# facebookresearch/habitat-lab

Measured on AMD Instinct MI355X. Metric: env-steps/sec (SPS) PointNav RGB-D 256x256, 64 envs x 128 rollout, higher is better.
Workload: dtype f32; 1 GPU; PointNav SimpleCNN+GRU, 64 envs x 128 steps, 256x256 RGB-D synthetic; envs_per_gpu=64, rollout_steps=128, ppo_epoch=4, num_mini_batch=4, parallelism=dp1

## Files before the change

### habitat-lab_amd/csrc/conv_patch_bf3.h

```cpp
#pragma once
#include <atomic>
#include "igemm_bf3.h"

namespace hab {

constexpr int CPB_CC = 32;
constexpr int CPB_PIX = CPB_CC + 8;

struct PatchGeom {
    const float* in;
    int Hi, Wi, Ci;
    int Ho, Wo;
    int KH, KW, off_h, off_w;
    int flip;
    int TH, tiles_per_img, PW, PP;
    FastDiv dPW;
    int nt_m, nt_n;
};

template <class P, int TW, int WM, int WN, int TN, int BT>
struct ConvPatchCfg {
    static constexpr int NT = WM * WN * 64;
    static constexpr int BN = WN * TN * 32;
    static constexpr int ROWS_PER_MT = 32 / TW;
    static constexpr int TH = WM * ROWS_PER_MT;
    static constexpr int BP = BT * CPB_CC + 8;
    static constexpr int B_PLANE = BN * BP;
    static constexpr int MAX_PP = (TH + 2) * (TW + 2);
    static constexpr size_t LDS_BYTES = (size_t)(3 * MAX_PP * CPB_PIX + 3 * B_PLANE) * 2;
};

inline size_t cpb_w_elems(const ConvFwdProb& p) { return (size_t)p.N * p.K; }
inline size_t cpb_w_elems(const ConvDgradProb& p) { return (size_t)p.N * p.Kfull; }

__global__ void cpb_split_weights(const float* __restrict__ w, size_t n, unsigned short* __restrict__ planes) {
    const size_t e = (size_t)blockIdx.x * blockDim.x + threadIdx.x;
    if (e >= n) return;
    unsigned h1, h2, h3;
    bf3_split(w[e], h1, h2, h3);
    planes[e] = (unsigned short)h1; planes[n + e] = (unsigned short)h2; planes[2 * n + e] = (unsigned short)h3;
    bf3_split(-w[e], h1, h2, h3);
    planes[3 * n + e] = (unsigned short)h1; planes[4 * n + e] = (unsigned short)h2; planes[5 * n + e] = (unsigned short)h3;
}

constexpr int CPB_DRAW_SLOTS = 64;
__device__ unsigned cpb_draw_pool[CPB_DRAW_SLOTS * 16];

template <class P, int TW, int WM, int WN, int TN, int BT, bool PRE>
__global__ void __launch_bounds__(WM* WN * 64) conv_patch_bf3_kernel(const P p, const PatchGeom gq, const int sign_schedule,
                                                                      const unsigned short* __restrict__ wplanes, const size_t wn_elems,
                                                                      unsigned* __restrict__ dyn_ctr) {
    using Cfg = ConvPatchCfg<P, TW, WM, WN, TN, BT>;
    constexpr int NT = Cfg::NT, BN = Cfg::BN, BP = Cfg::BP, TH = Cfg::TH;
    constexpr int PU = (Cfg::MAX_PP * (CPB_CC / 4) + NT - 1) / NT;
    static_assert(EpiV4<P>::value, "transposed-accumulator epilogue");
    extern __shared__ __attribute__((aligned(16))) unsigned short smem16[];
    const int PPL = gq.PP * CPB_PIX;
    unsigned short* Pa = smem16;
    unsigned short* Bs = smem16 + 3 * Cfg::MAX_PP * CPB_PIX;

    const int t = threadIdx.x;
    const int lane = t & 63, wave = t >> 6;
    const int wm = wave / WN, wn = wave % WN;
    const int li = lane & 31, hi = lane >> 5;
    const int ntiles = gq.nt_m * gq.nt_n;
    auto tile_of = [&](int vb) {
        const int q = ntiles >> 3, r = ntiles & 7, xcd = vb & 7, idx = vb >> 3;
        return (xcd < r ? xcd * (q + 1) : r * (q + 1) + (xcd - r) * q) + idx;
    };
    const int ty = wm * Cfg::ROWS_PER_MT + li / TW, tx = li % TW;
    const int txc = tx < gq.Wo ? tx : gq.Wo - 1;
    const int pix0 = ty * gq.PW + txc;
    const int patch_units = gq.PP * (CPB_CC / 4);
    const int nchunks = gq.Ci / CPB_CC;
    const int nstage = 9 / BT;
    const typename P::KCtx kc = p.k_ctx(0, p.K);

    f32x4 pv[PU];
    int prow[PU], poff[PU];
#pragma unroll
    for (int j = 0; j < PU; ++j) {
        const int u = t + NT * j;
        const int pix = u >> 3, cq = u & 7;
        int pr, pc;
        gq.dPW.divmod(pix, pr, pc);
        const int w_ = pc + gq.off_w;
        const bool colok = (u < patch_units) & ((unsigned)w_ < (unsigned)gq.Wi);
        prow[j] = colok ? pr + gq.off_h : HAB_FAR;
        poff[j] = ((pr + gq.off_h) * gq.Wi + w_) * gq.Ci + cq * 4;
    }
    auto fetch_patch = [&](int tile_m, int chunk) {
        const int img = tile_m / gq.tiles_per_img, ho0 = (tile_m - img * gq.tiles_per_img) * TH;
        const float* base = gq.in + ((size_t)img * gq.Hi + ho0) * gq.Wi * gq.Ci + chunk * CPB_CC;
#pragma unroll
        for (int j = 0; j < PU; ++j) {
// ... 143 lines not shown
                    load_group(g + 1, 1);
                    constexpr int PA[6] = {2, 0, 1, 1, 0, 0}, PB[6] = {0, 2, 1, 0, 1, 0};
#pragma unroll
                    for (int q = 0; q < 6; ++q)
#pragma unroll
                        for (int j = 0; j < TN; ++j) {
                            acc[j] = __builtin_amdgcn_mfma_f32_32x32x16_bf16(bf[0][j][PB[q]], af[0][PA[q]], acc[j], 0, 0, 0);
                            acc2[j] = __builtin_amdgcn_mfma_f32_32x32x16_bf16(bf[1][j][PB[q]], af[1][PA[q]], acc2[j], 0, 0, 0);
                        }
                }
                __syncthreads();
            }
#pragma unroll
            for (int j = 0; j < TN; ++j)
#pragma unroll
                for (int v = 0; v < 16; ++v) {
                    tot[j][v] += acc[j][v] + acc2[j][v];
                    acc[j][v] = 0.0f; acc2[j][v] = 0.0f;
                }
        }
#pragma unroll
        for (int j = 0; j < TN; ++j)
#pragma unroll
            for (int v = 0; v < 16; ++v) acc[j][v] = flip_all ? -tot[j][v] : tot[j][v];
        {
            const int img = tile_m / gq.tiles_per_img, ho = (tile_m - img * gq.tiles_per_img) * TH + ty;
            const int m = (tx < gq.Wo && ho < gq.Ho) ? (img * gq.Ho + ho) * gq.Wo + tx : p.M;
            const typename P::EpiRow erow = p.epi_row(m);
#pragma unroll
            for (int j = 0; j < TN; ++j) {
                typename P::EpiCol4 ecol[4];
                typename P::EpiAux4 aux[4];
#pragma unroll
                for (int g = 0; g < 4; ++g) {
                    ecol[g] = p.epi_col4(n0 + (wn * TN + j) * 32 + 8 * g + 4 * hi);
                    aux[g] = p.epi_fetch4(erow, ecol[g]);
                }
#pragma unroll
                for (int g = 0; g < 4; ++g) {
                    f32x4 v;
                    v[0] = acc[j][4 * g]; v[1] = acc[j][4 * g + 1]; v[2] = acc[j][4 * g + 2]; v[3] = acc[j][4 * g + 3];
                    p.epi_store4(erow, ecol[g], aux[g], v);
                }
            }
        }
        if (!more) { leave(); break; }
        vb = vb_next;
        if (dyn) { const int i2 = s_draw[it & 1]; vb_next = i2 < run_len ? i2 * 8 + xcd : ntiles; }
        else vb_next = vb + gridDim.x;
        ++it;
    }
}

template <class P, int TW, int WM, int WN, int TN, int BT>
inline int conv_patch_bf3_launch(const P& p, PatchGeom gq, float* ws, size_t ws_floats, hipStream_t stream) {
    using Cfg = ConvPatchCfg<P, TW, WM, WN, TN, BT>;
    gq.TH = Cfg::TH;
    gq.tiles_per_img = cdiv(gq.Ho, Cfg::TH);
    gq.PW = gq.Wo + 2;
    gq.PP = (Cfg::TH + 2) * gq.PW;
    gq.dPW = FastDiv(gq.PW);
    if (gq.PP > Cfg::MAX_PP) return 1;
    const int B = p.M / (gq.Ho * gq.Wo);
    gq.nt_m = B * gq.tiles_per_img;
    gq.nt_n = cdiv(p.N, Cfg::BN);
    const int ntiles = gq.nt_m * gq.nt_n;
    static const int sign_schedule = !hab_env_flag("HAB_BF3_NOSIGN");
    constexpr int wgs_per_cu = 2;
    const int occ = (int)(160 * 1024 / Cfg::LDS_BYTES) < wgs_per_cu ? (int)(160 * 1024 / Cfg::LDS_BYTES) : wgs_per_cu;
    int grid = 256 * (occ > 0 ? occ : 1);
    if (grid > ntiles) grid = (ntiles + 7) / 8 * 8;
    constexpr int pre_min = 131072;
    const size_t wn_elems = cpb_w_elems(p);
    const bool pre = ws && ((reinterpret_cast<uintptr_t>(ws) & 15) == 0) && ws_floats * 4 >= wn_elems * 12 && p.M >= pre_min && (wn_elems % 4 == 0);
    hipError_t e = hipSuccess;
    static const bool dyn_on = !hab_env_flag("HAB_NO_DYN_TILES");
    unsigned* ctr = nullptr;
    if (dyn_on && grid < ntiles) {
        static std::atomic<unsigned> next_slot{0};
        static unsigned* pool = nullptr;
        static const hipError_t sym_err = hipGetSymbolAddress(reinterpret_cast<void**>(&pool), HIP_SYMBOL(cpb_draw_pool));
        if (sym_err != hipSuccess || !pool) return HAB_ERR_ARG;
        ctr = pool + (size_t)(next_slot.fetch_add(1, std::memory_order_relaxed) % CPB_DRAW_SLOTS) * 16;
    }
    if (pre) {
        auto kern = conv_patch_bf3_kernel<P, TW, WM, WN, TN, BT, true>;
        static const hipError_t attr_err = (Cfg::LDS_BYTES > 64 * 1024) ? hipFuncSetAttribute(reinterpret_cast<const void*>(kern), hipFuncAttributeMaxDynamicSharedMemorySize, (int)Cfg::LDS_BYTES) : hipSuccess;
        if (attr_err != hipSuccess) return (int)attr_err;
        unsigned short* planes = reinterpret_cast<unsigned short*>(ws);
        cpb_split_weights<<<(unsigned)((wn_elems + 255) / 256), 256, 0, stream>>>(p.w, wn_elems, planes);
        HAB_LAUNCH_CHECK();
        kern<<<grid, Cfg::NT, Cfg::LDS_BYTES, stream>>>(p, gq, sign_schedule, planes, wn_elems, ctr);
    } else {
        auto kern = conv_patch_bf3_kernel<P, TW, WM, WN, TN, BT, false>;
        static const hipError_t attr_err = (Cfg::LDS_BYTES > 64 * 1024) ? hipFuncSetAttribute(reinterpret_cast<const void*>(kern), hipFuncAttributeMaxDynamicSharedMemorySize, (int)Cfg::LDS_BYTES) : hipSuccess;
        if (attr_err != hipSuccess) return (int)attr_err;
        kern<<<grid, Cfg::NT, Cfg::LDS_BYTES, stream>>>(p, gq, sign_schedule, nullptr, 0, ctr);
    }
    HAB_LAUNCH_CHECK();
    return HAB_OK;
}

template <class P>
inline int conv_patch_bf3_dispatch(const P& p, const PatchGeom& gq, float* ws, size_t ws_floats, hipStream_t stream) {
    if (gq.KH != 3 || gq.KW != 3 || gq.Ci % CPB_CC != 0 || (p.N & 31) || gq.Wo > 32 || gq.Wo < 5 || p.M % (gq.Ho * gq.Wo) != 0) return 1;
    if (p.N != 32) return 1;
    if (gq.Wo > 16) return conv_patch_bf3_launch<P, 32, 4, 1, 1, 3>(p, gq, ws, ws_floats, stream);
    if (gq.Wo > 8) return conv_patch_bf3_launch<P, 16, 4, 1, 1, 3>(p, gq, ws, ws_floats, stream);
    return 1;
}

}
```

### habitat-lab_amd/csrc/engine.h

```cpp
#pragma once
#include <string.h>

#include <algorithm>
#include <string>
#include <vector>

#include "heads.h"
#include "ops.h"
#include "problems.h"
#include "resnet_ops.h"
#include "../../include/habitat_amd.h"

struct ParamSpec {
    std::string name;
    int64_t shape[4];
    int ndim;
    int64_t offset;
    int64_t numel;
    int is_buffer = 0;
};

struct Arena {
    int64_t used = 0;
    int64_t take(int64_t n) {
        const int64_t o = used;
        used += (n + 63) & ~(int64_t)63;
        return o;
    }
};

struct RnnForm {
    int chunks = 0;
    bool wave = false;
};

struct hab_policy {
    hab_policy_desc d;
    std::vector<ParamSpec> params;
    int64_t param_floats = 0, packed_floats = 0, work_floats = 0;
    float *P = nullptr, *G = nullptr, *PK = nullptr, *WK = nullptr;
    int64_t work_bound = 0;
    int Cin = 0;
    hab::ConvDesc c1, c2, c3;
    int fc_in = 0, rnn_in = 0, rnn_ld = 0, G_ = 3, L = 1;
    int i_c1w = -1, i_c1b = -1, i_c2w = -1, i_c2b = -1, i_c3w = -1, i_c3b = -1, i_fcw = -1, i_fcb = -1, i_aw = -1, i_ab = -1, i_cw = -1, i_cb = -1;
    int i_astd = -1;
    int head_K = 0;
    int64_t w_gsaved = -1;
    std::vector<int> i_wih, i_whh, i_bih, i_bhh;
    int64_t pk_c1f = -1, pk_c2f = -1, pk_c2d = -1, pk_c3f = -1, pk_c3d = -1, pk_fc = -1;
    int64_t pk_c1img = -1;
    std::vector<int64_t> pk_whht;
    std::vector<int64_t> pk_wiht;
    int64_t pk_wih0 = -1;
    int64_t w_a1 = -1, w_a2 = -1, w_a3 = -1, w_da1 = -1, w_da2 = -1, w_da3 = -1;
    int64_t w_rnnin = -1, w_drnnin = -1, w_hinit = -1, w_cinit = -1, w_probs = -1, w_logitsn = -1, w_dzv = -1, w_dv = -1, w_dfeat = -1,
            w_scratch = -1, w_value = -1, w_logp = -1, w_ent = -1, w_hmask = -1, w_gistep = -1, w_step_h = -1, w_ws = -1;
    std::vector<int64_t> w_gi, w_gates, w_hn, w_hprev, w_cprev, w_c, w_out, w_dgi, w_dgh, w_dlayer;
    int64_t ws_floats = 0;
    int last_B = 0, last_n = 0;
    const uint8_t* last_masks = nullptr;
    hipStream_t s2 = nullptr;
    std::vector<hipEvent_t> evs;
    int64_t w_ws2 = -1, ws2_floats = 0, w_fmask = -1, w_iota = -1;
    RnnForm form;
    struct ResNetPlan* rn = nullptr;
    int save_acts = 1;
    int training = 1;
    hab_allreduce_fn allreduce_cb = nullptr;
    void* allreduce_ctx = nullptr;
    int world_size = 1;
    hab_grad_ready_fn grad_ready_cb = nullptr;
    void* grad_ready_ctx = nullptr;
    struct hab_comm* comm = nullptr;
    const float* xg_feat = nullptr; const float* xg_perc = nullptr;
    int comm_err = 0;
    int64_t comm_first = -1;
    hipStream_t cur_stream = nullptr;
    uint64_t probe_mask = 0;
    struct ProbeEv { int tag; hipEvent_t first, second; };
    std::vector<ProbeEv> probe_events;
    size_t probe_used = 0;
    double probe_flops[64] = {0}, probe_bytes[64] = {0};

    float* p(int i) const { return P + params[i].offset; }
    float* g(int i) const { return G + params[i].offset; }
};

inline int add_param(hab_policy* e, const std::string& name, std::initializer_list<int64_t> shape) {
    ParamSpec s;
    s.name = name;
    s.ndim = (int)shape.size();
    s.numel = 1;
    int k = 0;
    for (auto v : shape) { s.shape[k++] = v; s.numel *= v; }
    for (; k < 4; ++k) s.shape[k] = 1;
    s.offset = e->param_floats;
    e->param_floats += (s.numel + 3) & ~(int64_t)3;
    e->params.push_back(s);
    return (int)e->params.size() - 1;
}
inline int conv_out(int x, int k, int s, int p) { return (x + 2 * p - k) / s + 1; }

void add_tail_params(hab_policy* e);
void pack_tail(hab_policy* e, Arena& pk);
void plan_tail_workspace(hab_policy* e, Arena& wk, int64_t ws_floats);
int repack_tail(hab_policy* e, hipStream_t s);
int build_resnet(hab_policy* e);
void destroy_resnet(hab_policy* e);
int resnet_repack(hab_policy* e, hipStream_t s);
void grad_tail_ready(hab_policy* e, int first_param);
int comm_exchange_async(struct hab_comm* c, float* buf, int64_t first, int64_t count, hipStream_t compute);
extern "C" int hab_comm_allreduce_sum(struct hab_comm* c, float* buf, int64_t count, hipStream_t stream);
int resnet_feature_shape(const hab_policy* e, int* c, int* hf, int* wf);
int resnet_encode(hab_policy* e, const hab_obs* obs, int n, float* out, hipStream_t s);
int resnet_encoder_forward(hab_policy* e, const hab_obs* obs, const uint8_t* masks, const int* rows, int B, hipStream_t s, int f0 = 0, int nB = -1);
int resnet_encoder_backward(hab_policy* e, const hab_obs* obs, const uint8_t* masks, const int* rows, int B, hipStream_t s);
int resnet_tap(hab_policy* e, int which, const float** ptr, int64_t* floats);

struct Probe {
    hab_policy* e; hipStream_t s; bool on;
    Probe(hab_policy* e_, int tag, hipStream_t s_, double flops = 0.0, double bytes = 0.0) : e(e_), s(s_), on((e_->probe_mask >> tag) & 1) {
        if (!on) return;
        e->probe_flops[tag] += flops; e->probe_bytes[tag] += bytes;
        if (e->probe_used == e->probe_events.size()) {
            hipEvent_t a, b;
            (void)hipEventCreate(&a); (void)hipEventCreate(&b);
            e->probe_events.push_back({tag, a, b});
        }
        e->probe_events[e->probe_used].tag = tag;
        (void)hipEventRecord(e->probe_events[e->probe_used].first, s);
    }
    ~Probe() {
        if (!on) return;
        (void)hipEventRecord(e->probe_events[e->probe_used].second, s);
        e->probe_used++;
    }
};
```

### habitat-lab_amd/csrc/engine.hip

```cpp
#include <string.h>

#include <algorithm>

#include <string>
#include <vector>

#include "engine.h"

using namespace hab;

static void plan_tm_workspace(hab_policy* e, Arena& wk);
void add_tail_params(hab_policy* e) {
    const hab_policy_desc& d = e->d;
    const int H = d.hidden;
    const std::string rn = "net.state_encoder.rnn.";
    for (int l = 0; l < d.rnn_layers; ++l) {
        const int in = l == 0 ? e->rnn_in : H;
        const std::string sfx = "_l" + std::to_string(l);
        e->i_wih.push_back(add_param(e, rn + "weight_ih" + sfx, {e->G_ * H, in}));
        e->i_whh.push_back(add_param(e, rn + "weight_hh" + sfx, {e->G_ * H, H}));
        e->i_bih.push_back(add_param(e, rn + "bias_ih" + sfx, {e->G_ * H}));
        e->i_bhh.push_back(add_param(e, rn + "bias_hh" + sfx, {e->G_ * H}));
    }
    if (d.action_dist == HAB_DIST_GAUSSIAN) {
        if (d.gauss_flags & HAB_GAUSS_USE_STD_PARAM) e->i_astd = add_param(e, "action_distribution.std", {d.num_actions});
        e->head_K = (d.gauss_flags & HAB_GAUSS_USE_STD_PARAM) ? d.num_actions : 2 * d.num_actions;
        e->i_aw = add_param(e, "action_distribution.mu_maybe_std.weight", {e->head_K, H});
        e->i_ab = add_param(e, "action_distribution.mu_maybe_std.bias", {e->head_K});
    } else {
        e->i_aw = add_param(e, "action_distribution.linear.weight", {d.num_actions, H});
        e->i_ab = add_param(e, "action_distribution.linear.bias", {d.num_actions});
    }
    e->i_cw = add_param(e, "critic.fc.weight", {1, H});
    e->i_cb = add_param(e, "critic.fc.bias", {1});
}
void pack_tail(hab_policy* e, Arena& pk) {
    const int64_t GH = (int64_t)e->G_ * e->d.hidden;
    for (int l = 0; l < e->L; ++l) e->pk_whht.push_back(pk.take(GH * e->d.hidden));
    for (int l = 0; l < e->L; ++l) e->pk_wiht.push_back(l == 0 ? -1 : pk.take(GH * e->d.hidden));
    e->pk_wih0 = pk.take(GH * e->rnn_ld);
}
int repack_tail(hab_policy* e, hipStream_t s) {
    const int H = e->d.hidden;
    for (int l = 0; l < e->L; ++l) HAB_TRY(transpose2d(e->p(e->i_whh[l]), e->PK + e->pk_whht[l], e->G_ * H, H, s));
    for (int l = 1; l < e->L; ++l) HAB_TRY(transpose2d(e->p(e->i_wih[l]), e->PK + e->pk_wiht[l], e->G_ * H, H, s));
    return pad_rows(e->p(e->i_wih[0]), e->PK + e->pk_wih0, e->G_ * H, e->rnn_in, e->rnn_ld, s);
}
void plan_tail_workspace(hab_policy* e, Arena& wk, int64_t ws_floats) {
    const hab_policy_desc& d = e->d;
    const int64_t B = d.max_frames, F = d.max_frames;
    const int64_t H = d.hidden, GH = e->G_ * H;
    e->w_rnnin = wk.take(B * e->rnn_ld); e->w_drnnin = wk.take(B * e->rnn_ld);
    e->w_hinit = wk.take(e->L * F * H); e->w_cinit = wk.take(e->L * F * H);
    for (int l = 0; l < e->L; ++l) {
        e->w_gi.push_back(wk.take(B * GH)); e->w_gates.push_back(wk.take(B * GH));
        e->w_hn.push_back(wk.take(B * H)); e->w_hprev.push_back(wk.take(B * H));
        e->w_cprev.push_back(wk.take(B * H)); e->w_c.push_back(wk.take(B * H)); e->w_out.push_back(wk.take(B * H));
        e->w_dgi.push_back(wk.take(B * GH)); e->w_dgh.push_back(wk.take(B * GH));
        e->w_dlayer.push_back(wk.take(B * H));
    }
    e->w_probs = wk.take(B * 8); e->w_logitsn = wk.take(B * 8); e->w_dzv = wk.take(B * 8); e->w_dv = wk.take(B);
    e->w_dfeat = wk.take(B * H); e->w_scratch = wk.take((int64_t)std::max(3, 2 * e->L) * F * H);
    e->w_value = wk.take(B); e->w_logp = wk.take(B); e->w_ent = wk.take(B);
    if (d.action_dist == HAB_DIST_GAUSSIAN) e->w_gsaved = wk.take(B * 16);
    e->w_hmask = wk.take(2 * H * e->L * d.max_envs);
    e->w_gistep = wk.take(d.max_envs * GH);
    e->w_step_h = wk.take(d.max_envs * H * 2);
    e->ws_floats = ws_floats;
    e->w_ws = wk.take(ws_floats);
    plan_tm_workspace(e, wk);
}

static int build_baseline(hab_policy* e) {
    const hab_policy_desc& d = e->d;
    e->Cin = (d.has_rgb ? 3 : 0) + (d.has_depth ? 1 : 0);
    const bool blind = e->Cin == 0;
    if (blind && d.goal_dim <= 0) return HAB_ERR_ARG;
    if (d.rnn_type != HAB_RNN_GRU && d.rnn_type != HAB_RNN_LSTM) return HAB_ERR_ARG;
    const int H = d.hidden;
    e->G_ = d.rnn_type == HAB_RNN_GRU ? 3 : 4;
    e->L = d.rnn_layers;
    e->c1 = ConvDesc{0, d.H, d.W, blind ? 4 : e->Cin, 32, 8, 8, 4, 0};
    e->c2 = ConvDesc{0, conv_out(d.H, 8, 4, 0), conv_out(d.W, 8, 4, 0), 32, 64, 4, 4, 2, 0};
    e->c3 = ConvDesc{0, e->c2.Ho(), e->c2.Wo(), 64, 32, 3, 3, 1, 0};
    const int h3 = e->c3.Ho(), w3 = e->c3.Wo();
    if (!blind && (h3 <= 0 || w3 <= 0)) return HAB_ERR_ARG;
    e->fc_in = blind ? 0 : 32 * h3 * w3;
    e->rnn_in = (blind ? 0 : H) + d.goal_dim;
    e->rnn_ld = (e->rnn_in + 15) & ~15;
    const std::string ve = "net.visual_encoder.cnn.";
    if (!blind) {
        e->i_c1w = add_param(e, ve + "0.weight", {32, e->Cin, 8, 8});
        e->i_c1b = add_param(e, ve + "0.bias", {32});
        e->i_c2w = add_param(e, ve + "2.weight", {64, 32, 4, 4});
        e->i_c2b = add_param(e, ve + "2.bias", {64});
        e->i_c3w = add_param(e, ve + "4.weight", {32, 64, 3, 3});
        e->i_c3b = add_param(e, ve + "4.bias", {32});
        e->i_fcw = add_param(e, ve + "6.weight", {H, e->fc_in});
        e->i_fcb = add_param(e, ve + "6.bias", {H});
    }
    add_tail_params(e);

    Arena pk;
    e->pk_c1f = pk.take(32 * 64 * (blind ? 4 : e->Cin));
    e->pk_c1img = (!blind && e->Cin == 4) ? pk.take(obs_conv_weight_image_floats()) : -1;
    e->pk_c2f = pk.take(64 * 16 * 32);
    e->pk_c2d = pk.take(64 * 16 * 32);
    e->pk_c3f = pk.take(32 * 9 * 64);
    e->pk_c3d = pk.take(32 * 9 * 64);
    e->pk_fc = pk.take((int64_t)H * std::max(e->fc_in, 4));
    pack_tail(e, pk);
    e->packed_floats = pk.used;

    Arena wk;
    const int64_t B = d.max_frames;
    const int64_t m1 = blind ? 0 : (int64_t)e->c1.Ho() * e->c1.Wo() * 32, m2 = blind ? 0 : (int64_t)e->c2.Ho() * e->c2.Wo() * 64, m3 = e->fc_in;
    e->w_a1 = wk.take(B * m1); e->w_a2 = wk.take(B * m2); e->w_a3 = wk.take(B * m3);
    e->w_da1 = wk.take(B * m1); e->w_da2 = wk.take(B * m2); e->w_da3 = wk.take(B * m3);
    plan_tail_workspace(e, wk, std::max<int64_t>((int64_t)16 << 20, (int64_t)8 * H * e->fc_in / 4));
    e->work_floats = wk.used;
    return HAB_OK;
}

extern "C" int hab_policy_create(const hab_policy_desc* desc, hab_policy** out) {
    if (!desc || !out) return HAB_ERR_ARG;
    if (desc->hidden <= 0 || desc->hidden % 64 || desc->num_actions <= 0 || desc->num_actions > 8 || desc->max_frames <= 0 ||
        desc->max_envs <= 0 || desc->rnn_layers <= 0 || desc->goal_dim < 0 ||
        ((desc->has_rgb || desc->has_depth || desc->has_semantic) && (desc->H <= 0 || desc->W <= 0)))
        return HAB_ERR_ARG;
    if (desc->action_dist != HAB_DIST_CATEGORICAL && (desc->action_dist != HAB_DIST_GAUSSIAN || desc->arch != HAB_ARCH_RESNET))
        return HAB_ERR_UNSUPPORTED;
    if (desc->action_dist == HAB_DIST_GAUSSIAN && desc->num_actions > 4) return HAB_ERR_UNSUPPORTED;
    hab_policy* e = new hab_policy();
    e->d = *desc;
    int rc = HAB_ERR_UNSUPPORTED;
    if (desc->arch == HAB_ARCH_SIMPLE_CNN) rc = build_baseline(e);
    else if (desc->arch == HAB_ARCH_RESNET) rc = build_resnet(e);
    if (rc != HAB_OK) { destroy_resnet(e); delete e; return rc; }
    *out = e;
    return HAB_OK;
}
extern "C" void hab_policy_destroy(hab_policy* e) {
    if (!e) return;
    for (auto& ev : e->probe_events) { (void)hipEventDestroy(ev.first); (void)hipEventDestroy(ev.second); }
    for (auto& ev : e->evs) (void)hipEventDestroy(ev);
    if (e->s2) (void)hipStreamDestroy(e->s2);
    destroy_resnet(e);
    delete e;
}
extern "C" int hab_policy_num_params(const hab_policy* e) { return e ? (int)e->params.size() : HAB_ERR_ARG; }
extern "C" int hab_policy_param_info(const hab_policy* e, int i, char* name, int name_cap, int64_t* shape4, int* ndim,
                                     int64_t* offset_floats) {
    if (!e || i < 0 || i >= (int)e->params.size() || !name || name_cap <= 0) return HAB_ERR_ARG;
    const ParamSpec& s = e->params[i];
    strncpy(name, s.name.c_str(), name_cap - 1);
    name[name_cap - 1] = 0;
    if (shape4) for (int k = 0; k < 4; ++k) shape4[k] = s.shape[k];
    if (ndim) *ndim = s.ndim;
    if (offset_floats) *offset_floats = s.offset;
    return HAB_OK;
}
extern "C" int hab_policy_param_is_buffer(const hab_policy* e, int i) {
    if (!e || i < 0 || i >= (int)e->params.size()) return HAB_ERR_ARG;
    return e->params[i].is_buffer;
}
extern "C" int hab_policy_set_training(hab_policy* e, int training) {
    if (!e) return HAB_ERR_ARG;
    e->training = training ? 1 : 0;
    return HAB_OK;
}
extern "C" int hab_policy_set_grad_ready(hab_policy* e, hab_grad_ready_fn fn, void* ctx) {
    if (!e) return HAB_ERR_ARG;
    e->grad_ready_cb = fn; e->grad_ready_ctx = ctx;
    return HAB_OK;
}
void grad_tail_ready(hab_policy* e, int first_param) {
    if (e->comm) {
        static const bool no_overlap = hab_env_flag("HAB_NO_GRAD_OVERLAP");
        if (no_overlap || e->comm_err != HAB_OK) return;
        const int64_t first = e->g(first_param) - e->G;
        const int64_t end = e->comm_first < 0 ? (int64_t)e->param_floats : e->comm_first;
        if (first >= end) return;
        const int rc = comm_exchange_async(e->comm, e->G, first, end - first, e->cur_stream);
        if (rc == HAB_OK) e->comm_first = first;
        else e->comm_err = rc;
        return;
    }
    if (!e->grad_ready_cb) return;
    const int64_t first = e->g(first_param) - e->G;
    e->grad_ready_cb(first, (int64_t)e->param_floats - first, e->grad_ready_ctx);
}
extern "C" int hab_policy_set_allreduce(hab_policy* e, hab_allreduce_fn fn, void* ctx, int world_size) {
    if (!e || world_size < 1) return HAB_ERR_ARG;
    e->allreduce_cb = fn; e->allreduce_ctx = ctx; e->world_size = world_size;
    return HAB_OK;
}
extern "C" int64_t hab_policy_param_floats(const hab_policy* e) { return e ? e->param_floats : -1; }
extern "C" int64_t hab_policy_packed_floats(const hab_policy* e) { return e ? e->packed_floats : -1; }
extern "C" int64_t hab_policy_work_floats(const hab_policy* e) { return e ? e->work_floats : -1; }

extern "C" int hab_policy_bind(hab_policy* e, float* params, float* grads, float* packed, float* work, int64_t work_floats) {
    if (!e || !params || !packed || !work) return HAB_ERR_ARG;
    if (work_floats < e->work_floats) return HAB_ERR_ARG;
    if ((((uintptr_t)params | (uintptr_t)grads | (uintptr_t)packed | (uintptr_t)work) & 255) != 0) return HAB_ERR_ARG;
    e->P = params; e->G = grads; e->PK = packed; e->WK = work; e->work_bound = work_floats;
    return HAB_OK;
}

extern "C" int hab_policy_repack(hab_policy* e, hipStream_t stream) {
    if (!e || !e->P) return HAB_ERR_ARG;
    if (e->rn) return resnet_repack(e, stream);
    if (e->Cin == 0) return repack_tail(e, stream);
    HAB_TRY(repack_conv(e->p(e->i_c1w), e->PK + e->pk_c1f, nullptr, 32, e->Cin, 8, 8, e->Cin, stream));
    if (e->pk_c1img >= 0) {
        const int rc = obs_conv_weight_image(e->PK + e->pk_c1f, 32, 8, 8, e->Cin, e->PK + e->pk_c1img, stream);
        if (rc != HAB_OK) return rc == 1 ? HAB_ERR_UNSUPPORTED : rc;
    }
    HAB_TRY(repack_conv(e->p(e->i_c2w), e->PK + e->pk_c2f, e->PK + e->pk_c2d, 64, 32, 4, 4, 32, stream));
    HAB_TRY(repack_conv(e->p(e->i_c3w), e->PK + e->pk_c3f, e->PK + e->pk_c3d, 32, 64, 3, 3, 64, stream));
    HAB_TRY(repack_flatten(e->p(e->i_fcw), e->PK + e->pk_fc, e->d.hidden, 32, e->fc_in / 32, stream));
    return repack_tail(e, stream);
}

extern "C" int hab_policy_probe_enable(hab_policy* e, int tag) {
    if (!e || tag >= 64) return HAB_ERR_ARG;
    e->probe_mask = tag < 0 ? 0 : (uint64_t)1 << tag;
    e->probe_used = 0;
    for (int i = 0; i < 64; ++i) { e->probe_flops[i] = 0.0; e->probe_bytes[i] = 0.0; }
    return HAB_OK;
}
extern "C" int hab_policy_probe_enable_mask(hab_policy* e, uint64_t mask) {
    if (!e) return HAB_ERR_ARG;
    e->probe_mask = mask;
    e->probe_used = 0;
    for (int i = 0; i < 64; ++i) { e->probe_flops[i] = 0.0; e->probe_bytes[i] = 0.0; }
    return HAB_OK;
}
static int probe_sum(hab_policy* e, int tag, double* total_ms, int* count) {
    double t = 0;
    int n = 0;
    for (size_t i = 0; i < e->probe_used; ++i) {
        if (tag >= 0 && e->probe_events[i].tag != tag) continue;
        hipError_t err = hipEventSynchronize(e->probe_events[i].second);
        if (err != hipSuccess) return (int)err;
        float ms = 0;
        err = hipEventElapsedTime(&ms, e->probe_events[i].first, e->probe_events[i].second);
        if (err != hipSuccess) return (int)err;
        t += ms;
        ++n;
    }
    *total_ms = t;
    *count = n;
    return HAB_OK;
}
extern "C" int hab_policy_probe_work(hab_policy* e, int tag, double* flops, double* bytes) {
    if (!e || tag < 0 || tag >= 64 || !flops || !bytes) return HAB_ERR_ARG;
    *flops = e->probe_flops[tag]; *bytes = e->probe_bytes[tag];
    return HAB_OK;
}
extern "C" int hab_policy_probe_read(hab_policy* e, double* total_ms, int* count) {
    if (!e || !total_ms || !count) return HAB_ERR_ARG;
    HAB_TRY(probe_sum(e, -1, total_ms, count));
    e->probe_used = 0;
    return HAB_OK;
}
extern "C" int hab_policy_probe_read_tag(hab_policy* e, int tag, double* total_ms, int* count) {
    if (!e || !total_ms || !count || tag < 0 || tag >= 64) return HAB_ERR_ARG;
    return probe_sum(e, tag, total_ms, count);
}


static int encoder_forward(hab_policy* e, const hab_obs* obs, const uint8_t* masks, const int* rows, int B, hipStream_t s, int f0 = 0, int nB = -1) {
    if (e->rn) { Probe pr(e, HAB_PROBE_ENC_FWD, s); return resnet_encoder_forward(e, obs, masks, rows, B, s, f0, nB); }
    if (nB < 0) nB = B;
    float* W = e->WK;
    float* ws = W + e->w_ws;
    const int H = e->d.hidden;
    if (e->Cin == 0) {
        if (!rows && f0) return HAB_ERR_ARG;
        return gather_cols(obs->goal, e->d.goal_dim, rows ? rows + f0 : nullptr, W + e->w_rnnin + (int64_t)f0 * e->rnn_ld, e->rnn_ld, 0, e->d.goal_dim,
                           e->rnn_ld - e->rnn_in, nB, s);
    }
    const int64_t m1 = (int64_t)e->c1.Ho() * e->c1.Wo() * 32, m2 = (int64_t)e->c2.Ho() * e->c2.Wo() * 64, m3 = e->fc_in;
    float *a1 = W + e->w_a1 + f0 * m1, *a2 = W + e->w_a2 + f0 * m2, *a3 = W + e->w_a3 + f0 * m3, *rin = W + e->w_rnnin + (int64_t)f0 * e->rnn_ld;
    const int* rws = rows ? rows + f0 : nullptr;
    if (!rows && f0) return HAB_ERR_ARG;
    ObsView ov;
    ov.rgb = e->d.has_rgb ? obs->rgb : nullptr; ov.depth = e->d.has_depth ? obs->depth : nullptr; ov.rows = rws;
    ov.H = e->d.H; ov.W = e->d.W; ov.C = e->Cin;
    ConvDesc c1 = e->c1, c2 = e->c2, c3 = e->c3;
    c1.B = c2.B = c3.B = nB;
    { Probe pr(e, HAB_PROBE_CONV1_FWD, s);
      HAB_TRY(obs_conv_fwd(c1, ov, e->PK + e->pk_c1f, e->p(e->i_c1b), a1, 1, ws, e->ws_floats, s, e->pk_c1img >= 0 ? e->PK + e->pk_c1img : nullptr)); }
    { Probe pr(e, HAB_PROBE_CONV2_FWD, s);
      HAB_TRY(conv_fwd(c2, a1, e->PK + e->pk_c2f, e->p(e->i_c2b), a2, 1, ws, e->ws_floats, s)); }
    { Probe pr(e, HAB_PROBE_CONV3_FWD, s);
      HAB_TRY(conv_fwd(c3, a2, e->PK + e->pk_c3f, e->p(e->i_c3b), a3, 0, ws, e->ws_floats, s)); }
    { Probe pr(e, HAB_PROBE_FC_FWD, s);
      HAB_TRY(linear_fwd(a3, e->fc_in, e->PK + e->pk_fc, e->fc_in, e->p(e->i_fcb), rin, e->rnn_ld, nB, H, e->fc_in, 1, 0, ws, e->ws_floats, s)); }
    if (e->d.goal_dim > 0)
        HAB_TRY(gather_cols(obs->goal, e->d.goal_dim, rws, rin, e->rnn_ld, H, e->d.goal_dim, e->rnn_ld - e->rnn_in, nB, s));
    return HAB_OK;
}

static RnnForm rnn_form_cfg(const hab_policy* e, int frames, int n, bool tm_shape) {
    static const int chunks = hab_env_int("HAB_RNN_CHUNKS", 4), chunks_resnet = hab_env_int("HAB_RNN_CHUNKS_RESNET", -1);
    static const int wave = hab_env_int("HAB_RNN_WAVE", 1);
    RnnForm f;
    if (tm_shape) {
        int nc = chunks;
        if (e->rn && chunks > 1) nc = chunks_resnet >= 0 ? chunks_resnet : frames >= 4096 ? 2 : 0;
        f.chunks = std::max(0, std::min(nc, frames / n));
    }
    if (f.chunks == 0) f.wave = wave && e->L >= 2 && e->L <= 4;
    return f;
}
static RnnForm rnn_form(const hab_policy* e, const int* rows, const hab_pack_info* pack, int B, int n) {
    const bool tm_shape = e->Cin > 0 && rows && !pack->env_first_frame && (B % n) == 0 && B / n >= 2 && e->w_ws2 >= 0 &&
                          (int64_t)e->L * 2 * n <= 3 * (int64_t)e->d.max_frames;
    return rnn_form_cfg(e, B, n, tm_shape);
}
static void plan_tm_workspace(hab_policy* e, Arena& wk) {
    const int64_t B = e->d.max_frames;
    if (rnn_form_cfg(e, (int)B, 1, true).chunks == 0) return;
    e->ws2_floats = e->ws_floats;
    e->w_ws2 = wk.take(e->ws2_floats);
    e->w_fmask = wk.take((B + 3) / 4 + 64);
    e->w_iota = wk.take(B + 64);
}
static int tm_setup(hab_policy* e, int nev) {
    if (!e->s2) {
        int lo = 0, hi = 0;
        (void)hipDeviceGetStreamPriorityRange(&lo, &hi);
        hipError_t err = hipStreamCreateWithPriority(&e->s2, hipStreamNonBlocking, hi);
        if (err != hipSuccess) return (int)err;
    }
    while ((int)e->evs.size() < nev) {
        hipEvent_t ev;
        hipError_t err = hipEventCreateWithFlags(&ev, hipEventDisableTiming);
        if (err != hipSuccess) return (int)err;
        e->evs.push_back(ev);
    }
    return HAB_OK;
}
static int tm_order(hab_policy* e, int ev, hipStream_t from, hipStream_t to) {
    hipError_t err = hipEventRecord(e->evs[ev], from);
    if (err != hipSuccess) return (int)err;
    err = hipStreamWaitEvent(to, e->evs[ev], 0);
    return err == hipSuccess ? HAB_OK : (int)err;
}

static RnnLayerParams layer_params(hab_policy* e, int l) {
    RnnLayerParams lp;
    lp.w_ih = e->p(e->i_wih[l]); lp.w_hh = e->p(e->i_whh[l]); lp.b_ih = e->p(e->i_bih[l]); lp.b_hh = e->p(e->i_bhh[l]);
    lp.w_hh_t = e->PK + e->pk_whht[l];
    if (e->G) { lp.dw_ih = e->g(e->i_wih[l]); lp.dw_hh = e->g(e->i_whh[l]); lp.db_ih = e->g(e->i_bih[l]); lp.db_hh = e->g(e->i_bhh[l]); }
    else { lp.dw_ih = lp.dw_hh = lp.db_ih = lp.db_hh = nullptr; }
    lp.in_dim = l == 0 ? e->rnn_in : e->d.hidden;
    if (l == 0 && e->pk_wih0 >= 0) { lp.w_ih_pad = e->PK + e->pk_wih0; lp.w_ih_ld = e->rnn_ld; }
    else if (l > 0 && (e->d.hidden & 15) == 0) { lp.w_ih_pad = lp.w_ih; lp.w_ih_ld = e->d.hidden; }
    return lp;
}
static RnnWork layer_work(hab_policy* e, int l) {
    float* W = e->WK;
    RnnWork wk;
    wk.gi = W + e->w_gi[l]; wk.gates = W + e->w_gates[l]; wk.hn = W + e->w_hn[l]; wk.hprev = W + e->w_hprev[l];
    wk.cprev = W + e->w_cprev[l]; wk.c = W + e->w_c[l]; wk.out = W + e->w_out[l]; wk.dgi = W + e->w_dgi[l];
    wk.dgh = W + e->w_dgh[l];
    return wk;
}
static const float* layer_x(const hab_policy* e, int l) { return e->WK + (l == 0 ? e->w_rnnin : e->w_out[l - 1]); }
static int layer_ld(const hab_policy* e, int l) { return l == 0 ? e->rnn_ld : e->d.hidden; }
static float* layer_dx(const hab_policy* e, int l) { return e->WK + (l == 0 ? e->w_drnnin : e->w_dlayer[l]); }
static const float* layer_dout(const hab_policy* e, int l) { return l == e->L - 1 ? e->WK + e->w_dfeat : layer_dx(e, l + 1); }
static PackInfo pack_info(const hab_pack_info* pack, int n) {
    PackInfo pk;
    pk.select_inds = pack->select_inds; pk.step_offsets = pack->step_offsets_host; pk.num_seqs_at_step = pack->num_seqs_at_step_host;
    pk.frag_env = pack->frag_env; pk.frag_start = pack->frag_start; pk.P = pack->P; pk.F = pack->F; pk.max_len = pack->max_len;
    pk.n_envs = n;
    return pk;
}

extern "C" int hab_policy_encode(hab_policy* e, const hab_obs* obs, int n, float* out, hipStream_t stream) {
    if (!e || !e->P || !obs || !out || n <= 0 || n > e->d.max_frames) return HAB_ERR_ARG;
    if (!e->rn) return HAB_ERR_UNSUPPORTED;
    Probe pr(e, HAB_PROBE_ENC_FWD, stream);
    e->save_acts = 0;
    const int rc = resnet_encode(e, obs, n, out, stream);
    e->save_acts = 1;
    return rc;
}
extern "C" int hab_policy_visual_feature_shape(const hab_policy* e, int* c, int* hf, int* wf) {
    if (!e || !c || !hf || !wf) return HAB_ERR_ARG;
    if (!e->rn) return HAB_ERR_UNSUPPORTED;
    return resnet_feature_shape(e, c, hf, wf);
}

extern "C" int hab_policy_act(hab_policy* e, const hab_obs* obs, const float* hidden_in, const uint8_t* masks,
                              const float* exp_noise, int deterministic, int n, float* values, int64_t* actions,
                              float* action_log_probs, float* hidden_out, float* probs_out, hipStream_t stream) {
    if (!e || !e->P || !obs || !hidden_in || !masks || !values || n <= 0 || n > e->d.max_envs) return HAB_ERR_ARG;
// ... 16 lines not shown
        float* hout = hidden_out ? hidden_out + (size_t)l * H : step_h + (size_t)(l & 1) * n * H;
        const int hstride = hidden_out ? Lh * H : H;
        float* cout = (hidden_out && e->d.rnn_type == HAB_RNN_LSTM) ? hidden_out + (size_t)(L + l) * H : nullptr;
        HAB_TRY(rnn_step_layer_forward(e->d.rnn_type, H, lp, x, ldx, hidden_in + (size_t)l * H, Lh * H,
                                       e->d.rnn_type == HAB_RNN_LSTM ? hidden_in + (size_t)(L + l) * H : nullptr, Lh * H, masks, n,
                                       W + e->w_gistep, hout, hstride, cout, Lh * H, W + e->w_ws, e->ws_floats, stream));
        x = hout;
        ldx = hstride;
    }
    if (e->d.action_dist == HAB_DIST_GAUSSIAN) {
        GaussHeadsArgs ga;
        ga.B = n; ga.H = H; ga.A = e->d.num_actions; ga.K = e->head_K; ga.flags = e->d.gauss_flags;
        ga.min_std = e->d.gauss_min_std; ga.max_std = e->d.gauss_max_std;
        ga.mode = actions ? (deterministic ? 2 : 1) : 2;
        ga.feats = x; ga.feats_ld = ldx; ga.w = e->p(e->i_aw); ga.b = e->p(e->i_ab);
        ga.std_param = e->i_astd >= 0 ? e->p(e->i_astd) : nullptr; ga.w_critic = e->p(e->i_cw); ga.b_critic = e->p(e->i_cb);
        ga.actions_in = nullptr; ga.rows = nullptr; ga.noise = exp_noise;
        ga.actions_out = actions ? reinterpret_cast<float*>(actions) : W + e->w_dzv;
        ga.value = values; ga.logp = action_log_probs ? action_log_probs : W + e->w_logp; ga.entropy = nullptr; ga.saved = nullptr;
        if (ga.mode == 1 && !exp_noise) return HAB_ERR_ARG;
        if (probs_out) return HAB_ERR_ARG;
        return gauss_heads_forward(ga, stream);
    }
    HeadsArgs ha;
    ha.B = n; ha.H = H; ha.A = e->d.num_actions;
    ha.mode = actions ? (deterministic ? 2 : 1) : 2;
    ha.feats = x; ha.feats_ld = ldx; ha.w_actor = e->p(e->i_aw); ha.b_actor = e->p(e->i_ab); ha.w_critic = e->p(e->i_cw); ha.b_critic = e->p(e->i_cb);
    ha.actions_in = nullptr; ha.rows = nullptr; ha.noise = exp_noise;
    ha.actions_out = actions ? actions : reinterpret_cast<int64_t*>(W + e->w_dzv);
    ha.value = values; ha.logp = action_log_probs ? action_log_probs : W + e->w_logp; ha.entropy = nullptr;
    ha.probs = probs_out ? W + e->w_probs : nullptr; ha.logits_n = W + e->w_logitsn;
    if (ha.mode == 1 && !exp_noise) return HAB_ERR_ARG;
    HAB_TRY(heads_forward(ha, stream));
    if (probs_out) HAB_TRY(copy_rows(W + e->w_probs, nullptr, 8, probs_out, 8, n, 8, stream));
    return HAB_OK;
}

static int rnn_state_init(hab_policy* e, const float* hidden0, int hidden_env_stride, const int* rows, const uint8_t* masks,
                          const int* frag_env, const int* frag_start, int F, const int* env_first_frame, hipStream_t s) {
    const int H = e->d.hidden, L = e->L;
    for (int l = 0; l < L; ++l) {
        HAB_TRY(rnn_frag_init(hidden0 + (size_t)l * H, rows, hidden_env_stride, masks, rows, frag_env, frag_start, F, H,
                              e->WK + e->w_hinit + (size_t)l * F * H, s, env_first_frame));
        if (e->d.rnn_type == HAB_RNN_LSTM)
            HAB_TRY(rnn_frag_init(hidden0 + (size_t)(L + l) * H, rows, hidden_env_stride, masks, rows, frag_env, frag_start, F, H,
                                  e->WK + e->w_cinit + (size_t)l * F * H, s, env_first_frame));
    }
    return HAB_OK;
}
static int rnn_tm_forward(hab_policy* e, const hab_obs* obs, const int* rows, const float* hidden0, int hidden_env_stride,
                          const uint8_t* masks, int B, int n, hipStream_t stream) {
    float* W = e->WK;
    const int H = e->d.hidden, L = e->L, NC = e->form.chunks, T = B / n, Tc = (T + NC - 1) / NC;
    HAB_TRY(tm_setup(e, 2 * NC + 4));
    hipStream_t sB = e->s2;
    uint8_t* fmask = reinterpret_cast<uint8_t*>(W + e->w_fmask);
    HAB_TRY(rnn_tm_prepare(masks, rows, B, fmask, reinterpret_cast<int*>(W + e->w_iota), stream));
    HAB_TRY(rnn_state_init(e, hidden0, hidden_env_stride, rows, masks, nullptr, nullptr, n, nullptr, stream));
    for (int c = 0; c < NC; ++c) {
        const int t0 = c * Tc, t1 = std::min(T, t0 + Tc);
        if (t0 >= t1) break;
        HAB_TRY(encoder_forward(e, obs, masks, rows, B, stream, t0 * n, (t1 - t0) * n));
        HAB_TRY(tm_order(e, c, stream, sB));
        for (int l = 0; l < L; ++l) {
            Probe pr(e, HAB_PROBE_RNN_FWD, sB);
            HAB_TRY(rnn_tm_layer_forward(e->d.rnn_type, H, layer_params(e, l), layer_work(e, l), layer_x(e, l), layer_ld(e, l),
                                         W + e->w_hinit + (size_t)l * n * H, W + e->w_cinit + (size_t)l * n * H, fmask, n, T, t0, t1,
                                         W + e->w_ws2, e->ws2_floats, sB));
        }
    }
    return tm_order(e, NC, sB, stream);
}
static int rnn_packed_forward(hab_policy* e, const int* rows, const float* hidden0, int hidden_env_stride, const uint8_t* masks,
                              const hab_pack_info* pack, int n, hipStream_t stream) {
    float* W = e->WK;
    const int H = e->d.hidden, L = e->L;
    const PackInfo pk = pack_info(pack, n);
    HAB_TRY(rnn_state_init(e, hidden0, hidden_env_stride, rows, masks, pk.frag_env, pk.frag_start, pk.F, pack->env_first_frame, stream));
    if (e->form.wave) {
        RnnLayerParams lps[4]; RnnWork wks[4]; const float* hin[4]; const float* cin[4];
        for (int l = 0; l < L; ++l) {
            lps[l] = layer_params(e, l); wks[l] = layer_work(e, l);
            hin[l] = W + e->w_hinit + (size_t)l * pk.F * H; cin[l] = W + e->w_cinit + (size_t)l * pk.F * H;
        }
        Probe pr(e, HAB_PROBE_RNN_FWD, stream);
        const int rc = rnn_seq_wave_forward(e->d.rnn_type, H, L, lps, wks, layer_x(e, 0), layer_ld(e, 0), hin, cin, pk, W + e->w_ws,
                                            e->ws_floats, stream);
        return rc == 1 ? HAB_ERR_UNSUPPORTED : rc;
    }
    for (int l = 0; l < L; ++l) {
        Probe pr(e, HAB_PROBE_RNN_FWD, stream);
        HAB_TRY(rnn_seq_layer_forward(e->d.rnn_type, H, layer_params(e, l), layer_work(e, l), layer_x(e, l), layer_ld(e, l),
                                      W + e->w_hinit + (size_t)l * pk.F * H, W + e->w_cinit + (size_t)l * pk.F * H, pk, W + e->w_ws,
                                      e->ws_floats, stream));
    }
    return HAB_OK;
}

extern "C" int hab_policy_evaluate(hab_policy* e, const hab_obs* obs, const int* rows, const float* hidden0,
                                   int hidden_env_stride, const uint8_t* masks, const int64_t* actions,
                                   const hab_pack_info* pack, int B, int n, float* value, float* log_prob, float* entropy,
                                   hipStream_t stream) {
    if (!e || !e->P || !obs || !hidden0 || !masks || !actions || !pack || B <= 0 || n <= 0 || B > e->d.max_frames) return HAB_ERR_ARG;
    if (!pack->env_first_frame && (B % n)) return HAB_ERR_ARG;
    if (pack->P != B || pack->F <= 0 || pack->F > B || pack->max_len <= 0) return HAB_ERR_ARG;
    float* W = e->WK;
    const int H = e->d.hidden, L = e->L;
    e->form = rnn_form(e, rows, pack, B, n);
    if (e->form.chunks > 0) {
        HAB_TRY(rnn_tm_forward(e, obs, rows, hidden0, hidden_env_stride, masks, B, n, stream));
    } else {
        HAB_TRY(encoder_forward(e, obs, masks, rows, B, stream));
        HAB_TRY(rnn_packed_forward(e, rows, hidden0, hidden_env_stride, masks, pack, n, stream));
    }
    const float* feats = W + e->w_out[L - 1];
    if (e->d.action_dist == HAB_DIST_GAUSSIAN) {
        GaussHeadsArgs ga;
        ga.B = B; ga.H = H; ga.A = e->d.num_actions; ga.K = e->head_K; ga.flags = e->d.gauss_flags; ga.mode = 0;
        ga.min_std = e->d.gauss_min_std; ga.max_std = e->d.gauss_max_std;
        ga.feats = feats; ga.feats_ld = H; ga.w = e->p(e->i_aw); ga.b = e->p(e->i_ab);
        ga.std_param = e->i_astd >= 0 ? e->p(e->i_astd) : nullptr; ga.w_critic = e->p(e->i_cw); ga.b_critic = e->p(e->i_cb);
        ga.actions_in = reinterpret_cast<const float*>(actions); ga.rows = rows; ga.noise = nullptr; ga.actions_out = nullptr;
        ga.value = value ? value : W + e->w_value; ga.logp = log_prob ? log_prob : W + e->w_logp;
        ga.entropy = entropy ? entropy : W + e->w_ent; ga.saved = W + e->w_gsaved;
// ... 14 lines not shown
    return HAB_OK;
}

extern "C" int hab_policy_final_hidden(hab_policy* e, float* hidden_out, hipStream_t stream) {
    if (!e || !hidden_out || e->last_B <= 0 || e->last_n <= 0) return HAB_ERR_ARG;
    const int H = e->d.hidden, L = e->L, n = e->last_n, B = e->last_B;
    const int Lh = e->d.rnn_type == HAB_RNN_LSTM ? 2 * L : L;
    for (int l = 0; l < L; ++l) {
        HAB_TRY(copy_rows(e->WK + e->w_out[l] + (size_t)(B - n) * H, nullptr, H, hidden_out + (size_t)l * H, Lh * H, n, H, stream));
        if (e->d.rnn_type == HAB_RNN_LSTM)
            HAB_TRY(copy_rows(e->WK + e->w_c[l] + (size_t)(B - n) * H, nullptr, H, hidden_out + (size_t)(L + l) * H, Lh * H, n, H, stream));
    }
    return HAB_OK;
}

__global__ void add_rows_kernel(float* __restrict__ dst, const float* __restrict__ src, long long n) {
    for (long long i = (long long)blockIdx.x * blockDim.x + threadIdx.x; i < n; i += (long long)gridDim.x * blockDim.x) dst[i] += src[i];
}
__global__ void add_masked_cols_kernel(float* __restrict__ dst, int ldd, const float* __restrict__ src, const float* __restrict__ x, int ldx,
                                       int B, int H) {
    const long long n = (long long)B * H;
    for (long long i = (long long)blockIdx.x * blockDim.x + threadIdx.x; i < n; i += (long long)gridDim.x * blockDim.x) {
        const int f = (int)(i / H), c = (int)(i % H);
        if (x[(size_t)f * ldx + c] > 0.f) dst[(size_t)f * ldd + c] += src[i];
    }
}
extern "C" int hab_policy_set_extra_grads(hab_policy* e, const float* d_rnn_output, const float* d_perception_embed) {
    if (!e) return HAB_ERR_ARG;
    if (d_perception_embed && e->Cin == 0) return HAB_ERR_ARG;
    e->xg_feat = d_rnn_output; e->xg_perc = d_perception_embed;
    return HAB_OK;
}

static int cnn_dgrad(hab_policy* e, int64_t f0, int nB, hipStream_t s) {
    float* W = e->WK;
    float* ws = W + e->w_ws;
    const int64_t m1 = (int64_t)e->c1.Ho() * e->c1.Wo() * 32, m2 = (int64_t)e->c2.Ho() * e->c2.Wo() * 64, m3 = e->fc_in;
    ConvDesc c2 = e->c2, c3 = e->c3;
    c2.B = c3.B = nB;
    { Probe pr(e, HAB_PROBE_FC_DGRAD, s);
      HAB_TRY(linear_dgrad(W + e->w_drnnin + f0 * e->rnn_ld, e->rnn_ld, e->PK + e->pk_fc, e->fc_in, nullptr, 0, 0, W + e->w_da3 + f0 * m3,
                           e->fc_in, nB, e->fc_in, e->d.hidden, 0, ws, e->ws_floats, s)); }
    { Probe pr(e, HAB_PROBE_CONV3_DGRAD, s);
      HAB_TRY(conv_dgrad(c3, W + e->w_da3 + f0 * m3, e->PK + e->pk_c3d, W + e->w_a2 + f0 * m2, nullptr, W + e->w_da2 + f0 * m2, ws,
                         e->ws_floats, s)); }
    { Probe pr(e, HAB_PROBE_CONV2_DGRAD, s);
      HAB_TRY(conv_dgrad(c2, W + e->w_da2 + f0 * m2, e->PK + e->pk_c2d, W + e->w_a1 + f0 * m1, nullptr, W + e->w_da1 + f0 * m1, ws,
                         e->ws_floats, s)); }
    return HAB_OK;
}
static int rnn_tm_backward(hab_policy* e, int B, hipStream_t stream) {
    float* W = e->WK;
    const int H = e->d.hidden, L = e->L, n = e->last_n, T = B / n, NC = e->form.chunks, Tc = (T + NC - 1) / NC;
    hipStream_t sB = e->s2;
    const uint8_t* fmask = reinterpret_cast<const uint8_t*>(W + e->w_fmask);
    const int* iota = reinterpret_cast<const int*>(W + e->w_iota);
    HAB_TRY(tm_order(e, NC + 1, stream, sB));
    for (int c = NC - 1; c >= 0; --c) {
        const int t0 = c * Tc, t1 = std::min(T, t0 + Tc);
        if (t0 >= t1) continue;
        for (int l = L - 1; l >= 0; --l) {
            Probe pr(e, HAB_PROBE_RNN_BWD, sB);
            HAB_TRY(rnn_tm_layer_backward(e->d.rnn_type, H, layer_params(e, l), layer_work(e, l), layer_dout(e, l), layer_dx(e, l), layer_ld(e, l),
                                          l == 0 ? layer_x(e, 0) : nullptr, layer_ld(e, l), H, fmask, iota, n, T, t0, t1,
                                          W + e->w_scratch + (size_t)l * 2 * n * H, W + e->w_ws2, e->ws2_floats, sB));
        }
        if (!e->rn) {
            HAB_TRY(tm_order(e, NC + 2 + c, sB, stream));
            HAB_TRY(cnn_dgrad(e, (int64_t)t0 * n, (t1 - t0) * n, stream));
        }
    }
    for (int l = L - 1; l >= 0; --l)
        HAB_TRY(rnn_tm_layer_param_grads(e->d.rnn_type, H, layer_params(e, l), layer_work(e, l), layer_x(e, l), layer_ld(e, l), B, W + e->w_ws2,
                                         e->ws2_floats, sB));
    return HAB_OK;
}
static int rnn_packed_backward(hab_policy* e, const hab_pack_info* pack, hipStream_t stream) {
    float* W = e->WK;
    const int H = e->d.hidden, L = e->L;
    const PackInfo pk = pack_info(pack, e->last_n);
    const bool blind0 = !e->rn && e->Cin == 0, nofc = e->Cin == 0;
    const float* x0 = layer_x(e, 0);
    if (e->form.wave) {
        RnnLayerParams lps[4]; RnnWork wks[4]; const float* wiht[4];
        for (int l = 0; l < L; ++l) { lps[l] = layer_params(e, l); wks[l] = layer_work(e, l); wiht[l] = l ? e->PK + e->pk_wiht[l] : nullptr; }
        Probe pr(e, HAB_PROBE_RNN_BWD, stream);
        const int rc = rnn_seq_wave_backward(e->d.rnn_type, H, L, lps, wiht, wks, x0, e->rnn_ld, layer_dout(e, L - 1), blind0 ? nullptr : layer_dx(e, 0),
                                             e->rnn_ld, nofc ? nullptr : x0, e->rnn_ld, nofc ? 0 : H, pk, W + e->w_scratch, W + e->w_ws, e->ws_floats,
                                             stream);
        return rc == 1 ? HAB_ERR_UNSUPPORTED : rc;
    }
    for (int l = L - 1; l >= 0; --l) {
        Probe pr(e, HAB_PROBE_RNN_BWD, stream);
        HAB_TRY(rnn_seq_layer_backward(e->d.rnn_type, H, layer_params(e, l), layer_work(e, l), layer_x(e, l), layer_ld(e, l), layer_dout(e, l),
                                       (blind0 && l == 0) ? nullptr : layer_dx(e, l), layer_ld(e, l), (l == 0 && !nofc) ? x0 : nullptr,
                                       layer_ld(e, l), nofc ? 0 : H, pk, W + e->w_scratch, W + e->w_ws, e->ws_floats, stream));
    }
    return HAB_OK;
}

static int policy_backward_impl(hab_policy* e, const hab_obs* obs, const int* rows, const int64_t* actions,
                                const hab_pack_info* pack, const float* d_value, const float* d_log_prob,
                                const float* d_entropy, hipStream_t stream) {
    if (!e || !e->P || !e->G || !obs || !actions || !pack || !d_value || !d_log_prob || !d_entropy || e->last_B <= 0)
        return HAB_ERR_ARG;
    e->comm_err = HAB_OK;
    float* W = e->WK;
    float* ws = W + e->w_ws;
    const int H = e->d.hidden, L = e->L, B = e->last_B, A = e->d.num_actions;
    e->cur_stream = stream;
    e->comm_first = -1;
    const float* feats = W + e->w_out[L - 1];
    if (e->d.action_dist == HAB_DIST_GAUSSIAN) {
        const int K = e->head_K;
        GaussHeadsBwdArgs gb;
        gb.B = B; gb.H = H; gb.A = A; gb.K = K; gb.d_value = d_value; gb.d_logp = d_log_prob; gb.d_entropy = d_entropy;
        gb.actions = reinterpret_cast<const float*>(actions); gb.rows = rows; gb.saved = W + e->w_gsaved;
        gb.w = e->p(e->i_aw); gb.w_critic = e->p(e->i_cw); gb.dfeat = W + e->w_dfeat; gb.dz = W + e->w_dzv; gb.dv_out = W + e->w_dv;
        HAB_TRY(gauss_heads_backward(gb, stream));
        HAB_TRY(linear_wgrad(W + e->w_dzv, 8, feats, H, e->g(e->i_aw), H, B, K, H, 0, 0, 0, ws, e->ws_floats, stream));
        HAB_TRY(colsum(W + e->w_dzv, 8, B, K, e->g(e->i_ab), 0, ws, e->ws_floats, stream));
        if (e->i_astd >= 0) HAB_TRY(colsum(W + e->w_dzv + A, 8, B, A, e->g(e->i_astd), 0, ws, e->ws_floats, stream));
        HAB_TRY(linear_wgrad(W + e->w_dv, 1, feats, H, e->g(e->i_cw), H, B, 1, H, 0, 0, 0, ws, e->ws_floats, stream));
        HAB_TRY(colsum(W + e->w_dv, 1, B, 1, e->g(e->i_cb), 0, ws, e->ws_floats, stream));
    } else {
    HeadsBwdArgs hb;
        hb.B = B; hb.H = H; hb.A = A; hb.d_value = d_value; hb.d_logp = d_log_prob; hb.d_entropy = d_entropy;
        hb.actions = actions; hb.rows = rows; hb.probs = W + e->w_probs; hb.logits_n = W + e->w_logitsn;
        hb.w_actor = e->p(e->i_aw); hb.w_critic = e->p(e->i_cw); hb.dfeat = W + e->w_dfeat; hb.dzv = W + e->w_dzv; hb.dv_out = W + e->w_dv;
        HAB_TRY(heads_backward(hb, stream));
        HAB_TRY(linear_wgrad(W + e->w_dzv, 8, feats, H, e->g(e->i_aw), H, B, A, H, 0, 0, 0, ws, e->ws_floats, stream));
        HAB_TRY(linear_wgrad(W + e->w_dv, 1, feats, H, e->g(e->i_cw), H, B, 1, H, 0, 0, 0, ws, e->ws_floats, stream));
        HAB_TRY(colsum(W + e->w_dzv, 8, B, A, e->g(e->i_ab), 0, ws, e->ws_floats, stream));
        HAB_TRY(colsum(W + e->w_dv, 1, B, 1, e->g(e->i_cb), 0, ws, e->ws_floats, stream));
    }
    const int NC = e->form.chunks;
    if (e->xg_feat || e->xg_perc) {
        if (NC > 0) return HAB_ERR_UNSUPPORTED;
        if (e->xg_feat) {
            add_rows_kernel<<<(int)std::min<long long>(1024, cdivl((long long)B * H, 256)), 256, 0, stream>>>(W + e->w_dfeat, e->xg_feat, (long long)B * H);
            HAB_LAUNCH_CHECK();
        }
    }
    if (NC > 0) {
        HAB_TRY(rnn_tm_backward(e, B, stream));
    } else {
        HAB_TRY(rnn_packed_backward(e, pack, stream));
        if (e->xg_perc) {
            add_masked_cols_kernel<<<(int)std::min<long long>(1024, cdivl((long long)B * H, 256)), 256, 0, stream>>>(
                W + e->w_drnnin, e->rnn_ld, e->xg_perc, W + e->w_rnnin, e->rnn_ld, B, H);
            HAB_LAUNCH_CHECK();
        }
        if (!e->rn && e->Cin == 0) {
            grad_tail_ready(e, e->i_wih[0]);
            return HAB_OK;
        }
    }
    if (e->rn) {
        if (NC > 0) HAB_TRY(tm_order(e, 2 * NC + 3, e->s2, stream));
        Probe pr(e, HAB_PROBE_ENC_BWD, stream);
        return resnet_encoder_backward(e, obs, e->last_masks, rows, B, stream);
    }
    const float* dfc = W + e->w_drnnin;
    { Probe pr(e, HAB_PROBE_FC_WGRAD, stream);
      HAB_TRY(linear_wgrad(dfc, e->rnn_ld, W + e->w_a3, e->fc_in, e->g(e->i_fcw), e->fc_in, B, H, e->fc_in, 32, e->fc_in / 32, 0,
                           ws, e->ws_floats, stream)); }
    HAB_TRY(colsum(dfc, e->rnn_ld, B, H, e->g(e->i_fcb), 0, ws, e->ws_floats, stream));
    if (NC > 0) HAB_TRY(tm_order(e, 2 * NC + 3, e->s2, stream));
    grad_tail_ready(e, e->i_fcw);
    if (NC == 0) HAB_TRY(cnn_dgrad(e, 0, B, stream));
    ConvDesc c1 = e->c1, c2 = e->c2, c3 = e->c3;
    c1.B = c2.B = c3.B = B;
    { Probe pr(e, HAB_PROBE_CONV3_WGRAD, stream);
      HAB_TRY(conv_wgrad(c3, W + e->w_a2, W + e->w_da3, e->g(e->i_c3w), e->g(e->i_c3b), ws, e->ws_floats, stream)); }
    { Probe pr(e, HAB_PROBE_CONV2_WGRAD, stream);
      HAB_TRY(conv_wgrad(c2, W + e->w_a1, W + e->w_da2, e->g(e->i_c2w), e->g(e->i_c2b), ws, e->ws_floats, stream)); }
    ObsView ov;
    ov.rgb = e->d.has_rgb ? obs->rgb : nullptr; ov.depth = e->d.has_depth ? obs->depth : nullptr; ov.rows = rows;
    ov.H = e->d.H; ov.W = e->d.W; ov.C = e->Cin;
    { Probe pr(e, HAB_PROBE_CONV1_WGRAD, stream);
      HAB_TRY(obs_conv_wgrad(c1, ov, W + e->w_da1, e->g(e->i_c1w), e->g(e->i_c1b), ws, e->ws_floats, stream)); }
    return HAB_OK;
}
extern "C" int hab_policy_backward(hab_policy* e, const hab_obs* obs, const int* rows, const int64_t* actions,
                                   const hab_pack_info* pack, const float* d_value, const float* d_log_prob,
                                   const float* d_entropy, hipStream_t stream) {
    const int rc = policy_backward_impl(e, obs, rows, actions, pack, d_value, d_log_prob, d_entropy, stream);
    if (e) e->xg_feat = e->xg_perc = nullptr;
    return (rc == HAB_OK && e && e->comm_err != HAB_OK) ? e->comm_err : rc;
}

extern "C" int hab_policy_tap(hab_policy* e, int which, const float** ptr, int64_t* floats) {
    if (!e || !ptr || !floats || e->last_B <= 0) return HAB_ERR_ARG;
    const int64_t B = e->last_B;
    float* W = e->WK;
// ... 13 lines not shown
```

### habitat-lab_amd/csrc/engine_resnet.hip

```cpp
#include "engine.h"

using namespace hab;

namespace {

struct RnConv {
    ConvDesc cd;
    int groups = 0;
    int i_w = -1, i_gamma = -1, i_beta = -1;
    int64_t pk_f = -1, pk_d = -1;
    int64_t pk_p = -1;
    int64_t w_raw = -1, w_mean = -1, w_rstd = -1, w_out = -1;
    int cgroups = 1;
    int64_t out_floats() const { return (int64_t)cd.Ho() * cd.Wo() * cd.Cout; }
    int64_t in_floats() const { return (int64_t)cd.H * cd.W * cd.C; }
};

struct RnBlock {
    std::vector<int> convs;
    int ds = -1;
    int64_t w_in = -1;
    int64_t w_out = -1;
    int se_c = 0, se_r = 0;
    int i_se1w = -1, i_se1b = -1, i_se2w = -1, i_se2b = -1;
// ... 238 lines not shown
            place(c, true);
            r->gbuf_floats = std::max(r->gbuf_floats, c.out_floats());
        }
        if (blk.ds >= 0) { place(r->convs[blk.ds], true); r->gbuf_floats = std::max(r->gbuf_floats, r->convs[blk.ds].out_floats()); }
        blk.w_out = r->convs[blk.convs.back()].w_out;
        if (blk.se_c) {
            blk.w_out = wk.take(B * r->convs[blk.convs.back()].out_floats());
            blk.w_se_pool = wk.take(B * blk.se_c); blk.w_se_h = wk.take(B * blk.se_r); blk.w_se_gate = wk.take(B * blk.se_c);
        }
        prev = blk.w_out;
    }
    place(r->comp, true);
    r->gbuf_floats = std::max(r->gbuf_floats, r->comp.out_floats());
    for (int k = 0; k < 2; ++k) r->w_gstem[k] = wk.take(B * r->stem.out_floats());
    for (int k = 0; k < 6; ++k) r->w_gbuf.push_back(wk.take(B * r->gbuf_floats));
    r->w_chansums = wk.take(B * 2 * r->cmax);
    r->w_stats = wk.take(64);
    r->w_dscratch = wk.take(2 * (INGEST_MOM_MAX_BLOCKS * 16 + 16));
    if (se) r->w_se_scr = wk.take(B * ((int64_t)3 * r->cmax + r->cmax / 16 + 16));
    if (r->gdense_floats) r->w_gdense = wk.take(r->gdense_floats);
    }
    r->w_embsave = wk.take(B * 4 * EMB_MAX_SLOTS);
    plan_tail_workspace(e, wk, (int64_t)32 << 20);
    e->work_floats = wk.used;
    return HAB_OK;
}

void destroy_resnet(hab_policy* e) {
    delete e->rn;
    e->rn = nullptr;
}

int resnet_repack(hab_policy* e, hipStream_t s) {
    ResNetPlan* r = e->rn;
    auto rp = [&](const RnConv& c, int cin_real) {
        if (c.cgroups > 1)
            return repack_conv_grouped(e->p(c.i_w), e->PK + c.pk_f, c.pk_d >= 0 ? e->PK + c.pk_d : nullptr, c.cd.Cout, c.cd.C, c.cgroups,
                                       c.cd.KH, c.cd.KW, s);
        return repack_conv(e->p(c.i_w), e->PK + c.pk_f, c.pk_d >= 0 ? e->PK + c.pk_d : nullptr, c.cd.Cout, cin_real, c.cd.KH, c.cd.KW,
                           c.cd.C, s);
    };
    auto planes = [&](const RnConv& c) {
        if (c.pk_p < 0) return (int)HAB_OK;
        return weight_planes(e->PK + c.pk_f, c.cd.Cout, c.cd.KH * c.cd.KW * c.cd.C, reinterpret_cast<unsigned short*>(e->PK + c.pk_p), s);
    };
    if (!r->blind) {
        HAB_TRY(rp(r->stem, r->creal));
        if (r->stem.pk_p >= 0) HAB_TRY(stem_weight_planes(e->PK + r->stem.pk_f, reinterpret_cast<unsigned short*>(e->PK + r->stem.pk_p), s));
        for (const auto& c : r->convs) { HAB_TRY(rp(c, c.cd.C)); HAB_TRY(planes(c)); }
        HAB_TRY(rp(r->comp, r->comp.cd.C));
        HAB_TRY(planes(r->comp));
        HAB_TRY(repack_flatten(e->p(r->i_fcw), e->PK + r->pk_fc, e->d.hidden, r->comp_c, r->comp_hw, s));
    }
    return repack_tail(e, s);
}

static int fill_embed_slots(hab_policy* e, const hab_obs* obs, EmbedSlot* sl, bool grads) {
    ResNetPlan* r = e->rn;
    const hab_policy_desc& d = e->d;
    int n = 0;
    auto add = [&](int kind, const void* in, int iw, int ib, int ntok) {
        EmbedSlot& q = sl[n++];
        q.kind = kind; q.in = in; q.w = e->p(iw); q.b = ib >= 0 ? e->p(ib) : nullptr; q.ntok = ntok;
        q.dw = grads ? e->g(iw) : nullptr; q.db = (grads && ib >= 0) ? e->g(ib) : nullptr;
        return in != nullptr;
    };
    bool ok = true;
    if (d.goal_dim == 2) ok &= add(EMB_POLAR, obs->goal, r->i_tgw, r->i_tgb, 0);
    if (d.pointgoal_dim > 0) ok &= add(EMB_LINN, obs->pointgoal, r->i_pgw, r->i_pgb, d.pointgoal_dim);
    if (d.proximity_dim > 0) ok &= add(EMB_LINN, obs->proximity, r->i_pxw, r->i_pxb, d.proximity_dim);
    if (d.num_object_categories > 0) ok &= add(EMB_TOKEN, obs->objectgoal, r->i_objw, -1, d.num_object_categories);
    if (d.has_compass) ok &= add(EMB_COSSIN, obs->compass, r->i_cmpw, r->i_cmpb, 0);
    if (d.has_gps) ok &= add(EMB_LIN2, obs->gps, r->i_gpsw, r->i_gpsb, 0);
    if (d.action_dist == HAB_DIST_GAUSSIAN) ok &= add(EMB_PREVLIN, obs->prev_actions, r->i_emb, r->i_embb, d.num_actions);
    else ok &= add(EMB_PREV, obs->prev_actions, r->i_emb, -1, d.num_actions + 1);
    return (ok && n == r->nslots) ? HAB_OK : HAB_ERR_ARG;
}

static GnArgs gn_args(hab_policy* e, const RnConv& c, int B, int f0, int relu, const float* residual) {
    float* W = e->WK;
    GnArgs g;
    g.x = W + c.w_raw + (int64_t)f0 * c.out_floats(); g.y = W + c.w_out + (int64_t)f0 * c.out_floats();
    g.gamma = e->p(c.i_gamma); g.beta = e->p(c.i_beta); g.residual = residual;
    g.mean = W + c.w_mean + (int64_t)f0 * c.groups; g.rstd = W + c.w_rstd + (int64_t)f0 * c.groups;
    g.B = B; g.HW = c.cd.Ho() * c.cd.Wo(); g.C = c.cd.Cout; g.groups = c.groups; g.relu = relu; g.eps = 1e-5f;
    g.scratch = W + e->w_ws; g.scratch_floats = e->ws_floats;
    return g;
}

static int conv_gn_forward(hab_policy* e, const RnConv& c, const float* in, const float* residual, int relu, int B, hipStream_t s, int f0 = 0) {
    float* W = e->WK;
    ConvDesc cd = c.cd;
    cd.B = B;
    float* raw = W + c.w_raw + (int64_t)f0 * c.out_floats();
    const GnArgs g = gn_args(e, c, B, f0, relu, residual);
    constexpr int cgs_max_b = 256;
    if (c.pk_p >= 0 && B <= cgs_max_b && !e->save_acts) {
        ConvGnArgs q;
        q.x = in; q.w_planes = reinterpret_cast<const unsigned short*>(e->PK + c.pk_p); q.gamma = e->p(c.i_gamma); q.beta = e->p(c.i_beta);
        q.residual = residual; q.y = g.y;
        q.B = B; q.H = cd.H; q.W = cd.W; q.C = cd.C; q.Cout = cd.Cout; q.KH = cd.KH; q.KW = cd.KW; q.stride = cd.stride; q.pad = cd.pad;
        q.groups = c.groups; q.relu = relu; q.eps = 1e-5f;
        const int rc = conv_gn_fused(q, s);
        if (rc != 1) return rc;
    }
    HAB_TRY(conv_fwd(cd, in, e->PK + c.pk_f, nullptr, raw, 0, W + e->w_ws, e->ws_floats, s));
    return groupnorm_forward(g, s);
// ... 432 lines not shown
```

### habitat-lab_amd/csrc/gemm_ops.hip

```cpp
#include "igemm.h"
#include "igemm_dma.h"
#include "igemm_dma_wgrad.h"
#include "igemm_bf3.h"
#include "igemm_bf3_ws.h"
#include "dense_bf3.h"
#include "obs_conv_bf3.h"
#include "obs_conv_bf3_ws.h"
#include "obs_conv_patch.h"
#include "wgrad3x3_bf3.h"
#include "conv2_fwd_strip.h"
#include "conv2_dgrad_strip.h"
#include "obs_wgrad_bf3.h"
#include "conv_patch_bf3.h"
#include "wgrad3x3_patch.h"
#include "prob_build.h"
#include <stdlib.h>

#include <atomic>

#include "../../include/habitat_amd.h"

namespace hab {

static bool no_dma() { static const bool v = hab_env_flag("HAB_NO_DMA"); return v; }
// ... 37 lines not shown
            if (p.N <= 32) return bf3_launch<P, 2, 1, 4, 1>(p, ws, ws_floats, target_blocks, stream);
            if (p.N <= 64) {
                if (p.M >= 256 * 512 && p.K >= 576) return bf3_launch<P, 2, 2, 4, 1>(p, ws, ws_floats, target_blocks, stream);
                return bf3_launch<P, 1, 2, 4, 1>(p, ws, ws_floats, target_blocks, stream);
            }
            return bf3_launch<P, 2, 2, 2, 2>(p, ws, ws_floats, target_blocks, stream);
        }
    } else if constexpr (AKv<P>::value == 4) {
        if ((bf3_mode() & 4) && p.M > 64) {
            if (p.N <= 32) {
                if constexpr (WG) {
                    if (p.M % 96 == 0 || cdiv(p.M, 96) * 96 < cdiv(p.M, 256) * 256)
                        return bf3_launch<P, 1, 1, 3, 1>(p, ws, ws_floats, target_blocks, stream);
                }
                return bf3_launch<P, 2, 1, 4, 1>(p, ws, ws_floats, target_blocks, stream);
            }
            if (p.N <= 64) {
                if constexpr (WG) {
                    if (p.M % 96 == 0 || cdiv(p.M, 96) * 96 < cdiv(p.M, 128) * 128)
                        return bf3_launch<P, 1, 2, 3, 1>(p, ws, ws_floats, target_blocks, stream);
                }
                return bf3_launch<P, 1, 2, 4, 1>(p, ws, ws_floats, target_blocks, stream);
            }
            return bf3_launch<P, 2, 2, 2, 2>(p, ws, ws_floats, target_blocks, stream);
        }
    }
    if constexpr (std::is_same_v<P, ConvFwdProb> || std::is_same_v<P, ConvDgradProb>) {
        if (p.dma_ok() && p.M > 64 && !no_dma()) {
            if (p.N <= 32) return igemm_dma_launch<P, 2, 1, 4, 1, false>(p, ws, ws_floats, target_blocks, stream);
            if (p.N <= 64) return igemm_dma_launch<P, 1, 2, 4, 1, false>(p, ws, ws_floats, target_blocks, stream);
            if (p.N <= 128) return igemm_dma_launch<P, 2, 2, 2, 2, true>(p, ws, ws_floats, target_blocks, stream);
        }
    }
    if (p.N <= 32) {
        if (p.M <= 64) return igemm_launch<P, 1, 1, 2, 1>(p, ws, ws_floats, target_blocks, stream);
        if constexpr (WG) {
            if (p.M % 96 == 0 || cdiv(p.M, 96) * 96 < cdiv(p.M, 256) * 256)
                return igemm_launch<P, 1, 1, 3, 1>(p, ws, ws_floats, target_blocks, stream);
        }
        return igemm_launch<P, 2, 1, 4, 1>(p, ws, ws_floats, target_blocks, stream);
    } else if (p.N <= 64) {
        if (p.M <= 64) return igemm_launch<P, 1, 1, 2, 2>(p, ws, ws_floats, target_blocks, stream);
        if constexpr (WG) {
            if (p.M % 96 == 0 || cdiv(p.M, 96) * 96 < cdiv(p.M, 128) * 128)
                return igemm_launch<P, 1, 2, 3, 1>(p, ws, ws_floats, target_blocks, stream);
        }
        return igemm_launch<P, 1, 2, 4, 1>(p, ws, ws_floats, target_blocks, stream);
    } else {
        if (p.M <= 64) return igemm_launch<P, 1, 2, 2, 2>(p, ws, ws_floats, target_blocks, stream);
        return igemm_launch<P, 2, 2, 2, 2>(p, ws, ws_floats, target_blocks, stream);
    }
}

int conv_fwd(const ConvDesc& d, const float* x, const float* wf, const float* bias, float* y, int relu, float* ws,
             size_t ws_floats, hipStream_t stream) {
    ConvFwdProb p;
    HAB_TRY(build(p, d, x, wf, bias, y, relu));
    if ((bf3_mode() & 256) && (bf3_mode() & 1)) {
        const int rc = conv2_fwd_strip(p, ws, ws_floats, stream);
        if (rc != 1) return rc;
    }
    if ((bf3_mode() & 16) && d.stride == 1 && d.KH == 3 && d.KW == 3 && p.M > 64) {
        PatchGeom gq{};
        gq.in = x; gq.Hi = d.H; gq.Wi = d.W; gq.Ci = d.C; gq.Ho = p.g.Ho; gq.Wo = p.g.Wo; gq.KH = 3; gq.KW = 3;
        gq.off_h = -d.pad; gq.off_w = -d.pad; gq.flip = 0;
        const int rc = conv_patch_bf3_dispatch(p, gq, ws, ws_floats, stream);
        if (rc != 1) return rc;
    }
    return run_igemm(p, ws, ws_floats, stream);
}
int64_t obs_conv_weight_image_floats() { return ((int64_t)OCP_W_ELEMS + 1) / 2 + 4; }
int obs_conv_weight_image(const float* wf, int Cout, int KH, int KW, int C, void* img, hipStream_t stream) {
    return obs_conv_patch_weight_image(wf, Cout, KH, KW, C, reinterpret_cast<unsigned short*>(img), stream);
}
int obs_conv_fwd(const ConvDesc& d, const ObsView& obs, const float* wf, const float* bias, float* y, int relu, float* ws,
                 size_t ws_floats, hipStream_t stream, const void* wimg) {
    ObsConvFwdProb p;
    HAB_TRY(build(p, d, obs, wf, bias, y, relu));
    if ((bf3_mode() & 64) && (bf3_mode() & 2) && p.quad) {
        const int rc = obs_conv_patch_launch(p, ws, ws_floats, stream, reinterpret_cast<const unsigned short*>(wimg));
        if (rc != 1) return rc;
    }
    if ((bf3_mode() & 32) && (bf3_mode() & 2) && p.quad && p.M > 64) {
        const int rc = obs_conv_bf3_ws_launch(p, ws, ws_floats, stream);
        if (rc != 1) return rc;
    }
    if ((bf3_mode() & 2) && p.quad && p.M > 64) {
        const int rc = obs_conv_bf3_launch<2>(p, ws, ws_floats, stream);
        if (rc != 1) return rc;
    }
    return run_igemm(p, ws, ws_floats, stream);
}
__global__ void dgrad_empty_class_kernel(ConvDgradProb p) {
    const long long total = (long long)p.g.B * p.Hc * p.Wc * p.N;
    for (long long e = (long long)blockIdx.x * blockDim.x + threadIdx.x; e < total; e += (long long)gridDim.x * blockDim.x)
        p.store((int)(e / p.N), (int)(e % p.N), 0.f);
}

int conv_dgrad(const ConvDesc& d, const float* dy, const float* wd, const float* mask, const float* add, float* dx,
               float* ws, size_t ws_floats, hipStream_t stream) {
    if ((bf3_mode() & 512) && (bf3_mode() & 1)) {
        const int rc = conv2_dgrad_strip(d, dy, wd, mask, add, dx, stream);
        if (rc != 1) return rc;
    }
    if (d.stride > 1 && !no_dma() && !no_merged_dgrad()) {
        ConvDgradMergedProb q;
        HAB_TRY(check_conv(d));
        q.g = make_geom(d);
        if (ConvDgradMergedProb::applicable(q.g)) {
            q.dy = dy; q.w = wd; q.mask = mask; q.add = add; q.dx = dx;
            q.finish();
            if ((bf3_mode() & 1) && q.M > 64) {
                if (q.N <= 32) return bf3_launch<ConvDgradMergedProb, 2, 1, 4, 1>(q, ws, ws_floats, 256, stream);
                if (q.N <= 64) return bf3_launch<ConvDgradMergedProb, 1, 2, 4, 1>(q, ws, ws_floats, 256, stream);
                return bf3_launch<ConvDgradMergedProb, 2, 2, 2, 2>(q, ws, ws_floats, 256, stream);
            }
            if (q.dma_ok()) {
                if (q.N <= 32) return igemm_dma_launch<ConvDgradMergedProb, 2, 1, 4, 1, false>(q, ws, ws_floats, 1024, stream);
                if (q.N <= 64) return igemm_dma_launch<ConvDgradMergedProb, 1, 2, 4, 1, false>(q, ws, ws_floats, 1024, stream);
                return igemm_dma_launch<ConvDgradMergedProb, 2, 2, 2, 2, false>(q, ws, ws_floats, 1024, stream);
            }
        }
    }
    for (int ph = 0; ph < d.stride; ++ph)
        for (int pw = 0; pw < d.stride; ++pw) {
            ConvDgradProb p;
            HAB_TRY(build(p, d, dy, wd, mask, add, dx, ph, pw));
// ... 8 lines not shown
            }
            if (p.K <= 0) {
                p.M = d.B * p.Hc * p.Wc;
                dgrad_empty_class_kernel<<<1024, 256, 0, stream>>>(p);
                HAB_LAUNCH_CHECK();
                continue;
            }
            HAB_TRY(run_igemm(p, ws, ws_floats, stream));
        }
    return HAB_OK;
}
int conv_wgrad(const ConvDesc& d, const float* x, const float* dy, float* dw_oihw, float* dbias, float* ws, size_t ws_floats,
               hipStream_t stream) {
    ConvWgradProb p;
    HAB_TRY(build(p, d, x, dy, dw_oihw, dbias));
    if (ws && (bf3_mode() & 8) && (bf3_mode() & 128) && wgrad3x3_bf3_shape(p)) {
        const int rc = wgrad3x3_bf3(p, ws, ws_floats, stream);
        if (rc != 1) return rc;
    }
    if (ws && wgrad3x3_patch_ok(p) && !no_patch() && !(bf3_mode() & 8)) {
        ConvWgradProb q = p;
        q.colsum = nullptr;
        if (dbias) HAB_TRY(colsum(dy, p.N, p.K, p.N, dbias, 0, ws, ws_floats, stream));
        return wgrad3x3_patch(q, ws, ws_floats, stream);
    }
    if (ws && d.pad == 0 && p.N <= 32 && !no_dma() && !(bf3_mode() & 8)) {
        ConvWgradProb q = p;
        q.colsum = nullptr;
        if (wgrad_dma_ok(q)) {
            if (dbias) HAB_TRY(colsum(dy, p.N, p.K, p.N, dbias, 0, ws, ws_floats, stream));
            if ((q.M % 288 == 0) || (cdiv(q.M, 288) * 288 < cdiv(q.M, 256) * 256)) return igemm_dma_wgrad_launch<3, 3, 1>(q, ws, ws_floats, 1024, stream);
            return igemm_dma_wgrad_launch<2, 4, 1>(q, ws, ws_floats, 1024, stream);
        }
    }
    return run_igemm(p, ws, ws_floats, stream);
}
int obs_conv_wgrad(const ConvDesc& d, const ObsView& obs, const float* dy, float* dw_oihw, float* dbias, float* ws,
                   size_t ws_floats, hipStream_t stream) {
    ObsConvWgradProb p;
    HAB_TRY(build(p, d, obs, dy, dw_oihw, dbias));
    if ((bf3_mode() & 2) && p.quad && p.K > 4096) {
        const int rc = obs_wgrad_bf3_launch(p, ws, ws_floats, stream);
        if (rc != 1) return rc;
    }
    return run_igemm(p, ws, ws_floats, stream);
}
static bool dense_on() { return (bf3_mode() & 1024) && (bf3_mode() & 1); }
static bool dense_worth(long long M, long long N, long long K) {
    if (bf3_mode() & 2048) return true;
    static const long long min_flop = (long long)hab_env_int("HAB_DENSE_MIN_MFLOP", 4000) * 1000000LL;
    return 2 * M * N * K >= min_flop;
}
int linear_fwd(const float* x, int ldx, const float* w, int ldw, const float* bias, float* y, int ldy, int M, int N, int K,
               int relu, int accumulate, float* ws, size_t ws_floats, hipStream_t stream) {
    LinearFwdProb p;
    HAB_TRY(build(p, x, ldx, w, ldw, bias, y, ldy, M, N, K, relu, accumulate));
    if (dense_on() && dense_worth(M, N, K)) {
        DenseArgs g{};
        g.M = M; g.N = N; g.K = K; g.a = x; g.lda = ldx; g.b = w; g.ldb = ldw; g.c = y; g.ldc = ldy; g.bias = bias; g.relu = relu;
        g.accumulate = accumulate; g.partial = ws;
        g.a_bytes = ((long long)(M - 1) * ldx + K) * 4; g.b_bytes = ((long long)(N - 1) * ldw + K) * 4;
        if (dense_bf3_ok(g, false, false)) {
            g.nsplit = ws ? dense_bf3_splits(g, ws_floats) : 1;
            HAB_TRY((dense_bf3_launch<0, 0>(g, stream)));
            if (g.nsplit > 1) {
                igemm_splitk_reduce<LinearFwdProb>(p, ws, g.nsplit, stream);
                HAB_LAUNCH_CHECK();
            }
            return HAB_OK;
        }
    }
    return run_igemm(p, ws, ws_floats, stream);
}
int linear_dgrad(const float* dy, int lddy, const float* w, int ldw, const float* mask, int ldmask, int mask_cols, float* dx,
                 int lddx, int M, int Nin, int Kout, int accumulate, float* ws, size_t ws_floats, hipStream_t stream) {
    LinearDgradProb p;
    HAB_TRY(build(p, dy, lddy, w, ldw, mask, ldmask, mask_cols, dx, lddx, M, Nin, Kout, accumulate));
    if (dense_on() && !mask && dense_worth(M, Nin, Kout)) {
        DenseArgs g{};
        g.M = M; g.N = Nin; g.K = Kout; g.a = dy; g.lda = lddy; g.b = w; g.ldb = ldw; g.c = dx; g.ldc = lddx; g.accumulate = accumulate;
        g.partial = ws;
        g.a_bytes = ((long long)(M - 1) * lddy + Kout) * 4; g.b_bytes = ((long long)(Kout - 1) * ldw + Nin) * 4;
        if (dense_bf3_ok(g, false, true)) {
            g.nsplit = ws ? dense_bf3_splits(g, ws_floats) : 1;
            HAB_TRY((dense_bf3_launch<0, 1>(g, stream)));
            if (g.nsplit > 1) {
                igemm_splitk_reduce<LinearDgradProb>(p, ws, g.nsplit, stream);
                HAB_LAUNCH_CHECK();
            }
            return HAB_OK;
        }
    }
    return run_igemm(p, ws, ws_floats, stream);
}
int linear_wgrad(const float* dy, int lddy, const float* x, int ldx, float* dw, int lddw, int Mrows, int Nout, int Kin,
                 int perm_c, int perm_hw, int accumulate, float* ws, size_t ws_floats, hipStream_t stream) {
    LinearWgradProb p;
    HAB_TRY(build(p, dy, lddy, x, ldx, dw, lddw, Mrows, Nout, Kin, perm_c, perm_hw, accumulate));
    if (dense_on() && dense_worth(Nout, Kin, Mrows)) {
        DenseArgs g{};
        g.M = Nout; g.N = Kin; g.K = Mrows; g.a = dy; g.lda = lddy; g.b = x; g.ldb = ldx; g.c = dw; g.ldc = lddw; g.accumulate = accumulate;
        g.perm_c = perm_c; g.perm_hw = perm_hw; g.partial = ws;
        g.a_bytes = ((long long)(Mrows - 1) * lddy + Nout) * 4; g.b_bytes = ((long long)(Mrows - 1) * ldx + Kin) * 4;
        if (dense_bf3_ok(g, true, true)) {
            g.nsplit = ws ? dense_bf3_splits(g, ws_floats) : 1;
            HAB_TRY((dense_bf3_launch<1, 1>(g, stream)));
            if (g.nsplit > 1) {
                igemm_splitk_reduce<LinearWgradProb>(p, ws, g.nsplit, stream);
                HAB_LAUNCH_CHECK();
// ... 21 lines not shown
        }
        if (m < m_end) s0 += a[(size_t)m * lda + n];
    }
    sm[threadIdx.x] = s0 + s1;
    __syncthreads();
    if (r == 0 && n < N) {
        float t = 0.f;
        for (int q = 0; q < rl; ++q) t += sm[q * cw + c];
        partial[(size_t)blockIdx.y * N + n] = t;
    }
}
__global__ void __launch_bounds__(256) colsum_stage2(const float* __restrict__ partial, int nblocks, int N, float* __restrict__ out,
                                                     int accumulate) {
    __shared__ float sm[4][64];
    const int c = threadIdx.x & 63, r = threadIdx.x >> 6;
    const int n = blockIdx.x * 64 + c;
    float s0 = 0.f, s1 = 0.f, s2 = 0.f, s3 = 0.f;
    if (n < N) {
        int b = r;
        for (; b + 12 < nblocks; b += 16) {
            s0 += partial[(size_t)b * N + n];
            s1 += partial[(size_t)(b + 4) * N + n];
            s2 += partial[(size_t)(b + 8) * N + n];
            s3 += partial[(size_t)(b + 12) * N + n];
        }
        for (; b < nblocks; b += 4) s0 += partial[(size_t)b * N + n];
    }
    const float s = (s0 + s1) + (s2 + s3);
    sm[r][c] = s;
    __syncthreads();
    if (r == 0 && n < N) {
        const float t = (sm[0][c] + sm[1][c]) + (sm[2][c] + sm[3][c]);
        out[n] = accumulate ? out[n] + t : t;
    }
}

int colsum(const float* a, int lda, int M, int N, float* out, int accumulate, float* ws, size_t ws_floats, hipStream_t stream) {
    if (M <= 0 || N <= 0 || !a || !out || !ws) return HAB_ERR_ARG;
    const int cw = N < 64 ? N : 64;
    const int colblocks = cdiv(N, cw);
    int chunks = cdiv(1024, colblocks);
    if (chunks > cdiv(M, 16)) chunks = cdiv(M, 16);
    while (chunks > 1 && (size_t)chunks * N > ws_floats) chunks >>= 1;
    if ((size_t)chunks * N > ws_floats) return HAB_ERR_ARG;
    const int rpb = cdiv(M, chunks);
    chunks = cdiv(M, rpb);
    colsum_stage1<<<dim3(colblocks, chunks), 256, 0, stream>>>(a, lda, M, N, rpb, ws);
    HAB_LAUNCH_CHECK();
    colsum_stage2<<<cdiv(N, 64), 256, 0, stream>>>(ws, chunks, N, out, accumulate);
    HAB_LAUNCH_CHECK();
    return HAB_OK;
}

__global__ void repack_conv_kernel(const float* __restrict__ w, float* __restrict__ wf, float* __restrict__ wd, int Cout,
                                   int Cin, int KH, int KW, int cpad) {
    const int total = Cout * cpad * KH * KW;
    for (int e = blockIdx.x * blockDim.x + threadIdx.x; e < total; e += gridDim.x * blockDim.x) {
        const int ci = e % cpad;
        int t = e / cpad;
        const int kw = t % KW; t /= KW;
        const int kh = t % KH;
        const int co = t / KH;
        const float v = (ci < Cin) ? w[(((size_t)co * Cin + ci) * KH + kh) * KW + kw] : 0.f;
        if (wf) wf[e] = v;
        if (wd && ci < Cin) wd[(((size_t)ci * KH + kh) * KW + kw) * Cout + co] = v;
    }
}

int repack_conv(const float* w_oihw, float* wf, float* wd, int Cout, int Cin, int KH, int KW, int cpad, hipStream_t stream) {
    if (!w_oihw || Cout <= 0 || Cin <= 0 || KH <= 0 || KW <= 0 || cpad < Cin) return HAB_ERR_ARG;
    if (wd && cpad != Cin) return HAB_ERR_UNSUPPORTED;
    const int total = Cout * cpad * KH * KW;
    repack_conv_kernel<<<min(1024, cdiv(total, 256)), 256, 0, stream>>>(w_oihw, wf, wd, Cout, Cin, KH, KW, cpad);
    HAB_LAUNCH_CHECK();
    return HAB_OK;
}

__global__ void repack_flatten_kernel(const float* __restrict__ w, float* __restrict__ wp, int N, int C, int HW) {
    const size_t total = (size_t)N * C * HW;
    for (size_t e = (size_t)blockIdx.x * blockDim.x + threadIdx.x; e < total; e += (size_t)gridDim.x * blockDim.x) {
        const int c = (int)(e % C);
        const size_t t = e / C;
        const int hw = (int)(t % HW);
        const size_t n = t / HW;
        wp[e] = w[(n * C + c) * HW + hw];
    }
}
int repack_flatten(const float* w, float* wp, int N, int C, int HW, hipStream_t stream) {
    if (!w || !wp || N <= 0 || C <= 0 || HW <= 0) return HAB_ERR_ARG;
    const size_t total = (size_t)N * C * HW;
    repack_flatten_kernel<<<(int)fmin(4096.0, (double)cdivl((long long)total, 256)), 256, 0, stream>>>(w, wp, N, C, HW);
    HAB_LAUNCH_CHECK();
    return HAB_OK;
}

__global__ void transpose_kernel(const float* __restrict__ w, float* __restrict__ wt, int R, int C) {
    __shared__ float tile[32][33];
    const int bx = blockIdx.x * 32, by = blockIdx.y * 32;
    for (int j = threadIdx.y; j < 32; j += blockDim.y) {
        const int r = by + j, c = bx + threadIdx.x;
        tile[j][threadIdx.x] = (r < R && c < C) ? w[(size_t)r * C + c] : 0.f;
    }
    __syncthreads();
    for (int j = threadIdx.y; j < 32; j += blockDim.y) {
        const int c = bx + j, r = by + threadIdx.x;
        if (c < C && r < R) wt[(size_t)c * R + r] = tile[threadIdx.x][j];
    }
}
__global__ void pad_rows_kernel(const float* __restrict__ w, float* __restrict__ wp, int R, int C, int ld) {
    const long long total = (long long)R * ld;
    for (long long e = (long long)blockIdx.x * blockDim.x + threadIdx.x; e < total; e += (long long)gridDim.x * blockDim.x) {
        const int c = (int)(e % ld);
        const long long r = e / ld;
        wp[e] = c < C ? w[r * C + c] : 0.f;
    }
}
int pad_rows(const float* w, float* wp, int R, int C, int ld, hipStream_t stream) {
    if (!w || !wp || R <= 0 || C <= 0 || ld < C) return HAB_ERR_ARG;
    const long long total = (long long)R * ld;
    pad_rows_kernel<<<(int)fmin(2048.0, (double)cdivl(total, 256)), 256, 0, stream>>>(w, wp, R, C, ld);
    HAB_LAUNCH_CHECK();
    return HAB_OK;
}
int transpose2d(const float* w, float* wt, int R, int C, hipStream_t stream) {
    if (!w || !wt || R <= 0 || C <= 0) return HAB_ERR_ARG;
    transpose_kernel<<<dim3(cdiv(C, 32), cdiv(R, 32)), dim3(32, 8), 0, stream>>>(w, wt, R, C);
    HAB_LAUNCH_CHECK();
    return HAB_OK;
}

}

using namespace hab;

static ConvDesc mk(int B, int H, int W, int C, int Cout, int KH, int KW, int stride, int pad) {
    ConvDesc d;
    d.B = B; d.H = H; d.W = W; d.C = C; d.Cout = Cout; d.KH = KH; d.KW = KW; d.stride = stride; d.pad = pad;
    return d;
}
static ObsView mkobs(const uint8_t* rgb, const float* depth, const int* rows, int H, int W) {
    ObsView o;
    o.rgb = rgb; o.depth = depth; o.rows = rows; o.H = H; o.W = W; o.C = (rgb ? 3 : 0) + (depth ? 1 : 0);
    return o;
}

extern "C" int hab_conv2d_fwd(const float* x, const float* w_fwd, const float* bias, float* y, int B, int H, int W, int C,
                              int Cout, int KH, int KW, int stride, int pad, int relu, float* ws, size_t ws_floats,
                              hipStream_t stream) {
    if (!x || !w_fwd || !y) return HAB_ERR_ARG;
    return conv_fwd(mk(B, H, W, C, Cout, KH, KW, stride, pad), x, w_fwd, bias, y, relu, ws, ws_floats, stream);
}
extern "C" int hab_obs_conv2d_fwd(const uint8_t* rgb, const float* depth, const int* rows, const float* w_fwd,
                                  const float* bias, float* y, int B, int H, int W, int Cout, int KH, int KW, int stride,
                                  int pad, int relu, float* ws, size_t ws_floats, hipStream_t stream) {
    if ((!rgb && !depth) || !w_fwd || !y) return HAB_ERR_ARG;
    ObsView o = mkobs(rgb, depth, rows, H, W);
    return obs_conv_fwd(mk(B, H, W, o.C, Cout, KH, KW, stride, pad), o, w_fwd, bias, y, relu, ws, ws_floats, stream);
}
extern "C" int hab_conv2d_dgrad(const float* dy, const float* w_dgrad, const float* relu_mask, const float* add, float* dx,
                                int B, int H, int W, int C, int Cout, int KH, int KW, int stride, int pad, float* ws,
                                size_t ws_floats, hipStream_t stream) {
    if (!dy || !w_dgrad || !dx) return HAB_ERR_ARG;
    return conv_dgrad(mk(B, H, W, C, Cout, KH, KW, stride, pad), dy, w_dgrad, relu_mask, add, dx, ws, ws_floats, stream);
}
extern "C" int hab_conv2d_wgrad(const float* x, const float* dy, float* dw_oihw, float* dbias, int B, int H, int W, int C, int Cout,
                                int KH, int KW, int stride, int pad, float* ws, size_t ws_floats, hipStream_t stream) {
    if (!x || !dy || !dw_oihw) return HAB_ERR_ARG;
    return conv_wgrad(mk(B, H, W, C, Cout, KH, KW, stride, pad), x, dy, dw_oihw, dbias, ws, ws_floats, stream);
}
extern "C" int hab_obs_conv2d_wgrad(const uint8_t* rgb, const float* depth, const int* rows, const float* dy, float* dw_oihw,
                                    float* dbias, int B, int H, int W, int Cout, int KH, int KW, int stride, int pad, float* ws,
                                    size_t ws_floats, hipStream_t stream) {
    if ((!rgb && !depth) || !dy || !dw_oihw) return HAB_ERR_ARG;
    ObsView o = mkobs(rgb, depth, rows, H, W);
    return obs_conv_wgrad(mk(B, H, W, o.C, Cout, KH, KW, stride, pad), o, dy, dw_oihw, dbias, ws, ws_floats, stream);
}
extern "C" int hab_linear_fwd(const float* x, int ldx, const float* w, int ldw, const float* bias, float* y, int ldy, int M,
                              int N, int K, int relu, int accumulate, float* ws, size_t ws_floats, hipStream_t stream) {
    return linear_fwd(x, ldx, w, ldw, bias, y, ldy, M, N, K, relu, accumulate, ws, ws_floats, stream);
}
extern "C" int hab_linear_dgrad(const float* dy, int lddy, const float* w, int ldw, const float* relu_mask, int ldmask,
// ... 27 lines not shown
```

### habitat-lab_amd/csrc/hab_common.h

```cpp
#pragma once
#include <stdlib.h>
#include <hip/hip_runtime.h>
#include <stdint.h>

#define HAB_OK 0
#define HAB_ERR_ARG -1
#define HAB_ERR_UNSUPPORTED -2

#define HAB_LAUNCH_CHECK()                                  \
    do {                                                    \
        hipError_t e__ = hipGetLastError();                 \
        if (e__ != hipSuccess) return (int)e__;             \
    } while (0)

#define HAB_TRY(expr)                                       \
    do {                                                    \
        int r__ = (int)(expr);                              \
        if (r__ != 0) return r__;                           \
    } while (0)

typedef float f32x4 __attribute__((ext_vector_type(4)));
typedef float f32x16 __attribute__((ext_vector_type(16)));

namespace hab {

constexpr int WAVE = 64;

inline bool hab_env_flag(const char* name) { return getenv(name) != nullptr; }
inline int hab_env_int(const char* name, int dflt) { const char* v = getenv(name); return v ? atoi(v) : dflt; }

__host__ __device__ inline int cdiv(int a, int b) { return (a + b - 1) / b; }
__host__ __device__ inline long long cdivl(long long a, long long b) { return (a + b - 1) / b; }

__device__ inline float wave_sum(float v) {
#pragma unroll
    for (int o = 32; o > 0; o >>= 1) v += __shfl_xor(v, o, 64);
    return v;
}
__device__ inline float wave_max(float v) {
#pragma unroll
    for (int o = 32; o > 0; o >>= 1) v = fmaxf(v, __shfl_xor(v, o, 64));
    return v;
}
__device__ inline float wave_min(float v) {
#pragma unroll
    for (int o = 32; o > 0; o >>= 1) v = fminf(v, __shfl_xor(v, o, 64));
    return v;
}

__device__ inline float block_sum_256(float v, float* smem4) {
    v = wave_sum(v);
    const int w = threadIdx.x >> 6;
    __syncthreads();
    if ((threadIdx.x & 63) == 0) smem4[w] = v;
    __syncthreads();
    return (smem4[0] + smem4[1]) + (smem4[2] + smem4[3]);
}

__device__ inline float sigmoidf_(float x) { return 1.0f / (1.0f + expf(-x)); }

}

namespace hab {
struct FastDiv {
    uint32_t mul, shift, d, add;
    FastDiv() : mul(0), shift(0), d(1), add(1) {}
    explicit FastDiv(int dd) {
        d = (uint32_t)dd;
        mul = 0;
        shift = 0;
        add = 1;
        if (dd <= 1) return;
// ... 21 lines not shown
```

### habitat-lab_amd/csrc/igemm.h

```cpp
#pragma once
#include <type_traits>

#include "hab_common.h"

namespace hab {

constexpr int IGEMM_BK = 32;
constexpr int IGEMM_ICPAD = 4;

template <class P, class = void>
struct ColsumB : std::false_type {};
template <class P>
struct ColsumB<P, std::void_t<decltype(P::COLSUM_B)>> : std::bool_constant<P::COLSUM_B && !P::B_RC> {};

template <class P, class = void>
struct AKv : std::integral_constant<int, 4> {};
template <class P>
struct AKv<P, std::void_t<decltype(P::A_KV)>> : std::integral_constant<int, P::A_KV> {};

template <class P, class = void>
struct EpiV4 : std::false_type {};
template <class P>
struct EpiV4<P, std::void_t<decltype(P::EPI_VEC4)>> : std::bool_constant<P::EPI_VEC4> {};

template <class P, int TM, int TN>
__device__ __forceinline__ void igemm_epilogue_v4(const P& p, const f32x16 (&acc)[TM][TN], int mbase, int nbase, int li, int hi) {
    typename P::EpiCol4 ecol[TN][4];
#pragma unroll
    for (int j = 0; j < TN; ++j)
#pragma unroll
        for (int g = 0; g < 4; ++g) ecol[j][g] = p.epi_col4(nbase + j * 32 + 8 * g + 4 * hi);
#pragma unroll
    for (int i = 0; i < TM; ++i) {
        const typename P::EpiRow erow = p.epi_row(mbase + i * 32 + li);
#pragma unroll
        for (int j = 0; j < TN; ++j) {
            typename P::EpiAux4 aux[4];
#pragma unroll
            for (int g = 0; g < 4; ++g) aux[g] = p.epi_fetch4(erow, ecol[j][g]);
#pragma unroll
            for (int g = 0; g < 4; ++g) {
                f32x4 v;
                v[0] = acc[i][j][4 * g]; v[1] = acc[i][j][4 * g + 1]; v[2] = acc[i][j][4 * g + 2]; v[3] = acc[i][j][4 * g + 3];
                p.epi_store4(erow, ecol[j][g], aux[g], v);
            }
        }
    }
}

template <class P, int TM, int TN>
__device__ __forceinline__ void igemm_partial_v4(const P& p, const f32x16 (&acc)[TM][TN], float* __restrict__ slab, int mbase, int nbase,
                                                 int li, int hi) {
    const bool vec = ((p.N & 3) == 0) && ((reinterpret_cast<uintptr_t>(slab) & 15) == 0);
#pragma unroll
    for (int i = 0; i < TM; ++i) {
        const int row = mbase + i * 32 + li;
        if (row >= p.M) continue;
#pragma unroll
        for (int j = 0; j < TN; ++j)
#pragma unroll
            for (int g = 0; g < 4; ++g) {
                const int col = nbase + j * 32 + 8 * g + 4 * hi;
                float* dst = slab + (size_t)row * p.N + col;
                if (vec && col + 3 < p.N) {
                    f32x4 v;
                    v[0] = acc[i][j][4 * g]; v[1] = acc[i][j][4 * g + 1]; v[2] = acc[i][j][4 * g + 2]; v[3] = acc[i][j][4 * g + 3];
// ... 204 lines not shown
    }
    if (split) {
#pragma unroll
        for (int i = 0; i < TM; ++i)
#pragma unroll
            for (int j = 0; j < TN; ++j) {
                const int col = n0 + (wn * TN + j) * 32 + li;
#pragma unroll
                for (int v = 0; v < 16; ++v) {
                    const int row = m0 + (wm * TM + i) * 32 + (v & 3) + 8 * (v >> 2) + 4 * hi;
                    if (row < p.M && col < p.N) partial[((size_t)kz * MP + row) * p.N + col] = acc[i][j][v];
                }
            }
        return;
    }
    typename P::EpiCol ecol[TN];
#pragma unroll
    for (int j = 0; j < TN; ++j) ecol[j] = p.epi_col(n0 + (wn * TN + j) * 32 + li);
#pragma unroll
    for (int i = 0; i < TM; ++i)
#pragma unroll
        for (int g = 0; g < 4; ++g) {
            typename P::EpiRow erow[4];
            typename P::EpiAux eaux[4][TN];
#pragma unroll
            for (int q = 0; q < 4; ++q) {
                erow[q] = p.epi_row(m0 + (wm * TM + i) * 32 + q + 8 * g + 4 * hi);
#pragma unroll
                for (int j = 0; j < TN; ++j) eaux[q][j] = p.epi_fetch(erow[q], ecol[j]);
            }
#pragma unroll
            for (int q = 0; q < 4; ++q)
#pragma unroll
                for (int j = 0; j < TN; ++j) p.epi_store(erow[q], ecol[j], eaux[q][j], acc[i][j][g * 4 + q]);
        }
}

template <class P, bool WIDE>
__global__ void __launch_bounds__(256) igemm_splitk_reduce_kernel(const P p, const float* __restrict__ partial, int splits) {
    __shared__ float red[4][64];
    int MP = p.M;
    if constexpr (ColsumB<P>::value) MP += (p.colsum != nullptr) ? 1 : 0;
    const size_t total = (size_t)MP * p.N;
    if constexpr (!WIDE) {
        for (size_t e = (size_t)blockIdx.x * 256 + threadIdx.x; e < total; e += (size_t)gridDim.x * 256) {
            float s = 0.0f;
            for (int z = 0; z < splits; ++z) s += partial[(size_t)z * total + e];
            const int m = (int)(e / p.N), n = (int)(e % p.N);
            if constexpr (ColsumB<P>::value) {
                if (m == p.M) { p.store_colsum(n, s); continue; }
            }
            p.store(m, n, s);
        }
        return;
    }
    const int tx = threadIdx.x & 63, ty = threadIdx.x >> 6;
    const int chunk = (splits + 3) >> 2;
    const int z0 = ty * chunk, z1 = min(splits, z0 + chunk);
    for (size_t e0 = (size_t)blockIdx.x * 64; e0 < total; e0 += (size_t)gridDim.x * 64) {
        const size_t e = e0 + tx;
        float s = 0.0f;
        if (e < total) {
            const float* src = partial + e;
            int z = z0;
            for (; z + 8 <= z1; z += 8) {
                float v[8];
#pragma unroll
                for (int u = 0; u < 8; ++u) v[u] = src[(size_t)(z + u) * total];
#pragma unroll
                for (int u = 0; u < 8; ++u) s += v[u];
            }
            for (; z < z1; ++z) s += src[(size_t)z * total];
        }
        red[ty][tx] = s;
        __syncthreads();
        if (ty == 0 && e < total) {
            s = (red[0][tx] + red[1][tx]) + (red[2][tx] + red[3][tx]);
            const int m = (int)(e / p.N), n = (int)(e % p.N);
            bool done = false;
            if constexpr (ColsumB<P>::value) {
                if (m == p.M) { p.store_colsum(n, s); done = true; }
            }
            if (!done) p.store(m, n, s);
        }
        __syncthreads();
    }
}

template <class P>
inline void igemm_splitk_reduce(const P& p, const float* ws, int splits, hipStream_t stream) {
    const long long total = (long long)(p.M + 1) * p.N;
    if (splits >= 16) {
        int blocks = (int)cdivl(total, 64);
        if (blocks > 8192) blocks = 8192;
        igemm_splitk_reduce_kernel<P, true><<<blocks, 256, 0, stream>>>(p, ws, splits);
    } else {
        int blocks = (int)cdivl(total, 256);
        if (blocks > 4096) blocks = 4096;
        igemm_splitk_reduce_kernel<P, false><<<blocks, 256, 0, stream>>>(p, ws, splits);
    }
}

struct IgemmPlan {
    int splits = 1;
    int k_per_split = 0;
    size_t partial_floats = 0;
};

inline IgemmPlan igemm_plan(int BM, int BN, int M, int N, int K, int target_blocks, int max_splits, size_t max_partial_floats) {
    IgemmPlan pl;
    const long long tiles = (long long)cdiv(M, BM) * cdiv(N, BN);
    int splits = 1;
    if (tiles < target_blocks) splits = (int)((target_blocks + tiles - 1) / tiles);
    const int ktiles = cdiv(K, IGEMM_BK);
    if (splits > ktiles) splits = ktiles;
    if (splits > max_splits) splits = max_splits;
    while (splits > 1 && (size_t)splits * (size_t)(M + 1) * (size_t)N > max_partial_floats) --splits;
    if (splits < 1) splits = 1;
    pl.k_per_split = cdiv(ktiles, splits) * IGEMM_BK;
    pl.splits = cdiv(K, pl.k_per_split);
    pl.partial_floats = pl.splits > 1 ? (size_t)pl.splits * (M + 1) * N : 0;
    return pl;
}

template <class P, int TM, int TN, int WM, int WN>
inline int igemm_launch(const P& p, float* ws, size_t ws_floats, int target_blocks, hipStream_t stream) {
    using Cfg = IgemmCfg<P, TM, TN, WM, WN>;
    if (p.M <= 0 || p.N <= 0 || p.K <= 0) return HAB_ERR_ARG;
    const IgemmPlan pl = igemm_plan(Cfg::BM, Cfg::BN, p.M, p.N, p.K, target_blocks, 4096, ws ? ws_floats : 0);
    auto kern = igemm_kernel<P, TM, TN, WM, WN>;
    static const hipError_t attr_err = (Cfg::LDS_BYTES > 64 * 1024) ? hipFuncSetAttribute(reinterpret_cast<const void*>(kern), hipFuncAttributeMaxDynamicSharedMemorySize, (int)Cfg::LDS_BYTES) : hipSuccess;
    if (attr_err != hipSuccess) return (int)attr_err;
    dim3 grid(cdiv(p.M, Cfg::BM) * cdiv(p.N, Cfg::BN), 1, pl.splits);
    kern<<<grid, Cfg::NT, Cfg::LDS_BYTES, stream>>>(p, pl.k_per_split, ws);
    HAB_LAUNCH_CHECK();
    if (pl.splits > 1) {
        igemm_splitk_reduce<P>(p, ws, pl.splits, stream);
        HAB_LAUNCH_CHECK();
    }
    return HAB_OK;
}

}
```

### habitat-lab_amd/csrc/obs_conv_patch.h

```cpp
#pragma once
#include <utility>

#include "igemm_bf3.h"

namespace hab {

constexpr int OCP_TH = 4;
constexpr int OCP_R = 4 * OCP_TH + 4;
constexpr int OCP_KP = 256 + 8;
constexpr int OCP_DP = 64 + 8;

constexpr int OCP_W_ELEMS = 3 * 32 * OCP_KP + 2 * 32 * OCP_DP;
__global__ void obs_patch_split_weights(const float* __restrict__ w, int N, unsigned short* __restrict__ img) {
    const int e = blockIdx.x * blockDim.x + threadIdx.x;
    if (e >= 32 * 256) return;
    const int n = e >> 8, k = e & 255, c = k & 3;
    float v = n < N ? w[(size_t)n * 256 + k] : 0.f;
    if (c < 3) v *= HAB_RCP255;
    unsigned h1, h2, h3;
    bf3_split(v, h1, h2, h3);
    img[(0 * 32 + n) * OCP_KP + k] = (unsigned short)h1;
    img[(1 * 32 + n) * OCP_KP + k] = (unsigned short)h2;
    img[(2 * 32 + n) * OCP_KP + k] = (unsigned short)h3;
    if (c == 3) {
        unsigned short* d = img + 3 * 32 * OCP_KP;
        const int kd = k >> 2;
        d[(0 * 32 + n) * OCP_DP + kd] = (unsigned short)h1;
        d[(1 * 32 + n) * OCP_DP + kd] = (unsigned short)h2;
    }
    if (k < 8) {
        img[(0 * 32 + n) * OCP_KP + 256 + k] = 0; img[(1 * 32 + n) * OCP_KP + 256 + k] = 0; img[(2 * 32 + n) * OCP_KP + 256 + k] = 0;
        unsigned short* d = img + 3 * 32 * OCP_KP;
        d[(0 * 32 + n) * OCP_DP + 64 + k] = 0; d[(1 * 32 + n) * OCP_DP + 64 + k] = 0;
    }
}

template <class F, int... Is>
__device__ __forceinline__ void ocp_static_for_impl(F& f, std::integer_sequence<int, Is...>) { (f(std::integral_constant<int, Is>()), ...); }
template <int N, class F>
__device__ __forceinline__ void ocp_static_for(F& f) { ocp_static_for_impl(f, std::make_integer_sequence<int, N>()); }

struct ObsPatchGeom {
    int W, H, Ho, Wo, tiles_per_img, ntiles;
    int units;
    int patch_elems;
};

template <int UPT>
__global__ void __launch_bounds__(512) obs_conv_patch_kernel(const ObsConvFwdProb p, const ObsPatchGeom gq, const unsigned short* __restrict__ wimg,
                                                              const int sign_schedule, const int ablate) {
    using P = ObsConvFwdProb;
    static_assert(EpiV4<P>::value, "transposed-accumulator epilogue");
    extern __shared__ __attribute__((aligned(16))) unsigned short smem16[];
    const int W = gq.W;
    const int t = threadIdx.x;
    const int lane = t & 63, wave = __builtin_amdgcn_readfirstlane(t >> 6), group = wave >> 2, gw = wave & 3, tg = t & 255;
    const int li = lane & 31, hi = lane >> 5;
    unsigned short* W12 = smem16;
    unsigned short* WD1 = W12 + 2 * 32 * OCP_KP;
    float* biasL = reinterpret_cast<float*>(WD1 + 32 * OCP_DP);
    unsigned short* P0 = WD1 + 32 * OCP_DP + 64 + group * gq.patch_elems;
    unsigned short* P1 = P0 + OCP_R * W * 4;
    unsigned short* P2 = P1 + OCP_R * W;

    for (int i = t; i < 2 * 32 * OCP_KP / 8; i += 512) reinterpret_cast<u32x4*>(W12)[i] = reinterpret_cast<const u32x4*>(wimg)[i];
    for (int i = t; i < 32 * OCP_DP / 8; i += 512) reinterpret_cast<u32x4*>(WD1)[i] = reinterpret_cast<const u32x4*>(wimg + 3 * 32 * OCP_KP)[i];
    if (t < 32) biasL[t] = (p.bias && t < p.N) ? p.bias[t] : 0.f;
    bf16x8 w3f[8][2], wd2f[4];
    {
        const unsigned short* w3 = wimg + 2 * 32 * OCP_KP + li * OCP_KP + hi * 8;
        const unsigned short* wd = wimg + 3 * 32 * OCP_KP + li * OCP_DP + hi * 8;
#pragma unroll
        for (int kh = 0; kh < 8; ++kh)
#pragma unroll
            for (int s = 0; s < 2; ++s) w3f[kh][s] = *reinterpret_cast<const bf16x8*>(w3 + kh * 32 + s * 16);
#pragma unroll
        for (int j = 0; j < 4; ++j) wd2f[j] = *reinterpret_cast<const bf16x8*>(wd + 32 * OCP_DP + j * 16);
    }

    auto tile_of = [&](int vb) {
        const int q = gq.ntiles >> 3, r = gq.ntiles & 7, xcd = vb & 7, idx = vb >> 3;
        return (xcd < r ? xcd * (q + 1) : r * (q + 1) + (xcd - r) * q) + idx;
    };

    struct Rgb12 { uint32_t d0, d1, d2; };
    Rgb12 rg[UPT];
    f32x4 dp[UPT];
// ... 134 lines not shown
    auto store_tile = [&](int tile, bool neg) {
        if ((ablate & 4) && acc[0][0] != 12345.f) return;
        const int img = tile / gq.tiles_per_img, ho = (tile - img * gq.tiles_per_img) * OCP_TH + gw;
        if (ho >= gq.Ho) return;
#pragma unroll
        for (int i = 0; i < 2; ++i) {
            const int wo = 32 * i + li;
            if (wo >= gq.Wo) continue;
            const size_t base = ((size_t)(img * gq.Ho + ho) * gq.Wo + wo) * p.N;
#pragma unroll
            for (int g = 0; g < 4; ++g) {
                const int n = 8 * g + 4 * hi;
                if (n + 3 >= p.N) continue;
                f32x4 v;
                v[0] = acc[i][4 * g]; v[1] = acc[i][4 * g + 1]; v[2] = acc[i][4 * g + 2]; v[3] = acc[i][4 * g + 3];
                if (neg) { v[0] = -v[0]; v[1] = -v[1]; v[2] = -v[2]; v[3] = -v[3]; }
                v += *reinterpret_cast<const f32x4*>(biasL + n);
                if (p.relu) { v[0] = fmaxf(v[0], 0.f); v[1] = fmaxf(v[1], 0.f); v[2] = fmaxf(v[2], 0.f); v[3] = fmaxf(v[3], 0.f); }
                if (p.y) *reinterpret_cast<f32x4*>(p.y + base + n) = v;
            }
        }
    };

    const int vstep = 2 * gridDim.x;
    const int vb0 = blockIdx.x + group * gridDim.x;
    const int n_mine = vb0 < gq.ntiles ? (gq.ntiles - vb0 + vstep - 1) / vstep : 0;
    const int n_first = (int)blockIdx.x < gq.ntiles ? (gq.ntiles - (int)blockIdx.x + vstep - 1) / vstep : 0;
    if (n_first == 0) return;
    if (n_mine > 0) { fetch_depth(tile_of(vb0)); if (group == 0) fetch_rgb(tile_of(vb0)); }
    if (group == 0) stage();
    __syncthreads();
    for (int pI = 0; pI <= 2 * n_first; ++pI) {
        if ((pI & 1) == group) {
            const int k = pI >> 1;
            if (k < n_mine) {
                if (k + 1 < n_mine) fetch_depth(tile_of(vb0 + (k + 1) * vstep));
                const int tile = tile_of(vb0 + k * vstep);
                matrix_phase((sign_schedule && (tile & 1)) ? 0x80008000u : 0u);
            }
        } else {
            const int kd = (pI - 1 - group) / 2;
            const int ks = (pI + 1 - group) / 2;
            if (ks < n_mine) {
                fetch_rgb(tile_of(vb0 + ks * vstep));
                stage();
            }
            if (pI >= 1 + group && kd < n_mine) {
                const int tile_d = tile_of(vb0 + kd * vstep);
                store_tile(tile_d, sign_schedule && (tile_d & 1));
            }
        }
        __syncthreads();
    }
}

inline int obs_conv_patch_weight_image(const float* w_packed, int N, int KH, int KW, int C, unsigned short* img, hipStream_t stream) {
    if (KH != 8 || KW != 8 || C != 4 || N > 32 || (N & 3) || !w_packed || !img || (reinterpret_cast<uintptr_t>(img) & 15)) return 1;
    obs_patch_split_weights<<<32, 256, 0, stream>>>(w_packed, N, img);
    HAB_LAUNCH_CHECK();
    return HAB_OK;
}

inline int obs_conv_patch_launch(const ObsConvFwdProb& p, float* ws, size_t ws_floats, hipStream_t stream, const unsigned short* wimg_cached = nullptr) {
    const ConvGeom& g = p.g;
    if (!p.quad || g.KH != 8 || g.KW != 8 || g.stride != 4 || g.pad != 0 || p.N > 32 || (p.N & 3) || p.K != 256 || g.W > 256 || (g.W & 3) || g.Wo > 64 ||
        g.Wo < 1 || p.M <= 0)
        return 1;
    if (!wimg_cached && (!ws || ws_floats * 4 < (size_t)OCP_W_ELEMS * 2 || (reinterpret_cast<uintptr_t>(ws) & 15))) return 1;
    if (reinterpret_cast<uintptr_t>(wimg_cached) & 15) return 1;
    ObsPatchGeom gq;
    gq.W = g.W; gq.H = g.H; gq.Ho = g.Ho; gq.Wo = g.Wo;
    gq.tiles_per_img = cdiv(g.Ho, OCP_TH);
    gq.ntiles = g.B * gq.tiles_per_img;
    gq.units = OCP_R * (g.W >> 2);
    if (cdiv(gq.units, 256) > 5) return 1;
    gq.patch_elems = OCP_R * g.W * 6 + 64;
    const size_t lds = ((size_t)2 * 32 * OCP_KP + 32 * OCP_DP + 64 + (size_t)2 * gq.patch_elems) * 2;
    if (lds > 160 * 1024) return 1;
    const unsigned short* wimg = wimg_cached;
    if (!wimg) {
        unsigned short* built = reinterpret_cast<unsigned short*>(ws);
        obs_patch_split_weights<<<32, 256, 0, stream>>>(p.w, p.N, built);
        HAB_LAUNCH_CHECK();
        wimg = built;
    }
    auto kern = obs_conv_patch_kernel<5>;
    static const hipError_t attr_err = hipFuncSetAttribute(reinterpret_cast<const void*>(kern), hipFuncAttributeMaxDynamicSharedMemorySize, 160 * 1024);
    if (attr_err != hipSuccess) return (int)attr_err;
    static const int sign_schedule = !hab_env_flag("HAB_BF3_NOSIGN");
    static const int ablate = hab_env_int("HAB_OCP_ABLATE", 0);
    const int pairs = (gq.ntiles + 1) / 2;
    const int grid = pairs < 256 ? (pairs + 7) / 8 * 8 : 256;
    kern<<<grid, 512, lds, stream>>>(p, gq, wimg, sign_schedule, ablate);
    HAB_LAUNCH_CHECK();
    return HAB_OK;
}

}
```

### habitat-lab_amd/csrc/ops.h

```cpp
#pragma once
#include "hab_common.h"

namespace hab {

struct ConvDesc {
    int B, H, W, C, Cout, KH, KW, stride, pad;
    int Creal = 0;
    int Ho() const { return (H + 2 * pad - KH) / stride + 1; }
    int Wo() const { return (W + 2 * pad - KW) / stride + 1; }
};
struct ObsView;

int conv_fwd(const ConvDesc& d, const float* x, const float* wf, const float* bias, float* y, int relu, float* ws,
             size_t ws_floats, hipStream_t stream);
int obs_conv_fwd(const ConvDesc& d, const ObsView& obs, const float* wf, const float* bias, float* y, int relu, float* ws,
                 size_t ws_floats, hipStream_t stream, const void* wimg = nullptr);
int64_t obs_conv_weight_image_floats();
int obs_conv_weight_image(const float* wf, int Cout, int KH, int KW, int C, void* img, hipStream_t stream);
int conv_dgrad(const ConvDesc& d, const float* dy, const float* wd, const float* mask, const float* add, float* dx,
               float* ws, size_t ws_floats, hipStream_t stream);
int conv_wgrad(const ConvDesc& d, const float* x, const float* dy, float* dw_oihw, float* dbias, float* ws, size_t ws_floats,
               hipStream_t stream);
int obs_conv_wgrad(const ConvDesc& d, const ObsView& obs, const float* dy, float* dw_oihw, float* dbias, float* ws,
                   size_t ws_floats, hipStream_t stream);
int linear_fwd(const float* x, int ldx, const float* w, int ldw, const float* bias, float* y, int ldy, int M, int N, int K,
               int relu, int accumulate, float* ws, size_t ws_floats, hipStream_t stream);
int linear_dgrad(const float* dy, int lddy, const float* w, int ldw, const float* mask, int ldmask, int mask_cols, float* dx,
                 int lddx, int M, int Nin, int Kout, int accumulate, float* ws, size_t ws_floats, hipStream_t stream);
int linear_wgrad(const float* dy, int lddy, const float* x, int ldx, float* dw, int lddw, int Mrows, int Nout, int Kin,
                 int perm_c, int perm_hw, int accumulate, float* ws, size_t ws_floats, hipStream_t stream);
int colsum(const float* a, int lda, int M, int N, float* out, int accumulate, float* ws, size_t ws_floats, hipStream_t stream);
int repack_conv(const float* w_oihw, float* wf, float* wd, int Cout, int Cin, int KH, int KW, int cpad, hipStream_t stream);
int repack_flatten(const float* w, float* wp, int N, int C, int HW, hipStream_t stream);
int transpose2d(const float* w, float* wt, int R, int C, hipStream_t stream);
int pad_rows(const float* w, float* wp, int R, int C, int ld, hipStream_t stream);

struct PackInfo {
    const int* select_inds;
    const int* step_offsets;
    const int* num_seqs_at_step;
    const int* frag_env;
    const int* frag_start;
    int P, F, max_len, n_envs;
};

struct RnnLayerParams {
    const float* w_ih; const float* w_hh; const float* b_ih; const float* b_hh;
    const float* w_hh_t;
    float* dw_ih; float* dw_hh; float* db_ih; float* db_hh;
    int in_dim;
    const float* w_ih_pad = nullptr;
    int w_ih_ld = 0;
};

struct RnnWork {
    float* gi;
    float* gates;
    float* hn;
    float* hprev;
    float* cprev;
    float* c;
    float* out;
    float* dgi;
    float* dgh;
};

int rnn_frag_init(const float* h0, const int* env_rows, int env_stride, const uint8_t* masks, const int* mask_rows,
                  const int* frag_env, const int* frag_start, int F, int H, float* hinit, hipStream_t stream,
                  const int* env_first = nullptr);
int rnn_seq_layer_forward(int rnn_type, int H, const RnnLayerParams& lp, const RnnWork& wk, const float* x, int ldx,
                          const float* hinit, const float* cinit, const PackInfo& pk, float* ws, size_t ws_floats,
                          hipStream_t stream);
int rnn_seq_wave_forward(int rnn_type, int H, int L, const RnnLayerParams* lp, const RnnWork* wk, const float* x, int ldx,
                         const float* const* hinit, const float* const* cinit, const PackInfo& pk, float* ws, size_t ws_floats,
                         hipStream_t stream);
int rnn_seq_wave_backward(int rnn_type, int H, int L, const RnnLayerParams* lp, const float* const* w_ih_t, const RnnWork* wk, const float* x0,
                          int ldx0, const float* dout, float* dx0, int lddx0, const float* dx_mask, int ldmask, int mask_cols,
                          const PackInfo& pk, float* scratch , float* ws, size_t ws_floats, hipStream_t stream);
int rnn_step_layer_forward(int rnn_type, int H, const RnnLayerParams& lp, const float* x, int ldx, const float* h_in, int h_in_stride,
                           const float* c_in, int c_in_stride, const uint8_t* masks, int n, float* gi_scratch, float* h_out,
                           int h_out_stride, float* c_out, int c_out_stride, float* ws, size_t ws_floats, hipStream_t stream);
int rnn_seq_layer_backward(int rnn_type, int H, const RnnLayerParams& lp, const RnnWork& wk, const float* x, int ldx,
                           const float* dout, float* dx, int lddx, const float* dx_mask, int ldmask, int mask_cols,
                           const PackInfo& pk, float* scratch , float* ws, size_t ws_floats,
                           hipStream_t stream);
int matrix_path_bits();
int rnn_tm_prepare(const uint8_t* masks, const int* rows, int B, uint8_t* frame_mask, int* iota, hipStream_t stream);
int rnn_tm_layer_forward(int rnn_type, int H, const RnnLayerParams& lp, const RnnWork& wk, const float* x, int ldx, const float* hinit,
                         const float* cinit, const uint8_t* frame_mask, int n, int T_total, int t0, int t1, float* ws, size_t ws_floats,
                         hipStream_t stream);
int rnn_tm_layer_backward(int rnn_type, int H, const RnnLayerParams& lp, const RnnWork& wk, const float* dout, float* dx, int lddx,
                          const float* dx_mask, int ldmask, int mask_cols, const uint8_t* frame_mask, const int* iota, int n, int T, int t0,
                          int t1, float* scratch, float* ws, size_t ws_floats, hipStream_t stream);
int rnn_tm_layer_param_grads(int rnn_type, int H, const RnnLayerParams& lp, const RnnWork& wk, const float* x, int ldx, int P, float* ws,
                             size_t ws_floats, hipStream_t stream);

}
```

### habitat-lab_amd/csrc/problems.h

```cpp
#pragma once
#include <math.h>

#include "hab_common.h"
#include "bf3_split.h"

namespace hab {

#define HAB_HD __host__ __device__ inline

HAB_HD f32x4 zero4() {
    f32x4 z;
    z[0] = 0.f; z[1] = 0.f; z[2] = 0.f; z[3] = 0.f;
    return z;
}
HAB_HD f32x4 ld4(const float* p) { return *reinterpret_cast<const f32x4*>(p); }

struct Raw4 { f32x4 v; int ok; };
struct KKey { int k, ok; };
HAB_HD KKey kkey(int k, int k_end) { KKey q; q.k = k; q.ok = k < k_end; return q; }
HAB_HD f32x4 sel4(const Raw4& r) { return r.ok ? r.v : zero4(); }
struct NoCtx {};
struct NoAux {};

constexpr int HAB_FAR = -(1 << 28);
// ... 863 lines not shown
        EpiRow r;
        r.ok = i < M;
        int tap, ci, kh, kw;
        g.dC.divmod(r.ok ? i : 0, tap, ci);
        g.dKW.divmod(tap, kh, kw);
        r.off = (ci * g.KH + kh) * g.KW + kw;
        r.scale = (quad && ci < 3) ? HAB_RCP255 : 1.0f;
        return r;
    }
    HAB_HD EpiAux epi_fetch(const EpiRow&, const EpiCol&) const { return EpiAux(); }
    HAB_HD void epi_store(const EpiRow& r, const EpiCol& c, const EpiAux&, float v) const {
        if (!(r.ok & c.ok)) return;
        dw[(size_t)c.n * g.C * g.KH * g.KW + r.off] = v * r.scale;
    }
    HAB_GENERIC_STORE
};

HAB_HD Raw4 row_fetch4(const float* row, int row_ok, const KKey& q, int K, int vec) {
    Raw4 r;
    if (vec) {
        r.ok = row_ok & q.ok;
        r.v = ld4(row + (q.k & -r.ok));
    } else {
        r.ok = 1;
        r.v = zero4();
        for (int e = 0; e < 4; ++e)
            if (row_ok && q.ok && q.k + e < K) r.v[e] = row[q.k + e];
    }
    return r;
}
HAB_HD Raw4 col_fetch4(const float* base, int ld, int r, int r_ok, int j, int n) {
    Raw4 q;
    if (((ld & 3) == 0) && (j + 3 < n || j >= n)) {
        q.ok = r_ok & (j < n);
        q.v = ld4(base + (((size_t)r * ld + j) & (size_t)(-(long long)q.ok)));
    } else {
        q.ok = 1;
        q.v = zero4();
        for (int e = 0; e < 4; ++e)
            if (r_ok && j + e < n) q.v[e] = base[(size_t)r * ld + j + e];
    }
    return q;
}

struct LinearFwdProb {
    static constexpr bool A_RC = true, B_RC = true;
    int M, N, K;
    const float* x; int ldx;
    const float* w; int ldw;
    const float* bias;
    float* y; int ldy;
    int relu, vec;
    int accumulate;
    HAB_NO_KCTX
    using ACtx = WRowCtx;
    using BCtx = WRowCtx;
    using ARaw = Raw4;
    using BRaw = Raw4;
    HAB_HD ACtx a_ctx(int m) const { ACtx c; c.ok = m < M; c.row = c.ok ? x + (size_t)m * ldx : x; return c; }
    using AKey = KKey;
    using BKey = KKey;
    HAB_HD AKey a_key(const KCtx&, int k, int k_end) const { return kkey(k, k_end); }
    HAB_HD BKey b_key(const KCtx&, int k, int k_end) const { return kkey(k, k_end); }
    HAB_HD ARaw a_fetch(const ACtx& c, const KCtx&, const AKey& q) const { return row_fetch4(c.row, c.ok, q, K, vec); }
    HAB_HD BCtx b_ctx(int n) const { BCtx c; c.ok = n < N; c.row = c.ok ? w + (size_t)n * ldw : w; return c; }
    HAB_HD BRaw b_fetch(const BCtx& c, const KCtx&, const BKey& q) const { return row_fetch4(c.row, c.ok, q, K, vec); }
    HAB_PLAIN_CVT
    using EpiCol = ColN;
    using EpiRow = RowBase;
    struct EpiAux { float old; };
    HAB_HD EpiCol epi_col(int n) const { EpiCol c; c.n = n; c.ok = n < N; c.bias = (bias && c.ok) ? bias[n] : 0.f; return c; }
    HAB_HD EpiRow epi_row(int m) const { EpiRow r; r.ok = m < M; r.base = (size_t)m * ldy; return r; }
    HAB_HD EpiAux epi_fetch(const EpiRow& r, const EpiCol& c) const {
        EpiAux a;
        a.old = accumulate ? y[(r.ok & c.ok) ? r.base + c.n : 0] : 0.f;
        return a;
    }
    HAB_HD void epi_store(const EpiRow& r, const EpiCol& c, const EpiAux& a, float v) const {
        if (!(r.ok & c.ok)) return;
        v += c.bias;
        v += a.old;
        if (relu) v = v > 0.f ? v : 0.f;
        y[r.base + c.n] = v;
    }
    HAB_GENERIC_STORE
};

struct LinearDgradProb {
    static constexpr bool A_RC = true, B_RC = false;
    int M, N, K;
    const float* dy; int lddy;
    const float* w; int ldw;
    const float* mask; int ldmask;
    int mask_cols;
    float* dx; int lddx;
    int vec_a;
    int accumulate;
    HAB_NO_KCTX
    using ACtx = WRowCtx;
    struct BCtx { int j; };
    using ARaw = Raw4;
    using BRaw = Raw4;
    HAB_HD ACtx a_ctx(int m) const { ACtx c; c.ok = m < M; c.row = c.ok ? dy + (size_t)m * lddy : dy; return c; }
    using AKey = KKey;
    using BKey = KKey;
    HAB_HD AKey a_key(const KCtx&, int k, int k_end) const { return kkey(k, k_end); }
// ... 78 lines not shown
```

### habitat-lab_amd/csrc/rnn.hip

```cpp
#include "ops.h"
#include "rnn_gates.h"
#include "rnn_persist.h"
#include "../../include/habitat_amd.h"

namespace hab {

constexpr int RNN_GRU = 0, RNN_LSTM = 1;

__global__ void rnn_frag_init_kernel(const float* __restrict__ h0, const int* __restrict__ env_rows, int env_stride,
                                     const uint8_t* __restrict__ masks, const int* __restrict__ mask_rows,
                                     const int* __restrict__ frag_env, const int* __restrict__ frag_start, int F, int H,
                                     float* __restrict__ hinit, const int* __restrict__ env_first) {
    const int q = blockIdx.x;
    if (q >= F) return;
    const int f = frag_start ? frag_start[q] : q;
    int e = frag_env ? frag_env[q] : q;
    if (env_first) e = env_first[e];
    const bool keep = masks[mask_rows ? mask_rows[f] : f] != 0;
    const float* src = h0 + (size_t)(env_rows ? env_rows[e] : e) * env_stride;
    for (int u = threadIdx.x; u < H; u += blockDim.x) hinit[(size_t)q * H + u] = keep ? src[u] : 0.f;
}

int rnn_frag_init(const float* h0, const int* env_rows, int env_stride, const uint8_t* masks, const int* mask_rows,
                  const int* frag_env, const int* frag_start, int F, int H, float* hinit, hipStream_t stream, const int* env_first) {
// ... 476 lines not shown
        int rmax = 0;
        for (int l = 0; l < L; ++l) {
            BwdStepArgs& g = n.l[l];
            const int s = pk.max_len - 1 - (w - (L - 1 - l));
            g.H = H; g.K = K;
            g.R = (s >= 0 && s < pk.max_len) ? pk.num_seqs_at_step[s] : 0;
            if (g.R <= 0) { g.R = 0; continue; }
            rmax = std::max(rmax, g.R);
            g.R_next = (s + 1 < pk.max_len) ? pk.num_seqs_at_step[s + 1] : 0;
            g.idx = pk.select_inds + pk.step_offsets[s];
            g.idx_next = g.R_next ? pk.select_inds + pk.step_offsets[s + 1] : g.idx;
            g.next_keep = nullptr;
            g.dout = (l == L - 1) ? dout : nullptr;
            g.w_hh_t = lp[l].w_hh_t;
            g.dh_direct = scratch + (size_t)l * 2 * pk.F * H;
            g.dc_carry = g.dh_direct + (size_t)pk.F * H;
            g.gates = wk[l].gates; g.hn = wk[l].hn; g.hprev = wk[l].hprev; g.cprev = wk[l].cprev; g.c = wk[l].c;
            g.dgi = wk[l].dgi; g.dgh = (rnn_type == RNN_GRU) ? wk[l].dgh : wk[l].dgi;
            if (l < L - 1) { g.up_dgi = wk[l + 1].dgi; g.up_w_ih_t = w_ih_t[l + 1]; }
        }
        if (rmax == 0) continue;
        const dim3 grid(cdiv(rmax, 16), H / 16, L);
        if (rnn_type == RNN_GRU) {
            if (wide) rnn_bwd_step_wave_kernel<3, 8><<<grid, 512, 0, stream>>>(n);
            else rnn_bwd_step_wave_kernel<3, 4><<<grid, 256, 0, stream>>>(n);
        } else {
            if (wide) rnn_bwd_step_wave_kernel<4, 8><<<grid, 512, 0, stream>>>(n);
            else rnn_bwd_step_wave_kernel<4, 4><<<grid, 256, 0, stream>>>(n);
        }
        HAB_LAUNCH_CHECK();
    }
    for (int l = L - 1; l >= 0; --l) {
        const float* x = l == 0 ? x0 : wk[l - 1].out;
        const int ldx = l == 0 ? ldx0 : H;
        float* dgh = (rnn_type == RNN_GRU) ? wk[l].dgh : wk[l].dgi;
        HAB_TRY(linear_wgrad(wk[l].dgi, K, x, ldx, lp[l].dw_ih, lp[l].in_dim, pk.P, K, lp[l].in_dim, 0, 0, 0, ws, ws_floats, stream));
        HAB_TRY(linear_wgrad(dgh, K, wk[l].hprev, H, lp[l].dw_hh, H, pk.P, K, H, 0, 0, 0, ws, ws_floats, stream));
        HAB_TRY(colsum(wk[l].dgi, K, pk.P, K, lp[l].db_ih, 0, ws, ws_floats, stream));
        HAB_TRY(colsum(dgh, K, pk.P, K, lp[l].db_hh, 0, ws, ws_floats, stream));
    }
    if (dx0) HAB_TRY(linear_dgrad(wk[0].dgi, K, lp[0].w_ih, lp[0].in_dim, dx_mask, ldmask, mask_cols, dx0, lddx0, pk.P, lp[0].in_dim, K, 0, ws,
                                  ws_floats, stream));
    return HAB_OK;
}

__global__ void gather_u8_kernel(const uint8_t* __restrict__ src, const int* __restrict__ rows, int n, uint8_t* __restrict__ dst) {
    const int i = blockIdx.x * blockDim.x + threadIdx.x;
    if (i < n) dst[i] = src[rows ? rows[i] : i];
}
__global__ void iota_kernel(int* __restrict__ dst, int n) {
    const int i = blockIdx.x * blockDim.x + threadIdx.x;
    if (i < n) dst[i] = i;
}
int rnn_tm_prepare(const uint8_t* masks, const int* rows, int B, uint8_t* frame_mask, int* iota, hipStream_t stream) {
    if (!masks || !frame_mask || !iota || B <= 0) return HAB_ERR_ARG;
    gather_u8_kernel<<<cdiv(B, 256), 256, 0, stream>>>(masks, rows, B, frame_mask);
    iota_kernel<<<cdiv(B, 256), 256, 0, stream>>>(iota, B);
    HAB_LAUNCH_CHECK();
    return HAB_OK;
}

static bool tm_persist_ok(int rnn_type, int H, int n, int T, const float* ws, size_t ws_floats) {
    static const bool on = hab_env_int("HAB_RNN_PERSIST", 1) != 0;
    const int G = rnn_type == RNN_GRU ? 3 : 4;
    if (!on || (matrix_path_bits() & 4096) || !ws || ws_floats < 64) return false;
    if (H != 128 && H != 256 && H != 512) return false;
    if (cdiv(n, 16) > RNNP_MAX_ROW_TILES) return false;
    if ((size_t)T * n * G * H * 4 >= ((size_t)1 << 31)) return false;
    return true;
}

int rnn_tm_layer_forward(int rnn_type, int H, const RnnLayerParams& lp, const RnnWork& wk, const float* x, int ldx, const float* hinit,
                         const float* cinit, const uint8_t* frame_mask, int n, int T_total, int t0, int t1, float* ws, size_t ws_floats,
                         hipStream_t stream) {
    const int G = rnn_type == RNN_GRU ? 3 : 4;
    const size_t f0 = (size_t)t0 * n;
    HAB_TRY(linear_fwd(x + f0 * ldx, ldx, lp.w_ih, lp.in_dim, lp.b_ih, wk.gi + f0 * G * H, G * H, (t1 - t0) * n, G * H, lp.in_dim, 0, 0, ws,
                       ws_floats, stream));
    if (tm_persist_ok(rnn_type, H, n, T_total, ws, ws_floats) && wk.gates) {
        TmPersistFwdArgs a;
        a.n = n; a.H = H; a.T = T_total; a.t0 = t0; a.t1 = t1;
        a.hinit = hinit; a.cinit = cinit; a.frame_mask = frame_mask; a.gi = wk.gi; a.w_hh = lp.w_hh; a.b_hh = lp.b_hh;
        a.gates = wk.gates; a.hn = wk.hn; a.hprev = wk.hprev; a.cprev = wk.cprev; a.c = wk.c; a.out = wk.out;
        a.counters = reinterpret_cast<rnnp_u64*>(ws);
        if (hipMemsetAsync(ws, 0, 16 * sizeof(rnnp_u64), stream) != hipSuccess) return HAB_ERR_ARG;
        const dim3 grid(H / 16, cdiv(n, 16));
        const int kch = H / 128;
        if (rnn_type == RNN_GRU) {
            if (kch == 4) rnn_tm_persist_fwd_kernel<3, 4><<<grid, 512, 0, stream>>>(a);
            else if (kch == 2) rnn_tm_persist_fwd_kernel<3, 2><<<grid, 512, 0, stream>>>(a);
            else rnn_tm_persist_fwd_kernel<3, 1><<<grid, 512, 0, stream>>>(a);
        } else {
            if (kch == 4) rnn_tm_persist_fwd_kernel<4, 4><<<grid, 512, 0, stream>>>(a);
            else if (kch == 2) rnn_tm_persist_fwd_kernel<4, 2><<<grid, 512, 0, stream>>>(a);
            else rnn_tm_persist_fwd_kernel<4, 1><<<grid, 512, 0, stream>>>(a);
        }
        HAB_LAUNCH_CHECK();
        return HAB_OK;
    }
    for (int t = t0; t < t1; ++t) {
        const size_t f = (size_t)t * n, fp = (size_t)(t - 1) * n;
        StepArgs a;
        a.R = n; a.H = H;
        if (t == 0) {
            a.hp_base = hinit; a.cp_base = cinit; a.row_mask = nullptr;
        } else {
            a.hp_base = wk.out + fp * H; a.cp_base = wk.c + fp * H; a.row_mask = frame_mask + f;
        }
        a.hp_idx = nullptr; a.hp_stride = H; a.cp_idx = nullptr; a.cp_stride = H;
        a.out_idx = nullptr;
        a.gi = wk.gi + f * G * H; a.w_hh = lp.w_hh; a.b_hh = lp.b_hh;
        a.gates = wk.gates + f * G * H; a.hn = wk.hn ? wk.hn + f * H : nullptr; a.hprev = wk.hprev + f * H;
        a.cprev = wk.cprev ? wk.cprev + f * H : nullptr; a.c = wk.c ? wk.c + f * H : nullptr;
        a.out = wk.out + f * H; a.out_stride = H; a.c_out = nullptr; a.c_out_stride = 0;
        HAB_TRY(launch_step(rnn_type, a, stream));
    }
    return HAB_OK;
}

int rnn_tm_layer_backward(int rnn_type, int H, const RnnLayerParams& lp, const RnnWork& wk, const float* dout, float* dx, int lddx,
                          const float* dx_mask, int ldmask, int mask_cols, const uint8_t* frame_mask, const int* iota, int n, int T, int t0,
                          int t1, float* scratch, float* ws, size_t ws_floats, hipStream_t stream) {
    const int G = rnn_type == RNN_GRU ? 3 : 4;
    if (H % 64) return HAB_ERR_UNSUPPORTED;
    float* dh_direct = scratch;
    float* dc_carry = scratch + (size_t)n * H;
    float* dgh = (rnn_type == RNN_GRU) ? wk.dgh : wk.dgi;
    const int K = G * H;
    const bool wide = K % 128 == 0;
    bool persisted = false;
    if (tm_persist_ok(rnn_type, H, n, T, ws, ws_floats) && dout) {
        TmPersistBwdArgs a;
        a.n = n; a.H = H; a.T = T; a.t0 = t0; a.t1 = t1;
        a.frame_mask = frame_mask; a.dout = dout; a.w_hh_t = lp.w_hh_t; a.dh_direct = dh_direct; a.dc_carry = dc_carry;
        a.gates = wk.gates; a.hn = wk.hn; a.hprev = wk.hprev; a.cprev = wk.cprev; a.c = wk.c; a.dgi = wk.dgi; a.dgh = dgh;
        a.counters = reinterpret_cast<rnnp_u64*>(ws);
        if (hipMemsetAsync(ws, 0, 16 * sizeof(rnnp_u64), stream) != hipSuccess) return HAB_ERR_ARG;
        const dim3 grid(H / 16, cdiv(n, 16));
        const int kch = H / 128;
        if (rnn_type == RNN_GRU) {
            if (kch == 4) rnn_tm_persist_bwd_kernel<3, 12><<<grid, 512, 0, stream>>>(a);
            else if (kch == 2) rnn_tm_persist_bwd_kernel<3, 6><<<grid, 512, 0, stream>>>(a);
            else rnn_tm_persist_bwd_kernel<3, 3><<<grid, 512, 0, stream>>>(a);
        } else {
            if (kch == 4) rnn_tm_persist_bwd_kernel<4, 16><<<grid, 512, 0, stream>>>(a);
            else if (kch == 2) rnn_tm_persist_bwd_kernel<4, 8><<<grid, 512, 0, stream>>>(a);
            else rnn_tm_persist_bwd_kernel<4, 4><<<grid, 512, 0, stream>>>(a);
        }
        HAB_LAUNCH_CHECK();
        persisted = true;
    }
    for (int t = t1 - 1; t >= t0 && !persisted; --t) {
        BwdStepArgs g;
        g.R = n; g.H = H; g.K = K;
        g.R_next = (t + 1 < T) ? n : 0;
        g.idx = iota + (size_t)t * n;
        g.idx_next = g.R_next ? iota + (size_t)(t + 1) * n : g.idx;
        g.next_keep = g.R_next ? frame_mask + (size_t)(t + 1) * n : nullptr;
        g.dout = dout; g.w_hh_t = lp.w_hh_t; g.dh_direct = dh_direct; g.dc_carry = dc_carry;
        g.gates = wk.gates; g.hn = wk.hn; g.hprev = wk.hprev; g.cprev = wk.cprev; g.c = wk.c;
        g.dgi = wk.dgi; g.dgh = dgh;
        const dim3 grid(cdiv(g.R, 16), H / 16);
        if (rnn_type == RNN_GRU) {
            if (wide) rnn_bwd_step_kernel<3, 8><<<grid, 512, 0, stream>>>(g);
            else rnn_bwd_step_kernel<3, 4><<<grid, 256, 0, stream>>>(g);
        } else {
            if (wide) rnn_bwd_step_kernel<4, 8><<<grid, 512, 0, stream>>>(g);
            else rnn_bwd_step_kernel<4, 4><<<grid, 256, 0, stream>>>(g);
        }
        HAB_LAUNCH_CHECK();
    }
    const size_t f0 = (size_t)t0 * n;
    if (dx) HAB_TRY(linear_dgrad(wk.dgi + f0 * G * H, G * H, lp.w_ih, lp.in_dim, dx_mask ? dx_mask + f0 * ldmask : nullptr, ldmask, mask_cols,
                                 dx + f0 * lddx, lddx, (t1 - t0) * n, lp.in_dim, G * H, 0, ws, ws_floats, stream));
    return HAB_OK;
}

int rnn_tm_layer_param_grads(int rnn_type, int H, const RnnLayerParams& lp, const RnnWork& wk, const float* x, int ldx, int P, float* ws,
                             size_t ws_floats, hipStream_t stream) {
    const int G = rnn_type == RNN_GRU ? 3 : 4;
    float* dgh = (rnn_type == RNN_GRU) ? wk.dgh : wk.dgi;
    HAB_TRY(linear_wgrad(wk.dgi, G * H, x, ldx, lp.dw_ih, lp.in_dim, P, G * H, lp.in_dim, 0, 0, 0, ws, ws_floats, stream));
    HAB_TRY(linear_wgrad(dgh, G * H, wk.hprev, H, lp.dw_hh, H, P, G * H, H, 0, 0, 0, ws, ws_floats, stream));
    HAB_TRY(colsum(wk.dgi, G * H, P, G * H, lp.db_ih, 0, ws, ws_floats, stream));
    HAB_TRY(colsum(dgh, G * H, P, G * H, lp.db_hh, 0, ws, ws_floats, stream));
    return HAB_OK;
}

}
```

Baseline: 61750 env-steps/s.

## Cut per-step launches: batch repacks, precompute conv3 planes, preallocate RNN counters

Several launch-overhead reductions land together. Weight repacks are batched into one table-driven launch. The conv3 bf3 weight planes are precomputed at repack time instead of split on every forward call. The goal columns are fused into the FC epilogue. The iota buffer is cached, and the per-call counter memsets for the persistent RNN kernels are replaced by one memset over preallocated counters. The last chunk's RNN forward and first chunk's backward also run on the main stream, dropping some cross-stream event syncs. These changes shrink kernel launch and sync counts, at the cost of more bookkeeping and risk of stale cached state (e.g. iota_valid, precomputed planes) if weights change without a repack.

Result: no change. 62730 env-steps/s, median of 2 (+1.6%).

```diff
diff --git a/habitat-lab_amd/csrc/conv_patch_bf3.h b/habitat-lab_amd/csrc/conv_patch_bf3.h
--- a/habitat-lab_amd/csrc/conv_patch_bf3.h
+++ b/habitat-lab_amd/csrc/conv_patch_bf3.h
@@ -33,14 +33,16 @@
 inline size_t cpb_w_elems(const ConvFwdProb& p) { return (size_t)p.N * p.K; }
 inline size_t cpb_w_elems(const ConvDgradProb& p) { return (size_t)p.N * p.Kfull; }
 
+__device__ __forceinline__ void cpb_split_one(float v, size_t e, size_t n, unsigned short* __restrict__ planes) {
+    unsigned h1, h2, h3;
+    bf3_split(v, h1, h2, h3);
+    planes[e] = (unsigned short)h1; planes[n + e] = (unsigned short)h2; planes[2 * n + e] = (unsigned short)h3;
+    bf3_split(-v, h1, h2, h3);
+    planes[3 * n + e] = (unsigned short)h1; planes[4 * n + e] = (unsigned short)h2; planes[5 * n + e] = (unsigned short)h3;
+}
 __global__ void cpb_split_weights(const float* __restrict__ w, size_t n, unsigned short* __restrict__ planes) {
     const size_t e = (size_t)blockIdx.x * blockDim.x + threadIdx.x;
-    if (e >= n) return;
-    unsigned h1, h2, h3;
-    bf3_split(w[e], h1, h2, h3);
-    planes[e] = (unsigned short)h1; planes[n + e] = (unsigned short)h2; planes[2 * n + e] = (unsigned short)h3;
-    bf3_split(-w[e], h1, h2, h3);
-    planes[3 * n + e] = (unsigned short)h1; planes[4 * n + e] = (unsigned short)h2; planes[5 * n + e] = (unsigned short)h3;
+    if (e < n) cpb_split_one(w[e], e, n, planes);
 }
 
 constexpr int CPB_DRAW_SLOTS = 64;
@@ -290,8 +292,15 @@
     }
 }
 
+inline int64_t cpb_planes_floats(size_t n) { return (int64_t)(n * 12 + 3) / 4; }
+inline int cpb_split_weights_launch(const float* w, size_t n, void* planes, hipStream_t stream) {
+    cpb_split_weights<<<(unsigned)((n + 255) / 256), 256, 0, stream>>>(w, n, reinterpret_cast<unsigned short*>(planes));
+    HAB_LAUNCH_CHECK();
+    return HAB_OK;
+}
+
 template <class P, int TW, int WM, int WN, int TN, int BT>
-inline int conv_patch_bf3_launch(const P& p, PatchGeom gq, float* ws, size_t ws_floats, hipStream_t stream) {
+inline int conv_patch_bf3_launch(const P& p, PatchGeom gq, float* ws, size_t ws_floats, hipStream_t stream, const void* prepared = nullptr) {
     using Cfg = ConvPatchCfg<P, TW, WM, WN, TN, BT>;
     gq.TH = Cfg::TH;
     gq.tiles_per_img = cdiv(gq.Ho, Cfg::TH);
@@ -310,7 +319,9 @@
     if (grid > ntiles) grid = (ntiles + 7) / 8 * 8;
     constexpr int pre_min = 131072;
     const size_t wn_elems = cpb_w_elems(p);
-    const bool pre = ws && ((reinterpret_cast<uintptr_t>(ws) & 15) == 0) && ws_floats * 4 >= wn_elems * 12 && p.M >= pre_min && (wn_elems % 4 == 0);
+    const bool room = prepared ? (reinterpret_cast<uintptr_t>(prepared) & 15) == 0
+                               : ws && ((reinterpret_cast<uintptr_t>(ws) & 15) == 0) && ws_floats * 4 >= wn_elems * 12;
+    const bool pre = room && p.M >= pre_min && (wn_elems % 4 == 0);
     hipError_t e = hipSuccess;
     static const bool dyn_on = !hab_env_flag("HAB_NO_DYN_TILES");
     unsigned* ctr = nullptr;
@@ -325,9 +336,8 @@
         auto kern = conv_patch_bf3_kernel<P, TW, WM, WN, TN, BT, true>;
         static const hipError_t attr_err = (Cfg::LDS_BYTES > 64 * 1024) ? hipFuncSetAttribute(reinterpret_cast<const void*>(kern), hipFuncAttributeMaxDynamicSharedMemorySize, (int)Cfg::LDS_BYTES) : hipSuccess;
         if (attr_err != hipSuccess) return (int)attr_err;
-        unsigned short* planes = reinterpret_cast<unsigned short*>(ws);
-        cpb_split_weights<<<(unsigned)((wn_elems + 255) / 256), 256, 0, stream>>>(p.w, wn_elems, planes);
-        HAB_LAUNCH_CHECK();
+        const unsigned short* planes = reinterpret_cast<const unsigned short*>(prepared ? prepared : ws);
+        if (!prepared) HAB_TRY(cpb_split_weights_launch(p.w, wn_elems, ws, stream));
         kern<<<grid, Cfg::NT, Cfg::LDS_BYTES, stream>>>(p, gq, sign_schedule, planes, wn_elems, ctr);
     } else {
         auto kern = conv_patch_bf3_kernel<P, TW, WM, WN, TN, BT, false>;
@@ -340,11 +350,11 @@
 }
 
 template <class P>
-inline int conv_patch_bf3_dispatch(const P& p, const PatchGeom& gq, float* ws, size_t ws_floats, hipStream_t stream) {
+inline int conv_patch_bf3_dispatch(const P& p, const PatchGeom& gq, float* ws, size_t ws_floats, hipStream_t stream, const void* prepared = nullptr) {
     if (gq.KH != 3 || gq.KW != 3 || gq.Ci % CPB_CC != 0 || (p.N & 31) || gq.Wo > 32 || gq.Wo < 5 || p.M % (gq.Ho * gq.Wo) != 0) return 1;
     if (p.N != 32) return 1;
-    if (gq.Wo > 16) return conv_patch_bf3_launch<P, 32, 4, 1, 1, 3>(p, gq, ws, ws_floats, stream);
-    if (gq.Wo > 8) return conv_patch_bf3_launch<P, 16, 4, 1, 1, 3>(p, gq, ws, ws_floats, stream);
+    if (gq.Wo > 16) return conv_patch_bf3_launch<P, 32, 4, 1, 1, 3>(p, gq, ws, ws_floats, stream, prepared);
+    if (gq.Wo > 8) return conv_patch_bf3_launch<P, 16, 4, 1, 1, 3>(p, gq, ws, ws_floats, stream, prepared);
     return 1;
 }
 
diff --git a/habitat-lab_amd/csrc/engine.h b/habitat-lab_amd/csrc/engine.h
--- a/habitat-lab_amd/csrc/engine.h
+++ b/habitat-lab_amd/csrc/engine.h
@@ -49,6 +49,7 @@
     int64_t w_gsaved = -1;
     std::vector<int> i_wih, i_whh, i_bih, i_bhh;
     int64_t pk_c1f = -1, pk_c2f = -1, pk_c2d = -1, pk_c3f = -1, pk_c3d = -1, pk_fc = -1;
+    int64_t pk_c3pl = -1;
     int64_t pk_c1img = -1;
     std::vector<int64_t> pk_whht;
     std::vector<int64_t> pk_wiht;
@@ -63,6 +64,9 @@
     hipStream_t s2 = nullptr;
     std::vector<hipEvent_t> evs;
     int64_t w_ws2 = -1, ws2_floats = 0, w_fmask = -1, w_iota = -1;
+    int iota_valid = 0;
+    int64_t w_ctr = -1;
+    int ctr_chunks = 0;
     RnnForm form;
     struct ResNetPlan* rn = nullptr;
     int save_acts = 1;
@@ -105,7 +109,7 @@
 void add_tail_params(hab_policy* e);
 void pack_tail(hab_policy* e, Arena& pk);
 void plan_tail_workspace(hab_policy* e, Arena& wk, int64_t ws_floats);
-int repack_tail(hab_policy* e, hipStream_t s);
+int repack_tail(hab_policy* e, hab::RepackBatch& rb);
 int build_resnet(hab_policy* e);
 void destroy_resnet(hab_policy* e);
 int resnet_repack(hab_policy* e, hipStream_t s);
diff --git a/habitat-lab_amd/csrc/engine.hip b/habitat-lab_amd/csrc/engine.hip
--- a/habitat-lab_amd/csrc/engine.hip
+++ b/habitat-lab_amd/csrc/engine.hip
@@ -40,11 +40,11 @@
     for (int l = 0; l < e->L; ++l) e->pk_wiht.push_back(l == 0 ? -1 : pk.take(GH * e->d.hidden));
     e->pk_wih0 = pk.take(GH * e->rnn_ld);
 }
-int repack_tail(hab_policy* e, hipStream_t s) {
+int repack_tail(hab_policy* e, RepackBatch& rb) {
     const int H = e->d.hidden;
-    for (int l = 0; l < e->L; ++l) HAB_TRY(transpose2d(e->p(e->i_whh[l]), e->PK + e->pk_whht[l], e->G_ * H, H, s));
-    for (int l = 1; l < e->L; ++l) HAB_TRY(transpose2d(e->p(e->i_wih[l]), e->PK + e->pk_wiht[l], e->G_ * H, H, s));
-    return pad_rows(e->p(e->i_wih[0]), e->PK + e->pk_wih0, e->G_ * H, e->rnn_in, e->rnn_ld, s);
+    for (int l = 0; l < e->L; ++l) HAB_TRY(rb.transpose(e->p(e->i_whh[l]), e->PK + e->pk_whht[l], e->G_ * H, H));
+    for (int l = 1; l < e->L; ++l) HAB_TRY(rb.transpose(e->p(e->i_wih[l]), e->PK + e->pk_wiht[l], e->G_ * H, H));
+    return rb.pad_rows(e->p(e->i_wih[0]), e->PK + e->pk_wih0, e->G_ * H, e->rnn_in, e->rnn_ld);
 }
 void plan_tail_workspace(hab_policy* e, Arena& wk, int64_t ws_floats) {
     const hab_policy_desc& d = e->d;
@@ -108,6 +108,7 @@
     e->pk_c2d = pk.take(64 * 16 * 32);
     e->pk_c3f = pk.take(32 * 9 * 64);
     e->pk_c3d = pk.take(32 * 9 * 64);
+    e->pk_c3pl = pk.take(conv_fwd_planes_floats(32, 3, 3, 64));
     e->pk_fc = pk.take((int64_t)H * std::max(e->fc_in, 4));
     pack_tail(e, pk);
     e->packed_floats = pk.used;
@@ -204,22 +205,22 @@
     if (work_floats < e->work_floats) return HAB_ERR_ARG;
     if ((((uintptr_t)params | (uintptr_t)grads | (uintptr_t)packed | (uintptr_t)work) & 255) != 0) return HAB_ERR_ARG;
     e->P = params; e->G = grads; e->PK = packed; e->WK = work; e->work_bound = work_floats;
+    e->iota_valid = 0;
     return HAB_OK;
 }
 
 extern "C" int hab_policy_repack(hab_policy* e, hipStream_t stream) {
     if (!e || !e->P) return HAB_ERR_ARG;
     if (e->rn) return resnet_repack(e, stream);
-    if (e->Cin == 0) return repack_tail(e, stream);
-    HAB_TRY(repack_conv(e->p(e->i_c1w), e->PK + e->pk_c1f, nullptr, 32, e->Cin, 8, 8, e->Cin, stream));
-    if (e->pk_c1img >= 0) {
-        const int rc = obs_conv_weight_image(e->PK + e->pk_c1f, 32, 8, 8, e->Cin, e->PK + e->pk_c1img, stream);
-        if (rc != HAB_OK) return rc == 1 ? HAB_ERR_UNSUPPORTED : rc;
-    }
-    HAB_TRY(repack_conv(e->p(e->i_c2w), e->PK + e->pk_c2f, e->PK + e->pk_c2d, 64, 32, 4, 4, 32, stream));
-    HAB_TRY(repack_conv(e->p(e->i_c3w), e->PK + e->pk_c3f, e->PK + e->pk_c3d, 32, 64, 3, 3, 64, stream));
-    HAB_TRY(repack_flatten(e->p(e->i_fcw), e->PK + e->pk_fc, e->d.hidden, 32, e->fc_in / 32, stream));
-    return repack_tail(e, stream);
+    RepackBatch rb(stream);
+    if (e->Cin > 0) {
+        HAB_TRY(rb.conv(e->p(e->i_c1w), e->PK + e->pk_c1f, nullptr, 32, e->Cin, 8, 8, e->Cin, e->pk_c1img >= 0 ? e->PK + e->pk_c1img : nullptr));
+        HAB_TRY(rb.conv(e->p(e->i_c2w), e->PK + e->pk_c2f, e->PK + e->pk_c2d, 64, 32, 4, 4, 32));
+        HAB_TRY(rb.conv(e->p(e->i_c3w), e->PK + e->pk_c3f, e->PK + e->pk_c3d, 32, 64, 3, 3, 64, nullptr, e->PK + e->pk_c3pl));
+        HAB_TRY(rb.flatten(e->p(e->i_fcw), e->PK + e->pk_fc, e->d.hidden, 32, e->fc_in / 32));
+    }
+    HAB_TRY(repack_tail(e, rb));
+    return rb.flush();
 }
 
 extern "C" int hab_policy_probe_enable(hab_policy* e, int tag) {
@@ -295,10 +296,15 @@
     { Probe pr(e, HAB_PROBE_CONV2_FWD, s);
       HAB_TRY(conv_fwd(c2, a1, e->PK + e->pk_c2f, e->p(e->i_c2b), a2, 1, ws, e->ws_floats, s)); }
     { Probe pr(e, HAB_PROBE_CONV3_FWD, s);
-      HAB_TRY(conv_fwd(c3, a2, e->PK + e->pk_c3f, e->p(e->i_c3b), a3, 0, ws, e->ws_floats, s)); }
+      HAB_TRY(conv_fwd(c3, a2, e->PK + e->pk_c3f, e->p(e->i_c3b), a3, 0, ws, e->ws_floats, s, e->PK + e->pk_c3pl)); }
+    int goal_done = 0;
+    ExtraCols xc;
+    xc.src = obs->goal; xc.rows = rws; xc.dst = rin + H; xc.src_ld = e->d.goal_dim; xc.dst_ld = e->rnn_ld; xc.ncols = e->d.goal_dim;
+    xc.npad = e->rnn_ld - e->rnn_in; xc.B = nB; xc.done = &goal_done;
     { Probe pr(e, HAB_PROBE_FC_FWD, s);
-      HAB_TRY(linear_fwd(a3, e->fc_in, e->PK + e->pk_fc, e->fc_in, e->p(e->i_fcb), rin, e->rnn_ld, nB, H, e->fc_in, 1, 0, ws, e->ws_floats, s)); }
-    if (e->d.goal_dim > 0)
+      HAB_TRY(linear_fwd(a3, e->fc_in, e->PK + e->pk_fc, e->fc_in, e->p(e->i_fcb), rin, e->rnn_ld, nB, H, e->fc_in, 1, 0, ws, e->ws_floats, s,
+                         e->d.goal_dim > 0 ? &xc : nullptr)); }
+    if (e->d.goal_dim > 0 && !goal_done)
         HAB_TRY(gather_cols(obs->goal, e->d.goal_dim, rws, rin, e->rnn_ld, H, e->d.goal_dim, e->rnn_ld - e->rnn_in, nB, s));
     return HAB_OK;
 }
@@ -327,6 +333,8 @@
     e->w_ws2 = wk.take(e->ws2_floats);
     e->w_fmask = wk.take((B + 3) / 4 + 64);
     e->w_iota = wk.take(B + 64);
+    e->ctr_chunks = rnn_form_cfg(e, (int)B, 1, true).chunks;
+    e->w_ctr = wk.take((int64_t)2 * e->L * e->ctr_chunks * RNN_TM_COUNTER_FLOATS);
 }
 static int tm_setup(hab_policy* e, int nev) {
     if (!e->s2) {
@@ -347,6 +355,15 @@
     hipError_t err = hipEventRecord(e->evs[ev], from);
     if (err != hipSuccess) return (int)err;
     err = hipStreamWaitEvent(to, e->evs[ev], 0);
+    return err == hipSuccess ? HAB_OK : (int)err;
+}
+
+static float* tm_counters(hab_policy* e, int bwd, int l, int c) {
+    return e->WK + e->w_ctr + ((int64_t)(bwd * e->L + l) * e->ctr_chunks + c) * RNN_TM_COUNTER_FLOATS;
+}
+static int tm_zero_counters(hab_policy* e, int bwd, hipStream_t s) {
+    if (e->form.chunks > e->ctr_chunks) return HAB_ERR_ARG;
+    const hipError_t err = hipMemsetAsync(tm_counters(e, bwd, 0, 0), 0, (size_t)e->L * e->ctr_chunks * RNN_TM_COUNTER_FLOATS * sizeof(float), s);
     return err == hipSuccess ? HAB_OK : (int)err;
 }
 
@@ -469,24 +486,27 @@
                           const uint8_t* masks, int B, int n, hipStream_t stream) {
     float* W = e->WK;
     const int H = e->d.hidden, L = e->L, NC = e->form.chunks, T = B / n, Tc = (T + NC - 1) / NC;
+    const int last = (T + Tc - 1) / Tc - 1;
     HAB_TRY(tm_setup(e, 2 * NC + 4));
     hipStream_t sB = e->s2;
     uint8_t* fmask = reinterpret_cast<uint8_t*>(W + e->w_fmask);
-    HAB_TRY(rnn_tm_prepare(masks, rows, B, fmask, reinterpret_cast<int*>(W + e->w_iota), stream));
+    HAB_TRY(tm_zero_counters(e, 0, stream));
+    HAB_TRY(rnn_tm_prepare(masks, rows, B, fmask, reinterpret_cast<int*>(W + e->w_iota), &e->iota_valid, stream));
     HAB_TRY(rnn_state_init(e, hidden0, hidden_env_stride, rows, masks, nullptr, nullptr, n, nullptr, stream));
-    for (int c = 0; c < NC; ++c) {
+    for (int c = 0; c <= last; ++c) {
         const int t0 = c * Tc, t1 = std::min(T, t0 + Tc);
-        if (t0 >= t1) break;
         HAB_TRY(encoder_forward(e, obs, masks, rows, B, stream, t0 * n, (t1 - t0) * n));
-        HAB_TRY(tm_order(e, c, stream, sB));
+        hipStream_t sr = c < last ? sB : stream;
+        if (c < last) HAB_TRY(tm_order(e, c, stream, sB));
+        else if (c > 0) HAB_TRY(tm_order(e, NC, sB, stream));
         for (int l = 0; l < L; ++l) {
-            Probe pr(e, HAB_PROBE_RNN_FWD, sB);
+            Probe pr(e, HAB_PROBE_RNN_FWD, sr);
             HAB_TRY(rnn_tm_layer_forward(e->d.rnn_type, H, layer_params(e, l), layer_work(e, l), layer_x(e, l), layer_ld(e, l),
                                          W + e->w_hinit + (size_t)l * n * H, W + e->w_cinit + (size_t)l * n * H, fmask, n, T, t0, t1,
-                                         W + e->w_ws2, e->ws2_floats, sB));
+                                         W + (c < last ? e->w_ws2 : e->w_ws), e->ws_floats, tm_counters(e, 0, l, c), sr));
         }
     }
-    return tm_order(e, NC, sB, stream);
+    return HAB_OK;
 }
 static int rnn_packed_forward(hab_policy* e, const int* rows, const float* hidden0, int hidden_env_stride, const uint8_t* masks,
                               const hab_pack_info* pack, int n, hipStream_t stream) {
@@ -607,23 +627,23 @@
 static int rnn_tm_backward(hab_policy* e, int B, hipStream_t stream) {
     float* W = e->WK;
     const int H = e->d.hidden, L = e->L, n = e->last_n, T = B / n, NC = e->form.chunks, Tc = (T + NC - 1) / NC;
+    const int last = (T + Tc - 1) / Tc - 1;
     hipStream_t sB = e->s2;
     const uint8_t* fmask = reinterpret_cast<const uint8_t*>(W + e->w_fmask);
     const int* iota = reinterpret_cast<const int*>(W + e->w_iota);
-    HAB_TRY(tm_order(e, NC + 1, stream, sB));
-    for (int c = NC - 1; c >= 0; --c) {
+    for (int c = last; c >= 0; --c) {
         const int t0 = c * Tc, t1 = std::min(T, t0 + Tc);
-        if (t0 >= t1) continue;
+        hipStream_t sr = c == last ? stream : sB;
         for (int l = L - 1; l >= 0; --l) {
-            Probe pr(e, HAB_PROBE_RNN_BWD, sB);
+            Probe pr(e, HAB_PROBE_RNN_BWD, sr);
             HAB_TRY(rnn_tm_layer_backward(e->d.rnn_type, H, layer_params(e, l), layer_work(e, l), layer_dout(e, l), layer_dx(e, l), layer_ld(e, l),
                                           l == 0 ? layer_x(e, 0) : nullptr, layer_ld(e, l), H, fmask, iota, n, T, t0, t1,
-                                          W + e->w_scratch + (size_t)l * 2 * n * H, W + e->w_ws2, e->ws2_floats, sB));
+                                          W + e->w_scratch + (size_t)l * 2 * n * H, W + (c == last ? e->w_ws : e->w_ws2), e->ws_floats,
+                                          tm_counters(e, 1, l, c), sr));
         }
-        if (!e->rn) {
-            HAB_TRY(tm_order(e, NC + 2 + c, sB, stream));
-            HAB_TRY(cnn_dgrad(e, (int64_t)t0 * n, (t1 - t0) * n, stream));
-        }
+        if (c == last) HAB_TRY(tm_order(e, NC + 2 + c, stream, sB));
+        else if (!e->rn) HAB_TRY(tm_order(e, NC + 2 + c, sB, stream));
+        if (!e->rn) HAB_TRY(cnn_dgrad(e, (int64_t)t0 * n, (t1 - t0) * n, stream));
     }
     for (int l = L - 1; l >= 0; --l)
         HAB_TRY(rnn_tm_layer_param_grads(e->d.rnn_type, H, layer_params(e, l), layer_work(e, l), layer_x(e, l), layer_ld(e, l), B, W + e->w_ws2,
@@ -666,6 +686,11 @@
     e->cur_stream = stream;
     e->comm_first = -1;
     const float* feats = W + e->w_out[L - 1];
+    const int NC = e->form.chunks;
+    if (NC > 0 && (e->xg_feat || e->xg_perc)) return HAB_ERR_UNSUPPORTED;
+    hipStream_t hs = NC > 0 ? e->s2 : stream;
+    float* hws = NC > 0 ? W + e->w_ws2 : ws;
+    if (NC > 0) HAB_TRY(tm_zero_counters(e, 1, stream));
     if (e->d.action_dist == HAB_DIST_GAUSSIAN) {
         const int K = e->head_K;
         GaussHeadsBwdArgs gb;
@@ -673,29 +698,27 @@
         gb.actions = reinterpret_cast<const float*>(actions); gb.rows = rows; gb.saved = W + e->w_gsaved;
         gb.w = e->p(e->i_aw); gb.w_critic = e->p(e->i_cw); gb.dfeat = W + e->w_dfeat; gb.dz = W + e->w_dzv; gb.dv_out = W + e->w_dv;
         HAB_TRY(gauss_heads_backward(gb, stream));
-        HAB_TRY(linear_wgrad(W + e->w_dzv, 8, feats, H, e->g(e->i_aw), H, B, K, H, 0, 0, 0, ws, e->ws_floats, stream));
-        HAB_TRY(colsum(W + e->w_dzv, 8, B, K, e->g(e->i_ab), 0, ws, e->ws_floats, stream));
-        if (e->i_astd >= 0) HAB_TRY(colsum(W + e->w_dzv + A, 8, B, A, e->g(e->i_astd), 0, ws, e->ws_floats, stream));
-        HAB_TRY(linear_wgrad(W + e->w_dv, 1, feats, H, e->g(e->i_cw), H, B, 1, H, 0, 0, 0, ws, e->ws_floats, stream));
-        HAB_TRY(colsum(W + e->w_dv, 1, B, 1, e->g(e->i_cb), 0, ws, e->ws_floats, stream));
+        if (NC > 0) HAB_TRY(tm_order(e, NC + 1, stream, hs));
+        HAB_TRY(linear_wgrad(W + e->w_dzv, 8, feats, H, e->g(e->i_aw), H, B, K, H, 0, 0, 0, hws, e->ws_floats, hs));
+        HAB_TRY(colsum(W + e->w_dzv, 8, B, K, e->g(e->i_ab), 0, hws, e->ws_floats, hs));
+        if (e->i_astd >= 0) HAB_TRY(colsum(W + e->w_dzv + A, 8, B, A, e->g(e->i_astd), 0, hws, e->ws_floats, hs));
+        HAB_TRY(linear_wgrad(W + e->w_dv, 1, feats, H, e->g(e->i_cw), H, B, 1, H, 0, 0, 0, hws, e->ws_floats, hs));
+        HAB_TRY(colsum(W + e->w_dv, 1, B, 1, e->g(e->i_cb), 0, hws, e->ws_floats, hs));
     } else {
     HeadsBwdArgs hb;
         hb.B = B; hb.H = H; hb.A = A; hb.d_value = d_value; hb.d_logp = d_log_prob; hb.d_entropy = d_entropy;
         hb.actions = actions; hb.rows = rows; hb.probs = W + e->w_probs; hb.logits_n = W + e->w_logitsn;
         hb.w_actor = e->p(e->i_aw); hb.w_critic = e->p(e->i_cw); hb.dfeat = W + e->w_dfeat; hb.dzv = W + e->w_dzv; hb.dv_out = W + e->w_dv;
         HAB_TRY(heads_backward(hb, stream));
-        HAB_TRY(linear_wgrad(W + e->w_dzv, 8, feats, H, e->g(e->i_aw), H, B, A, H, 0, 0, 0, ws, e->ws_floats, stream));
-        HAB_TRY(linear_wgrad(W + e->w_dv, 1, feats, H, e->g(e->i_cw), H, B, 1, H, 0, 0, 0, ws, e->ws_floats, stream));
-        HAB_TRY(colsum(W + e->w_dzv, 8, B, A, e->g(e->i_ab), 0, ws, e->ws_floats, stream));
-        HAB_TRY(colsum(W + e->w_dv, 1, B, 1, e->g(e->i_cb), 0, ws, e->ws_floats, stream));
-    }
-    const int NC = e->form.chunks;
-    if (e->xg_feat || e->xg_perc) {
-        if (NC > 0) return HAB_ERR_UNSUPPORTED;
-        if (e->xg_feat) {
-            add_rows_kernel<<<(int)std::min<long long>(1024, cdivl((long long)B * H, 256)), 256, 0, stream>>>(W + e->w_dfeat, e->xg_feat, (long long)B * H);
-            HAB_LAUNCH_CHECK();
-        }
+        if (NC > 0) HAB_TRY(tm_order(e, NC + 1, stream, hs));
+        HAB_TRY(linear_wgrad(W + e->w_dzv, 8, feats, H, e->g(e->i_aw), H, B, A, H, 0, 0, 0, hws, e->ws_floats, hs));
+        HAB_TRY(linear_wgrad(W + e->w_dv, 1, feats, H, e->g(e->i_cw), H, B, 1, H, 0, 0, 0, hws, e->ws_floats, hs));
+        HAB_TRY(colsum(W + e->w_dzv, 8, B, A, e->g(e->i_ab), 0, hws, e->ws_floats, hs));
+        HAB_TRY(colsum(W + e->w_dv, 1, B, 1, e->g(e->i_cb), 0, hws, e->ws_floats, hs));
+    }
+    if (e->xg_feat) {
+        add_rows_kernel<<<(int)std::min<long long>(1024, cdivl((long long)B * H, 256)), 256, 0, stream>>>(W + e->w_dfeat, e->xg_feat, (long long)B * H);
+        HAB_LAUNCH_CHECK();
     }
     if (NC > 0) {
         HAB_TRY(rnn_tm_backward(e, B, stream));
diff --git a/habitat-lab_amd/csrc/engine_resnet.hip b/habitat-lab_amd/csrc/engine_resnet.hip
--- a/habitat-lab_amd/csrc/engine_resnet.hip
+++ b/habitat-lab_amd/csrc/engine_resnet.hip
@@ -314,7 +314,9 @@
         HAB_TRY(planes(r->comp));
         HAB_TRY(repack_flatten(e->p(r->i_fcw), e->PK + r->pk_fc, e->d.hidden, r->comp_c, r->comp_hw, s));
     }
-    return repack_tail(e, s);
+    RepackBatch rb(s);
+    HAB_TRY(repack_tail(e, rb));
+    return rb.flush();
 }
 
 static int fill_embed_slots(hab_policy* e, const hab_obs* obs, EmbedSlot* sl, bool grads) {
diff --git a/habitat-lab_amd/csrc/gemm_ops.hip b/habitat-lab_amd/csrc/gemm_ops.hip
--- a/habitat-lab_amd/csrc/gemm_ops.hip
+++ b/habitat-lab_amd/csrc/gemm_ops.hip
@@ -113,8 +113,9 @@
     }
 }
 
+int64_t conv_fwd_planes_floats(int Cout, int KH, int KW, int C) { return cpb_planes_floats((size_t)Cout * KH * KW * C); }
 int conv_fwd(const ConvDesc& d, const float* x, const float* wf, const float* bias, float* y, int relu, float* ws,
-             size_t ws_floats, hipStream_t stream) {
+             size_t ws_floats, hipStream_t stream, const void* planes) {
     ConvFwdProb p;
     HAB_TRY(build(p, d, x, wf, bias, y, relu));
     if ((bf3_mode() & 256) && (bf3_mode() & 1)) {
@@ -125,15 +126,12 @@
         PatchGeom gq{};
         gq.in = x; gq.Hi = d.H; gq.Wi = d.W; gq.Ci = d.C; gq.Ho = p.g.Ho; gq.Wo = p.g.Wo; gq.KH = 3; gq.KW = 3;
         gq.off_h = -d.pad; gq.off_w = -d.pad; gq.flip = 0;
-        const int rc = conv_patch_bf3_dispatch(p, gq, ws, ws_floats, stream);
+        const int rc = conv_patch_bf3_dispatch(p, gq, ws, ws_floats, stream, planes);
         if (rc != 1) return rc;
     }
     return run_igemm(p, ws, ws_floats, stream);
 }
 int64_t obs_conv_weight_image_floats() { return ((int64_t)OCP_W_ELEMS + 1) / 2 + 4; }
-int obs_conv_weight_image(const float* wf, int Cout, int KH, int KW, int C, void* img, hipStream_t stream) {
-    return obs_conv_patch_weight_image(wf, Cout, KH, KW, C, reinterpret_cast<unsigned short*>(img), stream);
-}
 int obs_conv_fwd(const ConvDesc& d, const ObsView& obs, const float* wf, const float* bias, float* y, int relu, float* ws,
                  size_t ws_floats, hipStream_t stream, const void* wimg) {
     ObsConvFwdProb p;
@@ -248,9 +246,13 @@
     return 2 * M * N * K >= min_flop;
 }
 int linear_fwd(const float* x, int ldx, const float* w, int ldw, const float* bias, float* y, int ldy, int M, int N, int K,
-               int relu, int accumulate, float* ws, size_t ws_floats, hipStream_t stream) {
+               int relu, int accumulate, float* ws, size_t ws_floats, hipStream_t stream, const ExtraCols* xc) {
     LinearFwdProb p;
     HAB_TRY(build(p, x, ldx, w, ldw, bias, y, ldy, M, N, K, relu, accumulate));
+    if (xc) {
+        if (!xc->src || !xc->dst || !xc->done || xc->B != M || xc->ncols <= 0 || xc->npad < 0) return HAB_ERR_ARG;
+        p.xc = *xc;
+    }
     if (dense_on() && dense_worth(M, N, K)) {
         DenseArgs g{};
         g.M = M; g.N = N; g.K = K; g.a = x; g.lda = ldx; g.b = w; g.ldb = ldw; g.c = y; g.ldc = ldy; g.bias = bias; g.relu = relu;
@@ -378,10 +380,11 @@
     return HAB_OK;
 }
 
-__global__ void repack_conv_kernel(const float* __restrict__ w, float* __restrict__ wf, float* __restrict__ wd, int Cout,
-                                   int Cin, int KH, int KW, int cpad) {
+__device__ __forceinline__ void repack_conv_body(const float* __restrict__ w, float* __restrict__ wf, float* __restrict__ wd, int Cout, int Cin,
+                                                 int KH, int KW, int cpad, unsigned short* __restrict__ img, unsigned short* __restrict__ planes,
+                                                 int bid, int nblk) {
     const int total = Cout * cpad * KH * KW;
-    for (int e = blockIdx.x * blockDim.x + threadIdx.x; e < total; e += gridDim.x * blockDim.x) {
+    for (int e = bid * 256 + threadIdx.x; e < total; e += nblk * 256) {
         const int ci = e % cpad;
         int t = e / cpad;
         const int kw = t % KW; t /= KW;
@@ -390,7 +393,13 @@
         const float v = (ci < Cin) ? w[(((size_t)co * Cin + ci) * KH + kh) * KW + kw] : 0.f;
         if (wf) wf[e] = v;
         if (wd && ci < Cin) wd[(((size_t)ci * KH + kh) * KW + kw) * Cout + co] = v;
-    }
+        if (img) obs_patch_split_one(v, e >> 8, e & 255, img);
+        if (planes) cpb_split_one(v, (size_t)e, (size_t)total, planes);
+    }
+}
+__global__ void __launch_bounds__(256) repack_conv_kernel(const float* __restrict__ w, float* __restrict__ wf, float* __restrict__ wd, int Cout,
+                                                          int Cin, int KH, int KW, int cpad) {
+    repack_conv_body(w, wf, wd, Cout, Cin, KH, KW, cpad, nullptr, nullptr, blockIdx.x, gridDim.x);
 }
 
 int repack_conv(const float* w_oihw, float* wf, float* wd, int Cout, int Cin, int KH, int KW, int cpad, hipStream_t stream) {
@@ -402,9 +411,9 @@
     return HAB_OK;
 }
 
-__global__ void repack_flatten_kernel(const float* __restrict__ w, float* __restrict__ wp, int N, int C, int HW) {
+__device__ __forceinline__ void repack_flatten_body(const float* __restrict__ w, float* __restrict__ wp, int N, int C, int HW, int bid, int nblk) {
     const size_t total = (size_t)N * C * HW;
-    for (size_t e = (size_t)blockIdx.x * blockDim.x + threadIdx.x; e < total; e += (size_t)gridDim.x * blockDim.x) {
+    for (size_t e = (size_t)bid * 256 + threadIdx.x; e < total; e += (size_t)nblk * 256) {
         const int c = (int)(e % C);
         const size_t t = e / C;
         const int hw = (int)(t % HW);
@@ -412,6 +421,9 @@
         wp[e] = w[(n * C + c) * HW + hw];
     }
 }
+__global__ void __launch_bounds__(256) repack_flatten_kernel(const float* __restrict__ w, float* __restrict__ wp, int N, int C, int HW) {
+    repack_flatten_body(w, wp, N, C, HW, blockIdx.x, gridDim.x);
+}
 int repack_flatten(const float* w, float* wp, int N, int C, int HW, hipStream_t stream) {
     if (!w || !wp || N <= 0 || C <= 0 || HW <= 0) return HAB_ERR_ARG;
     const size_t total = (size_t)N * C * HW;
@@ -420,26 +432,33 @@
     return HAB_OK;
 }
 
-__global__ void transpose_kernel(const float* __restrict__ w, float* __restrict__ wt, int R, int C) {
+__device__ __forceinline__ void transpose_body(const float* __restrict__ w, float* __restrict__ wt, int R, int C, float (*tile)[33], int bx, int by) {
+    const int tx = threadIdx.x & 31, ty = threadIdx.x >> 5;
+    bx *= 32; by *= 32;
+    for (int j = ty; j < 32; j += 8) {
+        const int r = by + j, c = bx + tx;
+        tile[j][tx] = (r < R && c < C) ? w[(size_t)r * C + c] : 0.f;
+    }
+    __syncthreads();
+    for (int j = ty; j < 32; j += 8) {
+        const int c = bx + j, r = by + tx;
+        if (c < C && r < R) wt[(size_t)c * R + r] = tile[tx][j];
+    }
+}
+__global__ void __launch_bounds__(256) transpose_kernel(const float* __restrict__ w, float* __restrict__ wt, int R, int C) {
     __shared__ float tile[32][33];
-    const int bx = blockIdx.x * 32, by = blockIdx.y * 32;
-    for (int j = threadIdx.y; j < 32; j += blockDim.y) {
-        const int r = by + j, c = bx + threadIdx.x;
-        tile[j][threadIdx.x] = (r < R && c < C) ? w[(size_t)r * C + c] : 0.f;
-    }
-    __syncthreads();
-    for (int j = threadIdx.y; j < 32; j += blockDim.y) {
-        const int c = bx + j, r = by + threadIdx.x;
-        if (c < C && r < R) wt[(size_t)c * R + r] = tile[threadIdx.x][j];
-    }
-}
-__global__ void pad_rows_kernel(const float* __restrict__ w, float* __restrict__ wp, int R, int C, int ld) {
+    transpose_body(w, wt, R, C, tile, blockIdx.x, blockIdx.y);
+}
+__device__ __forceinline__ void pad_rows_body(const float* __restrict__ w, float* __restrict__ wp, int R, int C, int ld, int bid, int nblk) {
     const long long total = (long long)R * ld;
-    for (long long e = (long long)blockIdx.x * blockDim.x + threadIdx.x; e < total; e += (long long)gridDim.x * blockDim.x) {
+    for (long long e = (long long)bid * 256 + threadIdx.x; e < total; e += (long long)nblk * 256) {
         const int c = (int)(e % ld);
         const long long r = e / ld;
         wp[e] = c < C ? w[r * C + c] : 0.f;
     }
+}
+__global__ void __launch_bounds__(256) pad_rows_kernel(const float* __restrict__ w, float* __restrict__ wp, int R, int C, int ld) {
+    pad_rows_body(w, wp, R, C, ld, blockIdx.x, gridDim.x);
 }
 int pad_rows(const float* w, float* wp, int R, int C, int ld, hipStream_t stream) {
     if (!w || !wp || R <= 0 || C <= 0 || ld < C) return HAB_ERR_ARG;
@@ -450,9 +469,74 @@
 }
 int transpose2d(const float* w, float* wt, int R, int C, hipStream_t stream) {
     if (!w || !wt || R <= 0 || C <= 0) return HAB_ERR_ARG;
-    transpose_kernel<<<dim3(cdiv(C, 32), cdiv(R, 32)), dim3(32, 8), 0, stream>>>(w, wt, R, C);
+    transpose_kernel<<<dim3(cdiv(C, 32), cdiv(R, 32)), 256, 0, stream>>>(w, wt, R, C);
     HAB_LAUNCH_CHECK();
     return HAB_OK;
+}
+
+__global__ void __launch_bounds__(256) repack_table_kernel(const RepackTable t) {
+    __shared__ float tile[32][33];
+    int s = 0;
+    while (s + 1 < t.n && (int)blockIdx.x >= t.seg[s + 1].block0) ++s;
+    const RepackSeg& g = t.seg[s];
+    const int bid = blockIdx.x - g.block0;
+    switch (g.op) {
+        case RepackSeg::CONV:
+            repack_conv_body(g.src, g.dst, g.dst2, g.a, g.b, g.c, g.d, g.e, reinterpret_cast<unsigned short*>(g.img),
+                             reinterpret_cast<unsigned short*>(g.planes), bid, g.nblocks);
+            break;
+        case RepackSeg::FLATTEN: repack_flatten_body(g.src, g.dst, g.a, g.b, g.c, bid, g.nblocks); break;
+        case RepackSeg::TRANSPOSE: transpose_body(g.src, g.dst, g.a, g.b, tile, bid % g.c, bid / g.c); break;
+        default: pad_rows_body(g.src, g.dst, g.a, g.b, g.c, bid, g.nblocks); break;
+    }
+}
+int RepackBatch::add(const RepackSeg& g) {
+    if (g.nblocks <= 0) return HAB_ERR_ARG;
+    if (t.n == REPACK_MAX_SEGS) HAB_TRY(flush());
+    RepackSeg& d = t.seg[t.n++];
+    d = g;
+    d.block0 = blocks;
+    blocks += g.nblocks;
+    return HAB_OK;
+}
+int RepackBatch::flush() {
+    if (t.n == 0) return HAB_OK;
+    repack_table_kernel<<<blocks, 256, 0, stream>>>(t);
+    t.n = 0; blocks = 0;
+    HAB_LAUNCH_CHECK();
+    return HAB_OK;
+}
+int RepackBatch::conv(const float* w_oihw, float* wf, float* wd, int Cout, int Cin, int KH, int KW, int cpad, void* img, void* planes) {
+    if (!w_oihw || Cout <= 0 || Cin <= 0 || KH <= 0 || KW <= 0 || cpad < Cin) return HAB_ERR_ARG;
+    if (wd && cpad != Cin) return HAB_ERR_UNSUPPORTED;
+    if (img && (Cout != 32 || KH != 8 || KW != 8 || cpad != 4 || (reinterpret_cast<uintptr_t>(img) & 15))) return HAB_ERR_UNSUPPORTED;
+    if (planes && (reinterpret_cast<uintptr_t>(planes) & 15)) return HAB_ERR_ARG;
+    RepackSeg g;
+    g.op = RepackSeg::CONV; g.src = w_oihw; g.dst = wf; g.dst2 = wd; g.img = img; g.planes = planes;
+    g.a = Cout; g.b = Cin; g.c = KH; g.d = KW; g.e = cpad;
+    g.nblocks = min(1024, cdiv(Cout * cpad * KH * KW, 256));
+    return add(g);
+}
+int RepackBatch::flatten(const float* w, float* wp, int N, int C, int HW) {
+    if (!w || !wp || N <= 0 || C <= 0 || HW <= 0) return HAB_ERR_ARG;
+    RepackSeg g;
+    g.op = RepackSeg::FLATTEN; g.src = w; g.dst = wp; g.a = N; g.b = C; g.c = HW;
+    g.nblocks = (int)fmin(4096.0, (double)cdivl((long long)N * C * HW, 256));
+    return add(g);
+}
+int RepackBatch::transpose(const float* w, float* wt, int R, int C) {
+    if (!w || !wt || R <= 0 || C <= 0) return HAB_ERR_ARG;
+    RepackSeg g;
+    g.op = RepackSeg::TRANSPOSE; g.src = w; g.dst = wt; g.a = R; g.b = C; g.c = cdiv(C, 32);
+    g.nblocks = cdiv(C, 32) * cdiv(R, 32);
+    return add(g);
+}
+int RepackBatch::pad_rows(const float* w, float* wp, int R, int C, int ld) {
+    if (!w || !wp || R <= 0 || C <= 0 || ld < C) return HAB_ERR_ARG;
+    RepackSeg g;
+    g.op = RepackSeg::PAD_ROWS; g.src = w; g.dst = wp; g.a = R; g.b = C; g.c = ld;
+    g.nblocks = (int)fmin(2048.0, (double)cdivl((long long)R * ld, 256));
+    return add(g);
 }
 
 }
diff --git a/habitat-lab_amd/csrc/hab_common.h b/habitat-lab_amd/csrc/hab_common.h
--- a/habitat-lab_amd/csrc/hab_common.h
+++ b/habitat-lab_amd/csrc/hab_common.h
@@ -18,6 +18,21 @@
         int r__ = (int)(expr);                              \
         if (r__ != 0) return r__;                           \
     } while (0)
+
+struct ExtraCols {
+    const float* src = nullptr; const int* rows = nullptr; float* dst = nullptr;
+    int src_ld = 0, dst_ld = 0, ncols = 0, npad = 0, B = 0;
+    int* done = nullptr;
+    __host__ __device__ inline void write(size_t first, size_t stride) const {
+        if (!src) return;
+        const int per = ncols + npad;
+        const size_t total = (size_t)B * per;
+        for (size_t e = first; e < total; e += stride) {
+            const int f = (int)(e / per), c = (int)(e % per);
+            dst[(size_t)f * dst_ld + c] = (c < ncols) ? src[(size_t)(rows ? rows[f] : f) * src_ld + c] : 0.f;
+        }
+    }
+};
 
 typedef float f32x4 __attribute__((ext_vector_type(4)));
 typedef float f32x16 __attribute__((ext_vector_type(16)));
diff --git a/habitat-lab_amd/csrc/igemm.h b/habitat-lab_amd/csrc/igemm.h
--- a/habitat-lab_amd/csrc/igemm.h
+++ b/habitat-lab_amd/csrc/igemm.h
@@ -12,6 +12,11 @@
 struct ColsumB : std::false_type {};
 template <class P>
 struct ColsumB<P, std::void_t<decltype(P::COLSUM_B)>> : std::bool_constant<P::COLSUM_B && !P::B_RC> {};
+
+template <class P, class = void>
+struct HasExtraCols : std::false_type {};
+template <class P>
+struct HasExtraCols<P, std::void_t<decltype(P::EXTRA_COLS)>> : std::bool_constant<P::EXTRA_COLS> {};
 
 template <class P, class = void>
 struct AKv : std::integral_constant<int, 4> {};
@@ -322,6 +327,7 @@
             }
             p.store(m, n, s);
         }
+        if constexpr (HasExtraCols<P>::value) p.xc.write((size_t)blockIdx.x * 256 + threadIdx.x, (size_t)gridDim.x * 256);
         return;
     }
     const int tx = threadIdx.x & 63, ty = threadIdx.x >> 6;
@@ -355,6 +361,7 @@
         }
         __syncthreads();
     }
+    if constexpr (HasExtraCols<P>::value) p.xc.write((size_t)blockIdx.x * 256 + threadIdx.x, (size_t)gridDim.x * 256);
 }
 
 template <class P>
@@ -368,6 +375,9 @@
         int blocks = (int)cdivl(total, 256);
         if (blocks > 4096) blocks = 4096;
         igemm_splitk_reduce_kernel<P, false><<<blocks, 256, 0, stream>>>(p, ws, splits);
+    }
+    if constexpr (HasExtraCols<P>::value) {
+        if (p.xc.src && p.xc.done) *p.xc.done = 1;
     }
 }
 
diff --git a/habitat-lab_amd/csrc/obs_conv_patch.h b/habitat-lab_amd/csrc/obs_conv_patch.h
--- a/habitat-lab_amd/csrc/obs_conv_patch.h
+++ b/habitat-lab_amd/csrc/obs_conv_patch.h
@@ -11,11 +11,8 @@
 constexpr int OCP_DP = 64 + 8;
 
 constexpr int OCP_W_ELEMS = 3 * 32 * OCP_KP + 2 * 32 * OCP_DP;
-__global__ void obs_patch_split_weights(const float* __restrict__ w, int N, unsigned short* __restrict__ img) {
-    const int e = blockIdx.x * blockDim.x + threadIdx.x;
-    if (e >= 32 * 256) return;
-    const int n = e >> 8, k = e & 255, c = k & 3;
-    float v = n < N ? w[(size_t)n * 256 + k] : 0.f;
+__device__ __forceinline__ void obs_patch_split_one(float v, int n, int k, unsigned short* __restrict__ img) {
+    const int c = k & 3;
     if (c < 3) v *= HAB_RCP255;
     unsigned h1, h2, h3;
     bf3_split(v, h1, h2, h3);
@@ -33,6 +30,12 @@
         unsigned short* d = img + 3 * 32 * OCP_KP;
         d[(0 * 32 + n) * OCP_DP + 64 + k] = 0; d[(1 * 32 + n) * OCP_DP + 64 + k] = 0;
     }
+}
+__global__ void obs_patch_split_weights(const float* __restrict__ w, int N, unsigned short* __restrict__ img) {
+    const int e = blockIdx.x * blockDim.x + threadIdx.x;
+    if (e >= 32 * 256) return;
+    const int n = e >> 8, k = e & 255;
+    obs_patch_split_one(n < N ? w[(size_t)n * 256 + k] : 0.f, n, k, img);
 }
 
 template <class F, int... Is>
@@ -273,13 +276,6 @@
         }
         __syncthreads();
     }
-}
-
-inline int obs_conv_patch_weight_image(const float* w_packed, int N, int KH, int KW, int C, unsigned short* img, hipStream_t stream) {
-    if (KH != 8 || KW != 8 || C != 4 || N > 32 || (N & 3) || !w_packed || !img || (reinterpret_cast<uintptr_t>(img) & 15)) return 1;
-    obs_patch_split_weights<<<32, 256, 0, stream>>>(w_packed, N, img);
-    HAB_LAUNCH_CHECK();
-    return HAB_OK;
 }
 
 inline int obs_conv_patch_launch(const ObsConvFwdProb& p, float* ws, size_t ws_floats, hipStream_t stream, const unsigned short* wimg_cached = nullptr) {
diff --git a/habitat-lab_amd/csrc/ops.h b/habitat-lab_amd/csrc/ops.h
--- a/habitat-lab_amd/csrc/ops.h
+++ b/habitat-lab_amd/csrc/ops.h
@@ -12,11 +12,11 @@
 struct ObsView;
 
 int conv_fwd(const ConvDesc& d, const float* x, const float* wf, const float* bias, float* y, int relu, float* ws,
-             size_t ws_floats, hipStream_t stream);
+             size_t ws_floats, hipStream_t stream, const void* planes = nullptr);
+int64_t conv_fwd_planes_floats(int Cout, int KH, int KW, int C);
 int obs_conv_fwd(const ConvDesc& d, const ObsView& obs, const float* wf, const float* bias, float* y, int relu, float* ws,
                  size_t ws_floats, hipStream_t stream, const void* wimg = nullptr);
 int64_t obs_conv_weight_image_floats();
-int obs_conv_weight_image(const float* wf, int Cout, int KH, int KW, int C, void* img, hipStream_t stream);
 int conv_dgrad(const ConvDesc& d, const float* dy, const float* wd, const float* mask, const float* add, float* dx,
                float* ws, size_t ws_floats, hipStream_t stream);
 int conv_wgrad(const ConvDesc& d, const float* x, const float* dy, float* dw_oihw, float* dbias, float* ws, size_t ws_floats,
@@ -24,7 +24,7 @@
 int obs_conv_wgrad(const ConvDesc& d, const ObsView& obs, const float* dy, float* dw_oihw, float* dbias, float* ws,
                    size_t ws_floats, hipStream_t stream);
 int linear_fwd(const float* x, int ldx, const float* w, int ldw, const float* bias, float* y, int ldy, int M, int N, int K,
-               int relu, int accumulate, float* ws, size_t ws_floats, hipStream_t stream);
+               int relu, int accumulate, float* ws, size_t ws_floats, hipStream_t stream, const ExtraCols* xc = nullptr);
 int linear_dgrad(const float* dy, int lddy, const float* w, int ldw, const float* mask, int ldmask, int mask_cols, float* dx,
                  int lddx, int M, int Nin, int Kout, int accumulate, float* ws, size_t ws_floats, hipStream_t stream);
 int linear_wgrad(const float* dy, int lddy, const float* x, int ldx, float* dw, int lddw, int Mrows, int Nout, int Kin,
@@ -34,6 +34,25 @@
 int repack_flatten(const float* w, float* wp, int N, int C, int HW, hipStream_t stream);
 int transpose2d(const float* w, float* wt, int R, int C, hipStream_t stream);
 int pad_rows(const float* w, float* wp, int R, int C, int ld, hipStream_t stream);
+constexpr int REPACK_MAX_SEGS = 16;
+struct RepackSeg {
+    enum Op { CONV, FLATTEN, TRANSPOSE, PAD_ROWS };
+    int op = CONV, block0 = 0, nblocks = 0;
+    const float* src = nullptr; float* dst = nullptr; float* dst2 = nullptr; void* img = nullptr; void* planes = nullptr;
+    int a = 0, b = 0, c = 0, d = 0, e = 0;
+};
+struct RepackTable { int n = 0; RepackSeg seg[REPACK_MAX_SEGS]; };
+struct RepackBatch {
+    RepackTable t; int blocks = 0; hipStream_t stream;
+    explicit RepackBatch(hipStream_t s) : stream(s) {}
+    int conv(const float* w_oihw, float* wf, float* wd, int Cout, int Cin, int KH, int KW, int cpad, void* img = nullptr, void* planes = nullptr);
+    int flatten(const float* w, float* wp, int N, int C, int HW);
+    int transpose(const float* w, float* wt, int R, int C);
+    int pad_rows(const float* w, float* wp, int R, int C, int ld);
+    int flush();
+  private:
+    int add(const RepackSeg& g);
+};
 
 struct PackInfo {
     const int* select_inds;
@@ -85,13 +104,14 @@
                            const PackInfo& pk, float* scratch , float* ws, size_t ws_floats,
                            hipStream_t stream);
 int matrix_path_bits();
-int rnn_tm_prepare(const uint8_t* masks, const int* rows, int B, uint8_t* frame_mask, int* iota, hipStream_t stream);
+int rnn_tm_prepare(const uint8_t* masks, const int* rows, int B, uint8_t* frame_mask, int* iota, int* iota_valid, hipStream_t stream);
+constexpr int RNN_TM_COUNTER_FLOATS = 32;
 int rnn_tm_layer_forward(int rnn_type, int H, const RnnLayerParams& lp, const RnnWork& wk, const float* x, int ldx, const float* hinit,
                          const float* cinit, const uint8_t* frame_mask, int n, int T_total, int t0, int t1, float* ws, size_t ws_floats,
-                         hipStream_t stream);
+                         void* counters, hipStream_t stream);
 int rnn_tm_layer_backward(int rnn_type, int H, const RnnLayerParams& lp, const RnnWork& wk, const float* dout, float* dx, int lddx,
                           const float* dx_mask, int ldmask, int mask_cols, const uint8_t* frame_mask, const int* iota, int n, int T, int t0,
-                          int t1, float* scratch, float* ws, size_t ws_floats, hipStream_t stream);
+                          int t1, float* scratch, float* ws, size_t ws_floats, void* counters, hipStream_t stream);
 int rnn_tm_layer_param_grads(int rnn_type, int H, const RnnLayerParams& lp, const RnnWork& wk, const float* x, int ldx, int P, float* ws,
                              size_t ws_floats, hipStream_t stream);
 
diff --git a/habitat-lab_amd/csrc/problems.h b/habitat-lab_amd/csrc/problems.h
--- a/habitat-lab_amd/csrc/problems.h
+++ b/habitat-lab_amd/csrc/problems.h
@@ -939,6 +939,8 @@
     float* y; int ldy;
     int relu, vec;
     int accumulate;
+    static constexpr bool EXTRA_COLS = true;
+    ExtraCols xc;
     HAB_NO_KCTX
     using ACtx = WRowCtx;
     using BCtx = WRowCtx;
diff --git a/habitat-lab_amd/csrc/rnn.hip b/habitat-lab_amd/csrc/rnn.hip
--- a/habitat-lab_amd/csrc/rnn.hip
+++ b/habitat-lab_amd/csrc/rnn.hip
@@ -552,18 +552,21 @@
     const int i = blockIdx.x * blockDim.x + threadIdx.x;
     if (i < n) dst[i] = i;
 }
-int rnn_tm_prepare(const uint8_t* masks, const int* rows, int B, uint8_t* frame_mask, int* iota, hipStream_t stream) {
-    if (!masks || !frame_mask || !iota || B <= 0) return HAB_ERR_ARG;
+int rnn_tm_prepare(const uint8_t* masks, const int* rows, int B, uint8_t* frame_mask, int* iota, int* iota_valid, hipStream_t stream) {
+    if (!masks || !frame_mask || !iota || !iota_valid || B <= 0) return HAB_ERR_ARG;
     gather_u8_kernel<<<cdiv(B, 256), 256, 0, stream>>>(masks, rows, B, frame_mask);
-    iota_kernel<<<cdiv(B, 256), 256, 0, stream>>>(iota, B);
+    if (B > *iota_valid) {
+        iota_kernel<<<cdiv(B, 256), 256, 0, stream>>>(iota, B);
+        *iota_valid = B;
+    }
     HAB_LAUNCH_CHECK();
     return HAB_OK;
 }
 
-static bool tm_persist_ok(int rnn_type, int H, int n, int T, const float* ws, size_t ws_floats) {
+static bool tm_persist_ok(int rnn_type, int H, int n, int T, const void* counters) {
     static const bool on = hab_env_int("HAB_RNN_PERSIST", 1) != 0;
     const int G = rnn_type == RNN_GRU ? 3 : 4;
-    if (!on || (matrix_path_bits() & 4096) || !ws || ws_floats < 64) return false;
+    if (!on || (matrix_path_bits() & 4096) || !counters) return false;
     if (H != 128 && H != 256 && H != 512) return false;
     if (cdiv(n, 16) > RNNP_MAX_ROW_TILES) return false;
     if ((size_t)T * n * G * H * 4 >= ((size_t)1 << 31)) return false;
@@ -572,18 +575,17 @@
 
 int rnn_tm_layer_forward(int rnn_type, int H, const RnnLayerParams& lp, const RnnWork& wk, const float* x, int ldx, const float* hinit,
                          const float* cinit, const uint8_t* frame_mask, int n, int T_total, int t0, int t1, float* ws, size_t ws_floats,
-                         hipStream_t stream) {
+                         void* counters, hipStream_t stream) {
     const int G = rnn_type == RNN_GRU ? 3 : 4;
     const size_t f0 = (size_t)t0 * n;
     HAB_TRY(linear_fwd(x + f0 * ldx, ldx, lp.w_ih, lp.in_dim, lp.b_ih, wk.gi + f0 * G * H, G * H, (t1 - t0) * n, G * H, lp.in_dim, 0, 0, ws,
                        ws_floats, stream));
-    if (tm_persist_ok(rnn_type, H, n, T_total, ws, ws_floats) && wk.gates) {
+    if (tm_persist_ok(rnn_type, H, n, T_total, counters) && wk.gates) {
         TmPersistFwdArgs a;
         a.n = n; a.H = H; a.T = T_total; a.t0 = t0; a.t1 = t1;
         a.hinit = hinit; a.cinit = cinit; a.frame_mask = frame_mask; a.gi = wk.gi; a.w_hh = lp.w_hh; a.b_hh = lp.b_hh;
         a.gates = wk.gates; a.hn = wk.hn; a.hprev = wk.hprev; a.cprev = wk.cprev; a.c = wk.c; a.out = wk.out;
-        a.counters = reinterpret_cast<rnnp_u64*>(ws);
-        if (hipMemsetAsync(ws, 0, 16 * sizeof(rnnp_u64), stream) != hipSuccess) return HAB_ERR_ARG;
+        a.counters = reinterpret_cast<rnnp_u64*>(counters);
         const dim3 grid(H / 16, cdiv(n, 16));
         const int kch = H / 128;
         if (rnn_type == RNN_GRU) {
@@ -620,7 +622,7 @@
 
 int rnn_tm_layer_backward(int rnn_type, int H, const RnnLayerParams& lp, const RnnWork& wk, const float* dout, float* dx, int lddx,
                           const float* dx_mask, int ldmask, int mask_cols, const uint8_t* frame_mask, const int* iota, int n, int T, int t0,
-                          int t1, float* scratch, float* ws, size_t ws_floats, hipStream_t stream) {
+                          int t1, float* scratch, float* ws, size_t ws_floats, void* counters, hipStream_t stream) {
     const int G = rnn_type == RNN_GRU ? 3 : 4;
     if (H % 64) return HAB_ERR_UNSUPPORTED;
     float* dh_direct = scratch;
@@ -629,13 +631,12 @@
     const int K = G * H;
     const bool wide = K % 128 == 0;
     bool persisted = false;
-    if (tm_persist_ok(rnn_type, H, n, T, ws, ws_floats) && dout) {
+    if (tm_persist_ok(rnn_type, H, n, T, counters) && dout) {
         TmPersistBwdArgs a;
         a.n = n; a.H = H; a.T = T; a.t0 = t0; a.t1 = t1;
         a.frame_mask = frame_mask; a.dout = dout; a.w_hh_t = lp.w_hh_t; a.dh_direct = dh_direct; a.dc_carry = dc_carry;
         a.gates = wk.gates; a.hn = wk.hn; a.hprev = wk.hprev; a.cprev = wk.cprev; a.c = wk.c; a.dgi = wk.dgi; a.dgh = dgh;
-        a.counters = reinterpret_cast<rnnp_u64*>(ws);
-        if (hipMemsetAsync(ws, 0, 16 * sizeof(rnnp_u64), stream) != hipSuccess) return HAB_ERR_ARG;
+        a.counters = reinterpret_cast<rnnp_u64*>(counters);
         const dim3 grid(H / 16, cdiv(n, 16));
         const int kch = H / 128;
         if (rnn_type == RNN_GRU) {
```
